# connortannahill/MM-ADMM

Hardware: AMD Instinct MI355X
Metric: ADMM iterations/sec on 1M-node 2D mesh; achieved HBM GB/s in SpMV (higher is better)
Workload: dtype f64

## Files before the change

### include/mmadmm.h

```cpp
#ifndef MMADMM_H
#define MMADMM_H
#include <stdint.h>

#ifdef __cplusplus
extern "C" {
#endif

#define MMADMM_OK 0
#define MMADMM_ERR_INVALID 1
#define MMADMM_ERR_HIP 2
#define MMADMM_ERR_INVERTED 3
#define MMADMM_ERR_IO 4
#define MMADMM_ERR_RCCL 5
#define MMADMM_ERR_NOCONV 6
#define MMADMM_ERR_NONFINITE 7

#define MMADMM_BOUNDARY_FREE 0
#define MMADMM_BOUNDARY_FIXED 1
#define MMADMM_INTERIOR 2

typedef struct mmadmm_engine* mmadmm_handle;
typedef struct mmadmm_meshbuf* mmadmm_mesh;

typedef void (*mmadmm_monitor_fn)(int dim, const double* x, double* M_rowmajor, void* user);

typedef struct mmadmm_params {
  double dt;
  double tau;
  double rho;
  int grad_use;
  int device;
  int rank;
  int nranks;
  int partition;
} mmadmm_params;

typedef struct mmadmm_stats {
  long long steps;
  long long admm_iters;
  long long bfgs_iters;
  int max_bfgs;
  double last_primal;
  double last_dual;
  double t_prox_ms;
  double t_xupdate_ms;
  double t_step_ms;
  long long n_prox;
  long long n_xupdate;
  long long n_steps_timed;
  double prox_bytes;
  double xupdate_bytes;
  long long newton_iters;
  long long jacobians;
  long long cg_iters;
  double t_jac_ms;
  double t_solve_ms;
  double t_be_ms;
  long long regrids;
  long long regrid_rows;
  double regrid_gather_bytes;
  long long regrid_cand;
  long long regrid_fallbacks;
  int monitor_iso;
  double t_exchange_ms;
  long long n_exchange;
  double halo_send_bytes;
  double halo_recv_bytes;
  int interior_nodes;
  int overlap;
} mmadmm_stats;

int mmadmm_regrid(mmadmm_handle h, double t);
int mmadmm_set_regrid(mmadmm_handle h, int every_step);

int mmadmm_regrid_values(mmadmm_handle h, const double* M);
int mmadmm_regrid_values_device(mmadmm_handle h, const double* d_M, void* producer_stream);
int mmadmm_regrid_field(mmadmm_handle h, const double* u, double alpha);
int mmadmm_regrid_field_device(mmadmm_handle h, const double* d_u, double alpha, void* producer_stream);
int mmadmm_field_hessian(mmadmm_handle h, const double* u, double* H);
int mmadmm_field_hessian_device(mmadmm_handle h, const double* d_u, double* d_H, void* stream);
int mmadmm_get_device(mmadmm_handle h, const char* what, double* d_out, void* consumer_stream);
int mmadmm_field_monitor(int dim, int nP, const double* Xp, int nF, const int32_t* F, const double* u,
                         double alpha, double* H, double* M);

int mmadmm_transfer(mmadmm_handle h, const double* Xold, const double* Xnew, int C, const double* uold, double* unew,
                    int32_t* where, int* counts);
int mmadmm_transfer_device(mmadmm_handle h, const double* d_Xold, const double* d_Xnew, int C, const double* d_uold,
                           double* d_unew, int32_t* d_where, int* counts, void* stream);
int mmadmm_transfer_field(int dim, int nP, const double* Xold, int nF, const int32_t* F, const double* Xnew, int C,
                          const double* uold, double* unew, int32_t* where, int* counts);
int mmadmm_face_neighbours(int dim, int nP, int nF, const int32_t* F, int32_t* nbr);

const char* mmadmm_last_error(void);
int mmadmm_version(void);
int mmadmm_build_info(char* out, int len);

int mmadmm_builtin_monitor(int dim, int mon_type, mmadmm_monitor_fn* fn, void** user);
int mmadmm_monitor_grid(int dim, int nP, const double* Xp, mmadmm_monitor_fn fn, void* user, int* rows,
                        double* vals);

int mmadmm_mesh_reorient(int dim, int nP, const double* Xp, int nF, int32_t* F);

int mmadmm_create(int dim, int nP, const double* Xp, const double* Xc, int nF, const int32_t* F,
                  const int32_t* mask, const mmadmm_params* p, mmadmm_monitor_fn fn, void* user,
                  mmadmm_handle* out);
int mmadmm_step(mmadmm_handle h, int n_iters, double tol, double* Ih, int* admm_iters);
int mmadmm_euler_step(mmadmm_handle h, double* Ih);
int mmadmm_backward_euler_step(mmadmm_handle h, double dt, double tol, double* Ih, int* newton_iters);
int mmadmm_get_jacobian(mmadmm_handle h, long long* nnz, int32_t* ia, int32_t* ja, double* a);
int mmadmm_be_begin(mmadmm_handle h, double dt, double* Ih);
int mmadmm_be_residual(mmadmm_handle h, double dt, double* F, double* norm1, double* Ih);
int mmadmm_be_fsubjac(mmadmm_handle h, double* a);
int mmadmm_be_add(mmadmm_handle h, const double* dx);
int mmadmm_energy(mmadmm_handle h, double* E);
int mmadmm_done(mmadmm_handle h);
int mmadmm_get(mmadmm_handle h, const char* what, double* out);
int mmadmm_get_simplices(mmadmm_handle h, int32_t* F);
int mmadmm_sizes(mmadmm_handle h, int* nP, int* nF, int* grid_rows);
int mmadmm_set_timing(mmadmm_handle h, int on);
int mmadmm_stats_get(mmadmm_handle h, mmadmm_stats* s);
int mmadmm_stats_reset(mmadmm_handle h);
int mmadmm_options_get(mmadmm_handle h, char* buf, int cap);
int mmadmm_sync(mmadmm_handle h);
int mmadmm_destroy(mmadmm_handle h);

int mmadmm_mesh_rect(int dim, int nx, int ny, int nz, double xa, double xb, double ya, double yb,
                     double za, double zb, int btype, mmadmm_mesh* out);
int mmadmm_mesh_levelset2d(int nx, int ny, double xa, double xb, double ya, double yb, int btype,
                           int compact_mask, mmadmm_mesh* out);
int mmadmm_mesh_levelset3d(int nx, int ny, int nz, double xa, double xb, double ya, double yb, double za,
                           double zb, int btype, int compact_mask, mmadmm_mesh* out);
int mmadmm_mesh_shoulder(int dim, int nx, int ny, int nz, double xa, double xb, double ya, double yb, double za,
                         double zb, int btype, mmadmm_mesh* out);
int mmadmm_mesh_reference_points(mmadmm_mesh h, double* Xc);
int mmadmm_mesh_hexdisc(int N, double r, double cx, double cy, int btype, mmadmm_mesh* out);
int mmadmm_mesh_read(int dim, const char* tri, const char* pnts, const char* mask, mmadmm_mesh* out);
int mmadmm_mesh_sizes(mmadmm_mesh m, int* dim, int* nP, int* nF, int* mask_len);
int mmadmm_mesh_copy(mmadmm_mesh m, double* Xp, int32_t* F, int32_t* mask);
int mmadmm_mesh_free(mmadmm_mesh m);
int mmadmm_write_points(const char* path, int dim, int nP, const double* Xp);
int mmadmm_write_simplices(const char* path, int dim, int nF, const int32_t* F);

int mmadmm_debug_blockgrad(mmadmm_handle h, int s, const double* z, const double* dxpu, int flags,
                           double* out);

#define MMADMM_PART_RCB 0
#define MMADMM_PART_RANGES 1
#define MMADMM_UNIQUE_ID_BYTES 128
typedef struct mmadmm_comm_s* mmadmm_comm;
typedef struct mmadmm_plan_s* mmadmm_plan;
int mmadmm_layout_check(unsigned* host_word);
int mmadmm_comm_unique_id(void* out, int len);
int mmadmm_comm_create_rccl(int nranks, int rank, const void* uid, int device, mmadmm_comm* out);
int mmadmm_comm_create_rccl_timeout(int nranks, int rank, const void* uid, int device, double timeout_s,
                                    mmadmm_comm* out);
int mmadmm_comm_create_loopback(int nranks, mmadmm_comm* out);
typedef int (*mmadmm_allgather_fn)(void* user, const double* send, double* recv, long long count);
typedef int (*mmadmm_exchange_fn)(void* user, int npeers, const int* peer_rank, const double* send,
                                  const long long* send_off, const long long* send_count, double* recv,
                                  const long long* recv_off, const long long* recv_count);
int mmadmm_comm_create_host(int nranks, int rank, mmadmm_allgather_fn allgather, mmadmm_exchange_fn exchange,
                            void* user, mmadmm_comm* out);
int mmadmm_comm_destroy(mmadmm_comm c);
int mmadmm_comm_nranks(mmadmm_comm c, int* nranks);
int mmadmm_create_partitioned(int dim, int nP, const double* Xp, const double* Xc, int nF, const int32_t* F,
                              const int32_t* mask, const mmadmm_params* p, mmadmm_monitor_fn fn, void* user,
                              mmadmm_comm comm, mmadmm_handle* out);
int mmadmm_local_nodes(mmadmm_handle h, int* n_local, int32_t* global_ids);
int mmadmm_plan_create(int dim, int nP, const double* Xp, int nF, const int32_t* F, int nranks, int rank, int method,
                       mmadmm_plan* out);
int mmadmm_plan_sizes(mmadmm_plan h, int* nLocalNodes, int* nLocalSimplices, int* nSources, int* nSend, int* nRecv,
                      int* nPeers, int* nInterface);
int mmadmm_plan_get(mmadmm_plan h, int32_t* localNodes, int32_t* localSimplices, int32_t* incPtr, int32_t* incSrc,
                    int32_t* sendOff, int32_t* peers);
int mmadmm_plan_destroy(mmadmm_plan h);

int mmadmm_devmath(int op, int n, const double* in, double* out);

#ifdef __cplusplus
}
#endif
#endif
```

### mm-admm_amd/csrc/host/engine.cpp

```cpp
#include <algorithm>
#include <chrono>
#include <cmath>
#include <cstring>
#include <limits>
#include <memory>
#include <mutex>
#include <string>
#include <vector>

#include "../../../include/mmx_sparse.h"
#include "../kernels/admm_kernels.h"
#include "../kernels/field_kernels.h"
#include "../kernels/regrid_kernels.h"
#include "../kernels/transfer_kernels.h"
#include "comm.h"
#include "common.h"
#include "partition.h"
#include "transfer.h"
#include "xup_records.h"

#define MMX_SP(expr)                                                                     \
  do {                                                                                   \
    const int rc_ = (expr);                                                              \
    if (rc_ != MMADMM_OK) throw ::mmx::Error(rc_, std::string(#expr) + ": " + mmadmm_last_error()); \
// ... 366 lines not shown
        timed_.push_back({a0, a1, b1});
      }
      prevEnd = b1;
      if (deferRed) {
        if (firstProx && i < nIters - 1) {
          prevEnd = nullptr;
          launch_reduce_partials(partA_.p + slice * i, nbp, res_ + (size_t)i * 2 * kNumPartials, st_, red_);
          firstDeferred = i + 1;
        } else if (i == nIters - 1) {
          const int i0 = firstProx ? i : firstDeferred;
          launch_reduce_steps(partA_.p + slice * i0, slice, nbp, partB_.p, nbx, nIters - i0,
                              res_ + (size_t)i0 * 2 * kNumPartials, st_, red_);
        }
      } else if (resid) {
        prevEnd = nullptr;
        launch_reduce_partials2(partA_.p, nbp, res_ + (size_t)i * 2 * kNumPartials, partB_.p, nbx,
                                res_ + (size_t)i * 2 * kNumPartials + kNumPartials, st_, red_);
      } else {
        prevEnd = nullptr;
        launch_reduce_partials(partA_.p, nbp, res_ + (size_t)i * 2 * kNumPartials, st_, red_);
      }
      done = i + 1;
      if (early) {
        std::vector<double> rv;
        fetchResults(res_ + (size_t)i * 2 * kNumPartials, 1, rv);
        const double* r = rv.data();
        primal = sqrt(r[kNumPartials + 2]);
        dual = sqrt(r[1]);
        if (r[4] > 0 || (primal < tol && dual < tol)) break;
      }
    }
    MMX_HIP(hipMemcpyAsync(Vp_.p, x_.p, (size_t)nP_ * D * sizeof(double), hipMemcpyDeviceToDevice, st_));
    vpVersion_++;
    if (timing) {
      eStep1 = nextEvent();
      MMX_HIP(hipEventRecord(eStep1, st_));
    }
    fetchResults(res_, done, hostRes_);
    MMX_HIP(hipGetLastError());
    bool bad = false;
    long long bf = 0;
    int mx = 0;
    for (int i = 0; i < done; ++i) {
      const double* r = &hostRes_[(size_t)i * 2 * kNumPartials];
      bad |= r[4] > 0;
      bf += (long long)r[3];
      mx = std::max(mx, (int)r[5]);
    }
#ifdef MMX_HINT_PROBE
    {
      double hits = 0;
      for (int i = 0; i < done; ++i) hits += hostRes_[(size_t)i * 2 * kNumPartials + 2];
      fprintf(stderr, "[hint-probe] step %lld: %.0f hits of %.0f lookups in %d proxes\n", (long long)stepsTaken_, hits,
              3.0 * nF_ * done, done);
    }
#endif
    const double* last = &hostRes_[(size_t)(done - 1) * 2 * kNumPartials];
    primal = sqrt(last[kNumPartials + 2]);
    dual = sqrt(last[1]);
    st_stats_.admm_iters += done;
    st_stats_.bfgs_iters += bf;
    st_stats_.max_bfgs = mx;
    st_stats_.last_primal = primal;
    st_stats_.last_dual = dual;
    st_stats_.steps += 1;
    if (timing) {
      stepEv_.push_back({eStep0, eStep1});
      if (evUsed_ >= kEvResolve) resolveTimed();
    }
    stepsTaken_++;
    if (bad) throwBad("in prox");
    if (Ih) *Ih = hostRes_[0];
    if (itersOut) *itersOut = done;
  }

  double eulerStep() override {
    clearInvFlag();
    int nb = 0;
    launch_grad_simplex<D>(m_, x_.p, gs_.p, false, partA_.p, &nb, st_);
    launch_reduce_partials(partA_.p, nb, res_, st_, red_);
    exchange(1);
    launch_euler_apply<D>(m_, knobs_, gs_.p, x_.p, prm_.dt / prm_.tau, st_);
    std::vector<double> rv;
    fetchResults(res_, 1, rv);
    const double* r = rv.data();
    if (r[4] > 0) throwBad("in the explicit Euler gradient");
    return r[0];
  }

  double backwardEulerStep(double dtBE, double tol, int* newtonOut) override {
    if (nranks_ > 1) throw Error(MMADMM_ERR_INVALID, "backward Euler runs on one rank (no element partition)");
    const auto tStep = Clock::now();
    const int n = nP_ * D;
    ensureJacobian();
    const double dtot = dtBE / prm_.tau;
    const double SAFETY_FAC = 1.0 / 10.0;
    const int MAX_ITERS = 1000;
    clearInvFlag();
    MMX_HIP(hipMemcpyAsync(xn_.p, x_.p, (size_t)n * sizeof(double), hipMemcpyDeviceToDevice, st_));
    int nb = 0, nb2 = 0;
    launch_grad_simplex<D>(m_, x_.p, gs_.p, false, partA_.p, &nb, st_);
    launch_euler_apply<D>(m_, knobs_, gs_.p, x_.p, dtot, st_);
    if (!beStepTaken_) buildJacobian(dtBE);
    int nIter = 0;
    double Ih = 0.0, normPrev = INFINITY;
    std::vector<double> rv;
    void* mst = nullptr;
    MMX_SP(mmx_matrix_stream(jac_, &mst));
    do {
      launch_grad_simplex<D>(m_, x_.p, gs_.p, false, partA_.p, &nb, st_);
      launch_be_residual<D>(m_, knobs_, gs_.p, x_.p, xn_.p, dtot, rhs_.p, partB_.p, &nb2, st_);
      launch_reduce_partials2(partA_.p, nb, res_, partB_.p, nb2, res_ + kNumPartials, st_, red_);
      fetchResults(res_, 1, rv);
      if (rv[4] > 0) throwBad("in backward Euler");
      Ih = rv[0];
      const double norm = rv[kNumPartials];
      if (norm < SAFETY_FAC * tol) break;
      if (!beStepTaken_ || std::fabs(norm - normPrev) / norm < 0.25) {
        buildJacobian(dtBE);
        beStepTaken_ = true;
      }
      waitStream();
      const auto tSolve = Clock::now();
      MMX_SP(mmx_matrix_set_rhs_device(jac_, rhs_.p));
      int cgIter = 0;
      MMX_SP(mmx_matrix_solve_device(jac_, &jprm_, dx_.p, &cgIter, 0));
      st_stats_.t_solve_ms += msSince(tSolve);
      if (cgIter > 0) st_stats_.cg_iters += cgIter;
      if (cgIter <= 0)
        throw Error(MMADMM_ERR_NOCONV, "backward Euler: CG-STAB did not converge (reference: assert(cgIter > 0))");
      launch_add_inplace(n, x_.p, dx_.p, st_);
      nIter++;
      normPrev = norm;
    } while (nIter < MAX_ITERS);
    streamWait();
    st_stats_.steps += 1;
    st_stats_.newton_iters += nIter;
    st_stats_.t_be_ms += msSince(tStep);
    if (newtonOut) *newtonOut = nIter;
    return Ih;
  }

  void newtonOp(int op, double dt, const double* in, double* out, double* sc) override {
    if (nranks_ > 1) throw Error(MMADMM_ERR_INVALID, "backward Euler runs on one rank (no element partition)");
    ensureJacobian();
    const int n = nP_ * D;
    std::vector<double> rv;
    int nb = 0, nb2 = 0;
    if (op == 0 || op == 1) clearInvFlag();
    if (op == 0) {
      MMX_HIP(hipMemcpyAsync(xn_.p, x_.p, (size_t)n * sizeof(double), hipMemcpyDeviceToDevice, st_));
      launch_grad_simplex<D>(m_, x_.p, gs_.p, false, partA_.p, &nb, st_);
      launch_reduce_partials(partA_.p, nb, res_, st_, red_);
      launch_euler_apply<D>(m_, knobs_, gs_.p, x_.p, dt / prm_.tau, st_);
      fetchResults(res_, 1, rv);
      if (rv[4] > 0) throwBad("in backward Euler");
      if (sc) sc[0] = rv[0];
    } else if (op == 1) {
      launch_grad_simplex<D>(m_, x_.p, gs_.p, false, partA_.p, &nb, st_);
      launch_be_residual<D>(m_, knobs_, gs_.p, x_.p, xn_.p, dt / prm_.tau, rhs_.p, partB_.p, &nb2, st_);
      launch_reduce_partials2(partA_.p, nb, res_, partB_.p, nb2, res_ + kNumPartials, st_, red_);
      fetchResults(res_, 1, rv);
      if (rv[4] > 0) throwBad("in backward Euler");
      std::vector<double> r((size_t)n);
      MMX_HIP(hipMemcpyAsync(r.data(), rhs_.p, (size_t)n * sizeof(double), hipMemcpyDeviceToHost, st_));
      streamWait();
      for (int i = 0; i < n; ++i) out[i] = -r[i];
      if (sc) {
        sc[0] = rv[0];
        sc[1] = rv[kNumPartials];
      }
    } else if (op == 2) {
      const double h = 10.0 * sqrt(std::numeric_limits<double>::epsilon());
      launch_fd_jac<D>(m_, Vp_.p, h, dv_.p, st_, fdWork_.p);
      clearInvFlag();
      if (jraw_.n != jja_.n) jraw_.alloc(std::max<size_t>(jja_.n, 1));
      launch_jac_assemble<D>(m_, knobs_, jia_.p, jja_.p, dv_.p, 1.0, jraw_.p, st_, false, maxColNodes_);
      MMX_HIP(hipMemcpyAsync(out, jraw_.p, jja_.n * sizeof(double), hipMemcpyDeviceToHost, st_));
      streamWait();
    } else if (op == 3) {
      MMX_HIP(hipMemcpyAsync(dx_.p, in, (size_t)n * sizeof(double), hipMemcpyHostToDevice, st_));
      launch_add_inplace(n, x_.p, dx_.p, st_);
      streamWait();
    } else {
      throw Error(MMADMM_ERR_INVALID, "newtonOp: unknown op");
    }
  }

  void jacobian(long long* nnz, int32_t* ia, int32_t* ja, double* a) override {
    if (!jac_) throw Error(MMADMM_ERR_INVALID, "no Jacobian yet: run a backward Euler step first");
    if (nnz) *nnz = (long long)jja_.n;
    if (ia) MMX_HIP(hipMemcpyAsync(ia, jia_.p, jia_.n * sizeof(int32_t), hipMemcpyDeviceToHost, st_));
    if (ja) MMX_HIP(hipMemcpyAsync(ja, jja_.p, jja_.n * sizeof(int32_t), hipMemcpyDeviceToHost, st_));
    if (a) MMX_HIP(hipMemcpyAsync(a, jval_.p, jval_.n * sizeof(double), hipMemcpyDeviceToHost, st_));
    streamWait();
  }

  double energy() override {
    int nb = 0;
    launch_energy<D>(m_, Vp_.p, partA_.p, &nb, st_);
    clearInvFlag();
    launch_reduce_partials(partA_.p, nb, res_, st_, red_);
    std::vector<double> rv;
    fetchResults(res_, 1, rv);
    return rv[0];
  }

  void done() override {
    MMX_HIP(hipMemcpyAsync(Vp_.p, x_.p, (size_t)nP_ * D * sizeof(double), hipMemcpyDeviceToDevice, st_));
    vpVersion_++;
    streamWait();
  }

  void get(const std::string& what, double* out) override {
    const DevBuf<double>* b = nullptr;
    if (what == "x") b = &x_;
    else if (what == "xPrev") b = &xPrev_;
    else if (what == "xBar") b = &xBar_;
    else if (what == "z" || what == "u") {
      if (!kZUInterleaved) {
        b = what == "z" ? &z_ : &u_;
      } else {
        std::vector<double> h(z_.n);
        MMX_HIP(hipMemcpyAsync(h.data(), z_.p, z_.n * sizeof(double), hipMemcpyDeviceToHost, st_));
        streamWait();
        const int sh = what == "u" ? D : 0;
        for (int s = 0; s < nF_; ++s)
          for (int i = 0; i < K; ++i) out[(size_t)s * K + i] = h[(size_t)s * 2 * K + (i / D) * 2 * D + i % D + sh];
        return;
      }
    }
    else if (what == "points") b = &Vp_;
    else if (what == "hess") b = &B_;
    else if (what == "gs") b = &gs_;
    else if (what == "grid") {
      if (gridOnDevice_) {
        MMX_HIP(hipMemcpyAsync(out, gvals_.p, gvals_.n * sizeof(double), hipMemcpyDeviceToHost, st_));
        streamWait();
      } else {
        std::memcpy(out, grid_.vals.data(), grid_.vals.size() * sizeof(double));
      }
      return;
    } else if (what == "Ehat") {
      std::memcpy(out, EhatH_, D * D * sizeof(double));
      return;
    } else {
      throw Error(MMADMM_ERR_INVALID, "mmadmm_get: unknown field '" + what + "'");
    }
    if (b == &B_) {
      std::vector<double> h(b->n);
      MMX_HIP(hipMemcpyAsync(h.data(), b->p, b->n * sizeof(double), hipMemcpyDeviceToHost, st_));
      streamWait();
      for (int s = 0; s < nF_; ++s)
        for (int ij = 0; ij < K * K; ++ij) out[(size_t)s * K * K + ij] = h[bIndex(s, ij)];
      return;
    }
    MMX_HIP(hipMemcpyAsync(out, b->p, b->n * sizeof(double), hipMemcpyDeviceToHost, st_));
    streamWait();
  }

  static size_t bIndex(int s, int ij) {
    if (D == 3 && MMX_B3_PAIRS) return ((size_t)(s >> 6) * K * K + (ij & ~1)) * 64 + 2 * (s & 63) + (ij & 1);
    return ((size_t)(s >> 6) * K * K + ij) * 64 + (s & 63);
  }

  void getSimplices(int32_t* F) override {
    for (size_t i = 0; i < plan_.Flocal.size(); ++i) F[i] = plan_.localNodes[plan_.Flocal[i]];
  }

  void localNodes(int* n, int32_t* ids) override {
    if (n) *n = nP_;
    if (ids) std::memcpy(ids, plan_.localNodes.data(), plan_.localNodes.size() * sizeof(int32_t));
  }

  void sizes(int* nP, int* nF, int* gridRows) override {
    if (nP) *nP = nP_;
    if (nF) *nF = nF_;
    if (gridRows) *gridRows = (int)(grid_.vals.size() / (D * D));
  }

  void setTiming(bool on) override {
    resolveTimed();
    timing_ = on;
  }

  void stats(mmadmm_stats* s) override {
    resolveTimed();
    *s = st_stats_;
    const double nF = nF_, nP = nP_;
    const double ts = knobs_.tslot ? 1.0 : 0.0;
    s->prox_bytes = nF * (4.0 * (D + 1) + 1 + 8.0 * (2 * K + K * K) * 2 + 8.0 * K * 2 + ts * 8.0 * K) +
                    nP * 8.0 * D;
    const double ch = D == 2 ? MMX_XU_CH2D : knobs_.xupCh;
    const double fixed = knobs_.xupRec ? nP * (4.0 * kXupRecInts + 8.0 + 4.0 * ch) + 4.0 * (double)xupTail_
                                 : 4.0 * (nP + 1) + 4.0 * (D + 1) * nF + 8.0 * nP;
    s->xupdate_bytes = fixed + (16.0 - 8.0 * ts) * K * nF + 8.0 * D * nP * 2;
    s->monitor_iso = iso_ ? 1 : 0;
    s->halo_send_bytes = 8.0 * D * (double)plan_.sendOff.size();
    s->halo_recv_bytes = nranks_ > 1 ? 8.0 * D * (double)plan_.recvRows : 0.0;
    s->interior_nodes = nInner_;
    s->overlap = knobs_.overlap;
  }

  std::string options() const override { return knobs_.text(); }

  void resetStats() override {
    resolveTimed();
    const mmadmm_stats z{};
    st_stats_ = z;
  }

  void resolveTimed() {
    if (stepEv_.empty() && timed_.empty() && exEv_.empty()) return;
    streamWait();
    float ms = 0;
    for (auto& p : stepEv_) {
      MMX_HIP(hipEventElapsedTime(&ms, p.first, p.second));
      st_stats_.t_step_ms += ms;
      st_stats_.n_steps_timed += 1;
    }
    if (st2_) MMX_HIP(hipStreamSynchronize(st2_));
    for (auto& p : exEv_) {
      MMX_HIP(hipEventElapsedTime(&ms, p.first, p.second));
      st_stats_.t_exchange_ms += ms;
      st_stats_.n_exchange += 1;
    }
    exEv_.clear();
    for (auto& t : timed_) {
      MMX_HIP(hipEventElapsedTime(&ms, t.a0, t.a1));
      st_stats_.t_prox_ms += ms;
      st_stats_.n_prox += 1;
      MMX_HIP(hipEventElapsedTime(&ms, t.a1, t.b1));
      st_stats_.t_xupdate_ms += ms;
      st_stats_.n_xupdate += 1;
    }
    stepEv_.clear();
    timed_.clear();
    evUsed_ = 0;
  }

  void sync() override { streamWait(); }

  void debugBlockGrad(int s, const double* z, const double* dx, int flags, double* out) override {
    if (s < 0 || s >= nF_) throw Error(MMADMM_ERR_INVALID, "debug_blockgrad: simplex out of range");
    DevBuf<double> dz, ddx, dout;
    dz.upload(z, K, st_);
    ddx.upload(dx, K, st_);
    dout.alloc(K + 2);
    launch_debug_blockgrad<D>(m_, s, dz.p, ddx.p, dout.p, flags, st_);
    MMX_HIP(hipMemcpyAsync(out, dout.p, (K + 2) * sizeof(double), hipMemcpyDeviceToHost, st_));
    streamWait();
  }

 private:
  struct Timed {
    hipEvent_t a0, a1, b1;
  };

  void profMark(const char* what, std::chrono::steady_clock::time_point& t) const {
    if (!knobs_.schedProf) return;
    const auto now = std::chrono::steady_clock::now();
    fprintf(stderr, "[sched] engine %s %.3f s\n", what, std::chrono::duration<double>(now - t).count());
    t = now;
  }
  void ensureJacobian() {
    if (jac_) return;
    auto tp = std::chrono::steady_clock::now();
    const int n = nP_ * D;
    mmx_struc sp = nullptr;
    MMX_SP(mmx_struc_create(n, 0, &sp));
    std::vector<int32_t> ia(n + 1), ja;
    long long nnz = 0;
    int rc = mmx_struc_mesh_pattern(sp, D, (int)(Fh_.size() / (D + 1)), Fh_.data());
    if (rc == MMADMM_OK) rc = mmx_struc_pack(sp);
    if (rc == MMADMM_OK) rc = mmx_struc_get(sp, nullptr, &nnz, nullptr, nullptr);
    if (rc == MMADMM_OK) {
      ja.resize(nnz);
      rc = mmx_struc_get(sp, nullptr, &nnz, ia.data(), ja.data());
    }
    profMark("pattern", tp);
    int dev = prm_.device;
    if (dev < 0) MMX_HIP(hipGetDevice(&dev));
    if (rc == MMADMM_OK) rc = mmx_matrix_create_from_struc(dev, sp, &jac_);
    (void)mmx_struc_destroy(sp);
    profMark("matrix create", tp);
    if (rc != MMADMM_OK) throw Error(rc, std::string("backward Euler Jacobian: ") + mmadmm_last_error());
    mmx_param_iter_mesh(&jprm_);
    maxColNodes_ = 0;
    for (int r = 0; r < n; ++r) maxColNodes_ = std::max(maxColNodes_, (ia[r + 1] - ia[r]) / D);
    jia_.upload(ia.data(), ia.size(), st_);
    jja_.upload(ja.data(), ja.size(), st_);
    jval_.alloc(std::max<size_t>(nnz, 1));
    dv_.alloc(std::max<size_t>((size_t)nF_ * (D + 1) * D * K, 1));
    if (knobs_.fdjFast) fdWork_.alloc((size_t)nF_ * (D + 1) + 1);
    xn_.alloc((size_t)n);
    rhs_.alloc((size_t)n);
    dx_.alloc((size_t)n);
    streamWait();
  }

  void buildJacobian(double dtBE) {
    if (jacVp_ == vpVersion_ && jacDt_ == dtBE) return;
    jacVp_ = vpVersion_;
    jacDt_ = dtBE;
    const auto t0 = Clock::now();
    auto tp = t0;
    const double h = 10.0 * sqrt(std::numeric_limits<double>::epsilon());
    launch_fd_jac<D>(m_, Vp_.p, h, dv_.p, st_, fdWork_.p);
    clearInvFlag();
    launch_jac_assemble<D>(m_, knobs_, jia_.p, jja_.p, dv_.p, dtBE / prm_.tau, jval_.p, st_, true, maxColNodes_);
    streamWait();
    profMark("FD Jacobian + assembly", tp);
    MMX_SP(mmx_matrix_set_values_device(jac_, jval_.p));
    if (!jacFactored_) {
      MMX_SP(mmx_matrix_sfac(jac_, &jprm_));
      jacFactored_ = true;
      profMark("sfac", tp);
    }
    streamWait();
    st_stats_.jacobians += 1;
    st_stats_.t_jac_ms += msSince(t0);
  }
  using Clock = std::chrono::steady_clock;
  static double msSince(Clock::time_point t) {
    return std::chrono::duration<double, std::milli>(Clock::now() - t).count();
  }

  static double hostDet(const double (&a)[3][3]) {
    if (D == 2) return a[0][0] * a[1][1] - a[1][0] * a[0][1];
    const double h0 = a[0][0] * (a[1][1] * a[2][2] - a[1][2] * a[2][1]);
    const double h1 = a[0][1] * (a[1][0] * a[2][2] - a[1][2] * a[2][0]);
    const double h2 = a[0][2] * (a[1][0] * a[2][1] - a[1][1] * a[2][0]);
    return h0 - h1 + h2;
  }

  void exchange(int mode, const PackZX& pz = {}, hipStream_t st = nullptr) {
    if (nranks_ == 1) return;
    if (!st) st = st_;
    hipEvent_t e0 = nullptr, e1 = nullptr;
    if (timing_ && mode == 0) {
      e0 = nextEvent();
      MMX_HIP(hipEventRecord(e0, st));
    }
    launch_pack_export<D>(mode, (int)plan_.sendOff.size(), expOff_.p, z_.p, uPtr(), gs_.p, w_, export_.p, st, pz);
    comm_->exchange(rank_, export_.p, remote_.p, plan_.peers, D, st);
    if (e0) {
      e1 = nextEvent();
      MMX_HIP(hipEventRecord(e1, st));
      exEv_.push_back({e0, e1});
    }
  }

  void xupdateHalo(const StepScalars& sc, int* nbx, bool resid, bool useTs, const PackZX& pz) {
    if (!knobs_.overlap) {
      exchange(0, pz);
      launch_xupdate<D>(m_, knobs_, sc, xBar_.p, z_.p, uPtr(), x_.p, partB_.p, nbx, resid, st_, useTs);
      return;
    }
    MMX_HIP(hipEventRecord(evProx_, st_));
    DeviceMesh<D> mi = m_;
    mi.xupHi = nInner_;
    int nb1 = 0, nb2 = 0;
    launch_xupdate<D>(mi, knobs_, sc, xBar_.p, z_.p, uPtr(), x_.p, partB_.p, &nb1, resid, st_, useTs);
    MMX_HIP(hipStreamWaitEvent(st2_, evProx_, 0));
    exchange(0, pz, st2_);
    MMX_HIP(hipEventRecord(evEx_, st2_));
    MMX_HIP(hipStreamWaitEvent(st_, evEx_, 0));
    DeviceMesh<D> mb = m_;
    mb.xupLo = nInner_;
    launch_xupdate<D>(mb, knobs_, sc, xBar_.p, z_.p, uPtr(), x_.p, partB_.p + (size_t)nb1 * kNumPartials, &nb2, resid,
                      st_, useTs);
    *nbx = nb1 + nb2;
  }

  void waitStream() {
    if (!knobs_.spin) {
      streamWait();
      return;
    }
    if (!evSync_) MMX_HIP(hipEventCreateWithFlags(&evSync_, hipEventDisableTiming));
    MMX_HIP(hipEventRecord(evSync_, st_));
    hipError_t r;
    while ((r = hipEventQuery(evSync_)) == hipErrorNotReady) __builtin_ia32_pause();
    MMX_HIP(r);
  }

  void streamWait() {
    if (nranks_ > 1 && comm_)
      comm_->wait(st_);
    else
      MMX_HIP(hipStreamSynchronize(st_));
  }

  void fetchResults(const double* dev, int rows, std::vector<double>& out) {
    const size_t cnt = (size_t)rows * 2 * kNumPartials;
    out.resize(cnt);
    if (resH_) {
      waitStream();
      std::memcpy(out.data(), resH_ + (dev - res_), cnt * sizeof(double));
      return;
    }
    if (nranks_ == 1) {
      MMX_HIP(hipMemcpyAsync(out.data(), dev, cnt * sizeof(double), hipMemcpyDeviceToHost, st_));
      streamWait();
      return;
    }
    if (resAll_.n < cnt * nranks_) resAll_.alloc(cnt * nranks_);
    comm_->allgather(rank_, dev, resAll_.p, cnt, st_);
    std::vector<double> all(cnt * nranks_);
    MMX_HIP(hipMemcpyAsync(all.data(), resAll_.p, all.size() * sizeof(double), hipMemcpyDeviceToHost, st_));
    streamWait();
    for (size_t i = 0; i < cnt; ++i) {
      const bool isMax = (i % kNumPartials) == 5;
      double v = all[i];
      for (int q = 1; q < nranks_; ++q) v = isMax ? std::max(v, all[(size_t)q * cnt + i]) : v + all[(size_t)q * cnt + i];
      out[i] = v;
    }
  }

  void setRegrid(bool on) override { regridEachStep_ = on; }

  void regrid(double t) override {
    if (nranks_ > 1) {
      const bool all = knobs_.regridGatherAll;
      if (!all && regridNear(t)) return;
      st_stats_.regrid_fallbacks += all ? 0 : 1;
    }
    regridAll(t);
  }

  void afterProducer(void* stream) {
    if (!stream) return;
    if (!evIn_) MMX_HIP(hipEventCreateWithFlags(&evIn_, hipEventDisableTiming));
    MMX_HIP(hipEventRecord(evIn_, (hipStream_t)stream));
    MMX_HIP(hipStreamWaitEvent(st_, evIn_, 0));
  }
  void beforeConsumer(void* stream) {
    if (!stream) {
      streamWait();
      return;
    }
    if (!evOut_) MMX_HIP(hipEventCreateWithFlags(&evOut_, hipEventDisableTiming));
    MMX_HIP(hipEventRecord(evOut_, st_));
    MMX_HIP(hipStreamWaitEvent((hipStream_t)stream, evOut_, 0));
  }
  void singleRankOnly(const char* what) const {
    if (nranks_ > 1) throw Error(MMADMM_ERR_INVALID, std::string(what) + ": single rank only (no element partition)");
  }
  void fieldScratch() {
    if (fldE_.p) return;
    fldE_.alloc(std::max<size_t>(field_ebuf_doubles<D>(nF_), 1));
    fldG_.alloc((size_t)nP_ * D);
  }

  void regridFrom(int src, const double* p, bool onDevice, double alpha, void* stream) override {
    singleRankOnly(src == kMonField ? "mmadmm_regrid_field" : "mmadmm_regrid_values");
    const size_t n = (size_t)nP_ * (src == kMonField ? 1 : D * D);
    if (!onDevice) {
      if (fldIn_.n < n) fldIn_.alloc(n);
      MMX_HIP(hipMemcpyAsync(fldIn_.p, p, n * sizeof(double), hipMemcpyHostToDevice, st_));
      streamWait();
      p = fldIn_.p;
    } else {
      afterProducer(stream);
    }
    srcPtr_ = p;
    srcAlpha_ = alpha;
    regridAll(0.0, (MonSource)src);
    srcPtr_ = nullptr;
    if (onDevice && !knobs_.iso) streamWait();
  }

  void fieldHessian(const double* u, double* H, bool onDevice, void* stream) override {
    singleRankOnly("mmadmm_field_hessian");
    fieldScratch();
    if (!onDevice) {
      if (fldIn_.n < (size_t)nP_) fldIn_.alloc(nP_);
      if (fldOut_.n < (size_t)nP_ * D * D) fldOut_.alloc((size_t)nP_ * D * D);
      MMX_HIP(hipMemcpyAsync(fldIn_.p, u, (size_t)nP_ * sizeof(double), hipMemcpyHostToDevice, st_));
      launch_field_hessian<D>(Vp_.p, fldIn_.p, F_.p, nF_, incPtr_.p, incOff_.p, nodeOrder_.p, nP_, fldE_.p, fldG_.p, 1.0,
                              fldOut_.p, nullptr, st_);
      MMX_HIP(hipGetLastError());
      MMX_HIP(hipMemcpyAsync(H, fldOut_.p, (size_t)nP_ * D * D * sizeof(double), hipMemcpyDeviceToHost, st_));
      streamWait();
      return;
    }
    afterProducer(stream);
    launch_field_hessian<D>(Vp_.p, u, F_.p, nF_, incPtr_.p, incOff_.p, nodeOrder_.p, nP_, fldE_.p, fldG_.p, 1.0, H,
                            nullptr, st_);
    MMX_HIP(hipGetLastError());
    beforeConsumer(stream);
  }

  void transferScratch() {
    if (trNbr_.p) return;
    trNbrH_.assign(std::max<size_t>((size_t)nF_ * (D + 1), 1), -1);
    build_face_neighbours(D, nF_, plan_.Flocal.data(), trNbrH_.data());
    trNbr_.upload(trNbrH_.data(), trNbrH_.size(), st_);
    trWhere_.alloc(std::max(nP_, 1));
    trCnt_.alloc(kTransferCountInts);
  }

  void transfer(const double* Xold, const double* Xnew, int C, const double* uold, double* unew, int32_t* where,
                int* counts, bool onDevice, void* stream) override {
    const char* who = onDevice ? "mmadmm_transfer_device" : "mmadmm_transfer";
    singleRankOnly(who);
    transferScratch();
    const size_t nx = (size_t)nP_ * D, nu = (size_t)nP_ * C;
    int cnt[kTransferCountInts];
    if (!onDevice) {
      if (trStage_.n < 2 * nx + 2 * nu) trStage_.alloc(2 * nx + 2 * nu);
      double *dXo = trStage_.p, *dXn = dXo + nx, *dUo = dXn + nx, *dUn = dUo + nu;
      MMX_HIP(hipMemcpyAsync(dXo, Xold, nx * sizeof(double), hipMemcpyHostToDevice, st_));
      if (Xnew) MMX_HIP(hipMemcpyAsync(dXn, Xnew, nx * sizeof(double), hipMemcpyHostToDevice, st_));
      MMX_HIP(hipMemcpyAsync(dUo, uold, nu * sizeof(double), hipMemcpyHostToDevice, st_));
      launch_transfer<D>(dXo, Xnew ? dXn : Vp_.p, F_.p, incPtr_.p, incOff_.p, nodeOrder_.p, trNbr_.p, nP_, C, dUo, dUn,
                         trWhere_.p, trCnt_.p, st_);
      MMX_HIP(hipGetLastError());
      MMX_HIP(hipMemcpyAsync(unew, dUn, nu * sizeof(double), hipMemcpyDeviceToHost, st_));
      if (where) MMX_HIP(hipMemcpyAsync(where, trWhere_.p, (size_t)nP_ * sizeof(int32_t), hipMemcpyDeviceToHost, st_));
      if (counts) MMX_HIP(hipMemcpyAsync(cnt, trCnt_.p, sizeof cnt, hipMemcpyDeviceToHost, st_));
      streamWait();
    } else {
      if (D == 2 && ((((uintptr_t)Xold) | ((uintptr_t)(Xnew ? Xnew : Vp_.p))) & 15))
        throw Error(MMADMM_ERR_INVALID, std::string(who) + ": 2D position arrays must be 16-byte aligned");
      afterProducer(stream);
      launch_transfer<D>(Xold, Xnew ? Xnew : Vp_.p, F_.p, incPtr_.p, incOff_.p, nodeOrder_.p, trNbr_.p, nP_, C, uold, unew,
                         where ? where : trWhere_.p, trCnt_.p, st_);
      MMX_HIP(hipGetLastError());
      if (counts) MMX_HIP(hipMemcpyAsync(cnt, trCnt_.p, sizeof cnt, hipMemcpyDeviceToHost, st_));
      beforeConsumer(stream);
      if (counts && stream) streamWait();
    }
    if (counts) transfer_sum_counts(cnt, counts);
  }

  void getDevice(const std::string& what, double* dOut, void* stream) override {
    singleRankOnly("mmadmm_get_device");
    const DevBuf<double>* b = what == "x" ? &x_ : what == "points" ? &Vp_ : nullptr;
    if (!b) throw Error(MMADMM_ERR_INVALID, "mmadmm_get_device: unknown field '" + what + "' (x, points)");
    MMX_HIP(hipMemcpyAsync(dOut, b->p, (size_t)nP_ * D * sizeof(double), hipMemcpyDeviceToDevice, st_));
    beforeConsumer(stream);
  }

  bool regridNear(double t) {
    constexpr int DD = D * D;
    const int nG = plan_.nP;
    const int nbl = std::max(1, std::min(256, (nP_ + 255) / 256));
    const int nbe = std::max(1, std::min(256, (nF_ + 255) / 256));
    const size_t smallN = (size_t)std::max(2 * D, nranks_);
    if (!rgnPart_.p) {
      rgnPart_.alloc((size_t)256 * 2 * D + 256 * D);
      rgnSmallS_.alloc(smallN);
      rgnSmallR_.alloc(smallN * nranks_);
      rgnSbox_.alloc((size_t)nranks_ * 2 * D);
      rgnCnt_.alloc(nranks_ + 1);
      rgnSend_.alloc((size_t)nranks_ * maxOwned_ * (D + 1));
      rgnGid_.upload(plan_.localNodes.data(), plan_.localNodes.size(), st_);
      ownGidH_.assign(ownAllGidH_.begin() + (size_t)rank_ * maxOwned_,
                      ownAllGidH_.begin() + (size_t)rank_ * maxOwned_ + std::max(nOwned_, 1));
      rgnOwnGid_.upload(ownGidH_.data(), ownGidH_.size(), st_);
      rgTmp_.alloc(gvals_.n);
      rgTmp2_.alloc(gvals_.n);
      MMX_HIP(hipHostMalloc((void**)&rgnHost_, sizeof(double) * ((size_t)256 * 3 * D + 2 * smallN * nranks_ + 64),
                            hipHostMallocDefault));
    }
    double* H0 = rgnHost_;
    launch_bbox<D>(Vp_.p, nP_, rgnPart_.p, nbl, st_);
    launch_extent<D>(Vp_.p, F_.p, nF_, rgnPart_.p + (size_t)256 * 2 * D, nbe, st_);
    MMX_HIP(hipMemcpyAsync(H0, rgnPart_.p, sizeof(double) * nbl * 2 * D, hipMemcpyDeviceToHost, st_));
    MMX_HIP(hipMemcpyAsync(H0 + (size_t)256 * 2 * D, rgnPart_.p + (size_t)256 * 2 * D, sizeof(double) * nbe * D,
                           hipMemcpyDeviceToHost, st_));
    streamWait();
    double llo[3] = {INFINITY, INFINITY, INFINITY}, lhi[3] = {-INFINITY, -INFINITY, -INFINITY};
    for (int b = 0; b < nbl; ++b)
      for (int d = 0; d < D; ++d) {
        llo[d] = std::min(llo[d], H0[(size_t)b * 2 * D + d]);
        lhi[d] = std::max(lhi[d], H0[(size_t)b * 2 * D + D + d]);
      }
    for (int d = 0; d < D; ++d) extMax_[d] = 0.0;
    for (int b = 0; b < nbe; ++b)
      for (int d = 0; d < D; ++d) extMax_[d] = std::max(extMax_[d], H0[(size_t)256 * 2 * D + (size_t)b * D + d]);
    double* hs = H0 + (size_t)256 * 3 * D;
    double* hr = hs + smallN;
    auto smallGather = [&](const double* in, int n) {
      MMX_HIP(hipMemcpyAsync(rgnSmallS_.p, in, sizeof(double) * n, hipMemcpyHostToDevice, st_));
      comm_->allgather(rank_, rgnSmallS_.p, rgnSmallR_.p, (size_t)n, st_);
      MMX_HIP(hipMemcpyAsync(hr, rgnSmallR_.p, sizeof(double) * n * nranks_, hipMemcpyDeviceToHost, st_));
      streamWait();
    };
    for (int d = 0; d < D; ++d) {
      hs[d] = llo[d];
      hs[D + d] = lhi[d];
    }
    smallGather(hs, 2 * D);
    double lo[3] = {INFINITY, INFINITY, INFINITY}, hi[3] = {-INFINITY, -INFINITY, -INFINITY};
    for (int q = 0; q < nranks_; ++q)
      for (int d = 0; d < D; ++d) {
        lo[d] = std::min(lo[d], hr[(size_t)q * 2 * D + d]);
        hi[d] = std::max(hi[d], hr[(size_t)q * 2 * D + D + d]);
      }
    setGridGeometry(nG, lo, hi);
    const CellGrid cg = cellGrid(lo, hi);
    int marg[3] = {0, 0, 0};
    const GridBox R = rowBox(llo, lhi, marg);
    const int passes = smoothPasses();
    const GridBox H = widenBox(R, passes);
    double slo[3] = {0, 0, 0}, shi[3] = {0, 0, 0};
    double diam = 0.0;
    for (int d = 0; d < D; ++d) diam += extMax_[d] * extMax_[d];
    diam = std::sqrt(diam);
    const double marginScale = knobs_.regridMargin;
    for (int d = 0; d < D; ++d) {
      const std::vector<double>& g = d == 0 ? grid_.gx : d == 1 ? grid_.gy : grid_.gz;
      const int sd = (D == 3 && d < 2) ? 1 - d : d;
      const double mu = marginScale * (diam + 2.0 * (g[1] - g[0]));
      slo[d] = g[H.lo[sd]] - mu;
      shi[d] = g[H.hi[sd]] + mu;
    }
    for (int d = 0; d < D; ++d) {
      hs[d] = slo[d];
      hs[D + d] = shi[d];
    }
    smallGather(hs, 2 * D);
    MMX_HIP(hipMemcpyAsync(rgnSbox_.p, hr, sizeof(double) * nranks_ * 2 * D, hipMemcpyHostToDevice, st_));
    MMX_HIP(hipMemsetAsync(rgnCnt_.p, 0, sizeof(int) * (nranks_ + 1), st_));
    launch_select_owned<D>(Vp_.p, ownLocal_.p, rgnOwnGid_.p, nOwned_, nranks_, rank_, rgnSbox_.p, rgnCnt_.p,
                           rgnSend_.p, maxOwned_, st_);
    std::vector<int> cnt(nranks_ + 1);
    MMX_HIP(hipMemcpyAsync(cnt.data(), rgnCnt_.p, sizeof(int) * nranks_, hipMemcpyDeviceToHost, st_));
    streamWait();
    for (int q = 0; q < nranks_; ++q) hs[q] = (double)cnt[q];
    smallGather(hs, nranks_);
    std::vector<HaloPeer> peers;
    int nRecv = 0;
    for (int q = 0; q < nranks_; ++q) {
      if (q == rank_) continue;
      const int sc = cnt[q], rc = (int)hr[(size_t)q * nranks_ + rank_];
      if (sc == 0 && rc == 0) continue;
      HaloPeer p;
      p.rank = q;
      p.sendOff = q * maxOwned_;
      p.sendCount = sc;
      p.recvOff = nRecv;
      p.recvCount = rc;
      nRecv += rc;
      peers.push_back(p);
    }
    const int nCand = nP_ + nRecv;
    if ((int)rgnRecv_.n < std::max(nRecv, 1) * (D + 1)) rgnRecv_.alloc((size_t)std::max(nRecv, 1) * (D + 1) * 2);
    if ((int)rgnCandX_.n < nCand * D) {
      rgnCandX_.alloc((size_t)nCand * D * 2);
      rgnCandGid_.alloc((size_t)nCand * 2);
      rgnCellOf_.alloc((size_t)nCand * 2);
      rgnNodes_.alloc((size_t)nCand * 2);
      rgnMon_.alloc((size_t)nCand * DD * 2);
    }
    comm_->exchange(rank_, rgnSend_.p, rgnRecv_.p, peers, D + 1, st_);
    launch_build_cand<D>(Vp_.p, rgnGid_.p, nP_, rgnRecv_.p, nRecv, rgnCandX_.p, rgnCandGid_.p, st_);
    evalMonitorAt(rgnCandX_.p, nCand, t, rgnMon_.p);
    ensureCells(cg);
    launch_bin<D>(rgnCandX_.p, nCand, cg, rgnCellOf_.p, rgCounts_.p, rgStarts_.p, rgFill_.p, rgnNodes_.p, rgScan_.p,
                  rgScanBytes_, st_);
    double clo[3], chi[3];
    for (int d = 0; d < 3; ++d) {
      clo[d] = (d < D && slo[d] <= lo[d]) ? -INFINITY : slo[d];
      chi[d] = (d < D && shi[d] >= hi[d]) ? INFINITY : shi[d];
    }
    NnCand nc{rgnCandGid_.p, {clo[0], clo[1], clo[2]}, {chi[0], chi[1], chi[2]}, rgnCnt_.p + nranks_};
    launch_nn_fill<D>(rgnCandX_.p, cg, rgStarts_.p, rgnNodes_.p, gx_.p, gy_.p, D == 3 ? gz_.p : gy_.p, grid_.nx,
                      grid_.ny, grid_.nz, rgnMon_.p, rgTmp_.p, H, st_, nc);
    int fail = 0;
    MMX_HIP(hipMemcpyAsync(&fail, rgnCnt_.p + nranks_, sizeof(int), hipMemcpyDeviceToHost, st_));
    streamWait();
    hs[0] = (double)fail;
    smallGather(hs, 1);
    for (int q = 0; q < nranks_; ++q)
      if (hr[q] != 0.0) return false;
    smoothCommit(R, passes, true);
    st_stats_.regrid_rows = (long long)(H.hi[0] - H.lo[0] + 1) * (H.hi[1] - H.lo[1] + 1) * (H.hi[2] - H.lo[2] + 1);
    st_stats_.regrid_gather_bytes = (double)sizeof(double) * ((size_t)nranks_ * (4 * D + nranks_ + 1) +
                                                              (size_t)nRecv * (D + 1));
    st_stats_.regrid_cand = nCand;
    MMX_HIP(hipGetLastError());
    gridOnDevice_ = true;
    updateIso();
    m_ = makeView();
    st_stats_.regrids += 1;
    return true;
  }

  void updateIso() {
    iso_ = false;
    if (!knobs_.iso) return;
    const long long np = (long long)(gvals_.n / (D * D));
    if (np <= 0) return;
    if ((long long)giso_.n != np) giso_.alloc(np);
    if (!isoFlag_.p) isoFlag_.alloc(1);
    MMX_HIP(hipMemsetAsync(isoFlag_.p, 0, sizeof(int), st_));
    launch_iso_compact<D>(gvals_.p, np, giso_.p, isoFlag_.p, st_);
    int notIso = 1;
    MMX_HIP(hipMemcpyAsync(&notIso, isoFlag_.p, sizeof(int), hipMemcpyDeviceToHost, st_));
    streamWait();
    iso_ = (notIso == 0);
  }
  void uploadGridCoords() {
    gx_.upload(grid_.gx.data(), grid_.gx.size(), st_);
    gy_.upload(grid_.gy.data(), grid_.gy.size(), st_);
    if (D == 3) {
      gz_.upload(grid_.gz.data(), grid_.gz.size(), st_);
      const std::vector<double>* ax[3] = {&grid_.gx, &grid_.gy, &grid_.gz};
      for (int a = 0; a < 3; ++a) {
        const std::vector<double>& g = *ax[a];
        const size_t nc = g.size() > 1 ? g.size() - 1 : 1;
        std::vector<double>& t = gcellH_[a];
        t.assign(4 * nc, 0.0);
        for (size_t i = 0; i + 1 < g.size(); ++i) {
          const double h = g[i + 1] - g[i];
          t[4 * i] = g[i];
          t[4 * i + 1] = h;
          t[4 * i + 2] = 1.0 / h;
        }
        gcell_[a].upload(t.data(), t.size(), st_);
      }
    }
  }
  void setGridGeometry(int nG, const double* lo, const double* hi) {
    grid_geometry(D, nG, lo, hi, grid_);
    uploadGridCoords();
  }
  CellGrid cellGrid(const double* lo, const double* hi) const {
    CellGrid cg{};
    const int gn[3] = {grid_.nx, grid_.ny, grid_.nz};
    cg.hmin = INFINITY;
    for (int d = 0; d < 3; ++d) {
      const double ext = d < D ? hi[d] - lo[d] : 0.0;
      cg.lo[d] = d < D ? lo[d] : 0.0;
      cg.n[d] = (d < D && ext > 0) ? std::max(1, gn[d] / 2) : 1;
      cg.inv[d] = (d < D && ext > 0) ? cg.n[d] / ext : 0.0;
      if (d < D && ext > 0) cg.hmin = std::min(cg.hmin, ext / cg.n[d]);
    }
    if (!(cg.hmin < INFINITY)) cg.hmin = 0.0;
    return cg;
  }
  void ensureCells(const CellGrid& cg) {
    const int ncell = cg.n[0] * cg.n[1] * cg.n[2];
    if ((int)rgStarts_.n < ncell + 1) {
      rgCounts_.alloc(ncell + 1);
      rgStarts_.alloc(ncell + 1);
      rgFill_.alloc(ncell);
      rgScanBytes_ = bin_scan_bytes(ncell);
      rgScan_.alloc(std::max<size_t>(rgScanBytes_, 1));
    }
  }
  static int smoothPasses() { return (D == 2) ? 5 : 2; }
  GridBox rowBox(const double* llo, const double* lhi, int* marg) const {
    const int gn3[3] = {grid_.nx, grid_.ny, D == 3 ? grid_.nz : 0};
    GridBox R{{0, 0, 0}, {gn3[0], gn3[1], gn3[2]}};
    for (int d = 0; d < D; ++d) {
      const std::vector<double>& g = d == 0 ? grid_.gx : d == 1 ? grid_.gy : grid_.gz;
      const double h = g[1] - g[0];
      const int M = (int)std::ceil(2.0 * extMax_[d] / h) + 2;
      marg[d] = M;
      R.lo[d] = std::max(0, std::min(gn3[d], (int)std::floor((llo[d] - g[0]) / h) - M));
      R.hi[d] = std::max(0, std::min(gn3[d], (int)std::floor((lhi[d] - g[0]) / h) + 1 + M));
    }
    return R;
  }
  GridBox widenBox(const GridBox& b, int w) const {
    const int gn3[3] = {grid_.nx, grid_.ny, D == 3 ? grid_.nz : 0};
    GridBox o = b;
    for (int d = 0; d < D; ++d) {
      o.lo[d] = std::max(0, b.lo[d] - w);
      o.hi[d] = std::min(gn3[d], b.hi[d] + w);
    }
    return o;
  }
  void evalMonitorAt(const double* X, int n, double t, double* mon) {
    constexpr int DD = D * D;
    if (builtin_monitor_kind(monFn_, monUser_) == 7) {
      double c[3];
      moving_bump_centre(t, c);
      launch_monitor_tv<D>(X, n, c, mon, st_);
    } else {
      std::vector<double> Xh((size_t)n * D), mv((size_t)n * DD);
      MMX_HIP(hipMemcpyAsync(Xh.data(), X, Xh.size() * sizeof(double), hipMemcpyDeviceToHost, st_));
      streamWait();
      for (int v = 0; v < n; ++v) {
        double M[9];
        for (int i = 0; i < DD; ++i) M[i] = 0.0;
        monFn_(D, &Xh[(size_t)v * D], M, monUser_);
        std::memcpy(&mv[(size_t)v * DD], M, DD * sizeof(double));
      }
      MMX_HIP(hipMemcpyAsync(mon, mv.data(), mv.size() * sizeof(double), hipMemcpyHostToDevice, st_));
      streamWait();
    }
  }
  void smoothCommit(const GridBox& R, int passes, bool part) {
    double* cur = rgTmp_.p;
    double* oth = part ? rgTmp2_.p : gvals_.p;
    for (int it = 0; it < passes; ++it) {
      launch_smooth<D>(cur, oth, grid_.nx, grid_.ny, grid_.nz, widenBox(R, part ? passes - 1 - it : 0), st_);
      std::swap(cur, oth);
    }
    if (part) {
      launch_box_commit<D>(cur, gvals_.p, D == 3 ? gpad_.p : nullptr, grid_.nx, grid_.ny, grid_.nz, R, st_);
    } else {
      if (cur != gvals_.p)
        MMX_HIP(hipMemcpyAsync(gvals_.p, cur, gvals_.n * sizeof(double), hipMemcpyDeviceToDevice, st_));
      if (D == 3) launch_pad_rows(gvals_.p, (long long)(gvals_.n / 9), gpad_.p, st_);
    }
  }

  void regridAll(double t, MonSource src = kMonCallback) {
    constexpr int DD = D * D;
    const int nG = (nranks_ > 1) ? plan_.nP : nP_;
    const int nb = std::max(1, std::min(256, (nG + 255) / 256));
    if (!rgPart_.p) {
      rgPart_.alloc((size_t)512 * 2 * D + 256 * D);
      rgMon_.alloc((size_t)nG * DD);
      rgCellOf_.alloc(nG);
      rgNodes_.alloc(nG);
      rgTmp_.alloc(gvals_.n);
      if (nranks_ > 1) rgTmp2_.alloc(gvals_.n);
      if (nranks_ > 1) {
        rgXg_.alloc((size_t)nG * D);
        rgSend_.alloc((size_t)maxOwned_ * D);
        rgRecv_.alloc((size_t)nranks_ * maxOwned_ * D);
      }
      MMX_HIP(hipHostMalloc((void**)&rgHost_, sizeof(double) * (512 * 2 * D + 256 * D), hipHostMallocDefault));
    }
    const double* X = Vp_.p;
    const bool part = nranks_ > 1;
    const int nbl = part ? std::max(1, std::min(256, (nP_ + 255) / 256)) : 0;
    const int nbe = part ? std::max(1, std::min(256, (nF_ + 255) / 256)) : 0;
    double* extPart = rgPart_.p + (size_t)512 * 2 * D;
    if (part) {
      launch_rows_gather(D, ownLocal_.p, nOwned_, Vp_.p, rgSend_.p, st_);
      comm_->allgather(rank_, rgSend_.p, rgRecv_.p, (size_t)maxOwned_ * D, st_);
      launch_rows_scatter(D, ownAllGid_.p, nranks_ * maxOwned_, rgRecv_.p, rgXg_.p, st_);
      X = rgXg_.p;
      launch_bbox<D>(Vp_.p, nP_, rgPart_.p + (size_t)256 * 2 * D, nbl, st_);
      launch_extent<D>(Vp_.p, F_.p, nF_, extPart, nbe, st_);
    }
    launch_bbox<D>(X, nG, rgPart_.p, nb, st_);
    MMX_HIP(hipMemcpyAsync(rgHost_, rgPart_.p, sizeof(double) * nb * 2 * D, hipMemcpyDeviceToHost, st_));
    if (part) {
      MMX_HIP(hipMemcpyAsync(rgHost_ + (size_t)256 * 2 * D, rgPart_.p + (size_t)256 * 2 * D, sizeof(double) * nbl * 2 * D,
                             hipMemcpyDeviceToHost, st_));
      MMX_HIP(hipMemcpyAsync(rgHost_ + (size_t)512 * 2 * D, extPart, sizeof(double) * nbe * D, hipMemcpyDeviceToHost,
                             st_));
    }
    streamWait();
    double lo[3] = {INFINITY, INFINITY, INFINITY}, hi[3] = {-INFINITY, -INFINITY, -INFINITY};
    double llo[3] = {INFINITY, INFINITY, INFINITY}, lhi[3] = {-INFINITY, -INFINITY, -INFINITY};
    for (int b = 0; b < nb; ++b)
      for (int d = 0; d < D; ++d) {
        lo[d] = std::min(lo[d], rgHost_[(size_t)b * 2 * D + d]);
        hi[d] = std::max(hi[d], rgHost_[(size_t)b * 2 * D + D + d]);
      }
    for (int b = 0; b < nbl; ++b)
      for (int d = 0; d < D; ++d) {
        llo[d] = std::min(llo[d], rgHost_[(size_t)(256 + b) * 2 * D + d]);
        lhi[d] = std::max(lhi[d], rgHost_[(size_t)(256 + b) * 2 * D + D + d]);
      }
    if (part) {
      for (int d = 0; d < D; ++d) extMax_[d] = 0.0;
      for (int b = 0; b < nbe; ++b)
        for (int d = 0; d < D; ++d) extMax_[d] = std::max(extMax_[d], rgHost_[(size_t)512 * 2 * D + (size_t)b * D + d]);
    }
    grid_geometry(D, nG, lo, hi, grid_);
    uploadGridCoords();
    CellGrid cg{};
    const int gn[3] = {grid_.nx, grid_.ny, grid_.nz};
    cg.hmin = INFINITY;
    for (int d = 0; d < 3; ++d) {
      const double ext = d < D ? hi[d] - lo[d] : 0.0;
      cg.lo[d] = d < D ? lo[d] : 0.0;
      cg.n[d] = (d < D && ext > 0) ? std::max(1, gn[d] / 2) : 1;
      cg.inv[d] = (d < D && ext > 0) ? cg.n[d] / ext : 0.0;
      if (d < D && ext > 0) cg.hmin = std::min(cg.hmin, ext / cg.n[d]);
    }
    if (!(cg.hmin < INFINITY)) cg.hmin = 0.0;
    const int ncell = cg.n[0] * cg.n[1] * cg.n[2];
    if ((int)rgStarts_.n < ncell + 1) {
      rgCounts_.alloc(ncell + 1);
      rgStarts_.alloc(ncell + 1);
      rgFill_.alloc(ncell);
      rgScanBytes_ = bin_scan_bytes(ncell);
      rgScan_.alloc(std::max<size_t>(rgScanBytes_, 1));
    }
    launch_bin<D>(X, nG, cg, rgCellOf_.p, rgCounts_.p, rgStarts_.p, rgFill_.p, rgNodes_.p, rgScan_.p, rgScanBytes_,
                  st_);
    if (src == kMonCallback && builtin_monitor_kind(monFn_, monUser_) == 7) src = kMonBuiltin7;
    if (src == kMonValues) {
      MMX_HIP(hipMemcpyAsync(rgMon_.p, srcPtr_, (size_t)nG * DD * sizeof(double), hipMemcpyDeviceToDevice, st_));
    } else if (src == kMonField) {
      fieldScratch();
      launch_field_hessian<D>(X, srcPtr_, F_.p, nF_, incPtr_.p, incOff_.p, nodeOrder_.p, nP_, fldE_.p, fldG_.p,
                              srcAlpha_, nullptr, rgMon_.p, st_);
    } else if (src == kMonBuiltin7) {
      double c[3];
      moving_bump_centre(t, c);
      launch_monitor_tv<D>(X, nG, c, rgMon_.p, st_);
    } else {
      std::vector<double> Xh((size_t)nG * D), mv((size_t)nG * DD);
      MMX_HIP(hipMemcpyAsync(Xh.data(), X, Xh.size() * sizeof(double), hipMemcpyDeviceToHost, st_));
      streamWait();
      for (int v = 0; v < nG; ++v) {
        double M[9];
        for (int i = 0; i < DD; ++i) M[i] = 0.0;
        monFn_(D, &Xh[(size_t)v * D], M, monUser_);
        std::memcpy(&mv[(size_t)v * DD], M, DD * sizeof(double));
      }
      MMX_HIP(hipMemcpyAsync(rgMon_.p, mv.data(), mv.size() * sizeof(double), hipMemcpyHostToDevice, st_));
      streamWait();
    }
    const int passes = (D == 2) ? 5 : 2;
    const int gn3[3] = {grid_.nx, grid_.ny, D == 3 ? grid_.nz : 0};
    GridBox R{{0, 0, 0}, {gn3[0], gn3[1], gn3[2]}};
    if (part) {
      for (int d = 0; d < D; ++d) {
        const std::vector<double>& g = d == 0 ? grid_.gx : d == 1 ? grid_.gy : grid_.gz;
        const double h = g[1] - g[0];
        const int M = (int)std::ceil(2.0 * extMax_[d] / h) + 2;
        R.lo[d] = std::max(0, std::min(gn3[d], (int)std::floor((llo[d] - g[0]) / h) - M));
        R.hi[d] = std::max(0, std::min(gn3[d], (int)std::floor((lhi[d] - g[0]) / h) + 1 + M));
      }
    }
    auto widen = [&](const GridBox& b, int w) {
      GridBox o = b;
      for (int d = 0; d < D; ++d) {
        o.lo[d] = std::max(0, b.lo[d] - w);
        o.hi[d] = std::min(gn3[d], b.hi[d] + w);
      }
      return o;
    };
    const GridBox H = widen(R, part ? passes : 0);
    launch_nn_fill<D>(X, cg, rgStarts_.p, rgNodes_.p, gx_.p, gy_.p, D == 3 ? gz_.p : gy_.p, grid_.nx, grid_.ny,
                      grid_.nz, rgMon_.p, rgTmp_.p, H, st_);
    double* cur = rgTmp_.p;
    double* oth = part ? rgTmp2_.p : gvals_.p;
    for (int it = 0; it < passes; ++it) {
      launch_smooth<D>(cur, oth, grid_.nx, grid_.ny, grid_.nz, widen(R, part ? passes - 1 - it : 0), st_);
      std::swap(cur, oth);
    }
    if (part) {
      launch_box_commit<D>(cur, gvals_.p, D == 3 ? gpad_.p : nullptr, grid_.nx, grid_.ny, grid_.nz, R, st_);
    } else {
      if (cur != gvals_.p)
        MMX_HIP(hipMemcpyAsync(gvals_.p, cur, gvals_.n * sizeof(double), hipMemcpyDeviceToDevice, st_));
      if (D == 3) launch_pad_rows(gvals_.p, (long long)(gvals_.n / 9), gpad_.p, st_);
    }
    st_stats_.regrid_rows = (long long)(H.hi[0] - H.lo[0] + 1) * (H.hi[1] - H.lo[1] + 1) * (H.hi[2] - H.lo[2] + 1);
    st_stats_.regrid_gather_bytes = part ? (double)nranks_ * maxOwned_ * D * sizeof(double) : 0.0;
    st_stats_.regrid_cand = part ? nG : 0;
    MMX_HIP(hipGetLastError());
    gridOnDevice_ = true;
    updateIso();
    m_ = makeView();
    st_stats_.regrids += 1;
  }

  DeviceMesh<D> makeView() const {
    DeviceMesh<D> m{};
    m.nP = nP_;
    m.nF = nF_;
    m.F = F_.p;
    m.sbits = sbits_.p;
    m.nodeInterior = interior_.p;
    m.inc_ptr = incPtr_.p;
    m.inc_off = incOff_.p;
    m.remote = nranks_ > 1 ? remote_.p : nullptr;
    m.tslot = knobs_.tslot ? tslot_.p : nullptr;
    m.gcache = gcache_.p;
    m.tieList = tieList_.p;
    m.tieCount = tieCount_.p + tiePar_;
    m.tieStale = tieCount_.p + (tiePar_ ^ 1);
    m.invFlag = tieCount_.p + 2;
    m.nodeOrder = nodeOrder_.p;
    m.xupLo = 0;
    m.xupHi = nP_;
    m.prox2dWave = knobs_.prox2dWave;
    m.xupSweep = knobs_.xupSweep;
    m.xupCh = knobs_.xupCh;
    m.xupEarly = knobs_.xupEarly;
    m.forceTie = knobs_.forceTie;
    m.monHint = knobs_.monHint;
    if (knobs_.xupRec) {
      m.xrec = xrec_.p;
      m.xinv = xinv_.p;
      m.xslot = xslot_.p;
      m.xslotStride = xslotStride_;
      m.xslotCh = xslotCh_;
    }
    m.invdiag = invdiag_.p;
    m.Vc = compMesh_ ? Vc_.p : nullptr;
    m.gx = gx_.p;
    m.gy = gy_.p;
    m.gz = (D == 3) ? gz_.p : gy_.p;
    m.gvals = gvals_.p;
    m.gpad = (D == 3) ? gpad_.p : nullptr;
    for (int a = 0; a < 3; ++a) m.gcell[a] = (D == 3) ? gcell_[a].p : nullptr;
    m.giso = iso_ ? giso_.p : nullptr;
    m.gnx = grid_.nx;
    m.gny = grid_.ny;
    m.gnz = grid_.nz;
    m.ghx = grid_.gx[1] - grid_.gx[0];
    m.ghy = grid_.gy[1] - grid_.gy[0];
    m.ghz = (D == 3) ? grid_.gz[1] - grid_.gz[0] : 1.0;
    m.grhx = 1.0 / m.ghx;
    m.grhy = 1.0 / m.ghy;
    m.grhz = 1.0 / m.ghz;
    const int ns[3] = {grid_.nx, grid_.ny, grid_.nz};
    double* A[3] = {&m.gax, &m.gay, &m.gaz};
    double* SP[3] = {&m.gspx, &m.gspy, &m.gspz};
    double* NS[3] = {&m.gnsx, &m.gnsy, &m.gnsz};
    double* RNS[3] = {&m.grnsx, &m.grnsy, &m.grnsz};
    for (int d = 0; d < 3; ++d) {
      const bool on = d < D;
      *A[d] = on ? grid_.lo[d] : 0.0;
      *SP[d] = on ? grid_.hi[d] - grid_.lo[d] : 0.0;
      *NS[d] = on ? (double)ns[d] : 1.0;
      *RNS[d] = 1.0 / *NS[d];
    }
    for (int i = 0; i < D * D; ++i) m.Ehat[i] = EhatH_[i];
    m.powd = powd_;
    m.w = w_;
    m.compMesh = compMesh_ ? 1 : 0;
    return m;
  }

  void ensureResults(int nIters) {
    if (nIters <= resultsCap_) return;
    resultsCap_ = std::max(nIters, 64);
    const size_t n = (size_t)resultsCap_ * 2 * kNumPartials;
    if (nranks_ == 1 && knobs_.spin) {
      if (resH_) MMX_HIP(hipHostFree(resH_));
      resH_ = nullptr;
      MMX_HIP(hipHostMalloc((void**)&resH_, n * sizeof(double), hipHostMallocMapped));
      MMX_HIP(hipHostGetDevicePointer((void**)&res_, resH_, 0));
    } else {
      results_.alloc(n);
      res_ = results_.p;
    }
  }

  void clearInvFlag() { MMX_HIP(hipMemsetAsync(tieCount_.p + 2, 0, sizeof(unsigned), st_)); }

  [[noreturn]] void throwBad(const char* where) {
    unsigned flag = 0;
    MMX_HIP(hipMemcpyAsync(&flag, tieCount_.p + 2, sizeof(unsigned), hipMemcpyDeviceToHost, st_));
    streamWait();
    if (flag) {
      MMX_HIP(hipMemsetAsync(tieCount_.p + 2, 0, sizeof(unsigned), st_));
      streamWait();
      throw Error(MMADMM_ERR_INVERTED, std::string("inverted element ") + where + " (reference: assert(Edet > 0))");
    }
    if (nranks_ > 1 && regridEachStep_)
      throw Error(MMADMM_ERR_NONFINITE, std::string("non-finite energy ") + where +
                                            ": a monitor evaluation left this rank's regrid box (no element inverted)");
    throw Error(MMADMM_ERR_NONFINITE, std::string("non-finite energy ") + where +
                                          " without an inverted element (a monitor value that is not finite)");
  }

  hipEvent_t nextEvent() {
    if (evUsed_ == evPool_.size()) {
      hipEvent_t e;
      MMX_HIP(hipEventCreateWithFlags(&e, hipEventDisableSystemFence));
      evPool_.push_back(e);
    }
    return evPool_[evUsed_++];
  }

  static std::vector<int32_t> orientedSimplices(int nP, const double* Xp, int nF, const int32_t* F) {
    std::vector<int32_t> Fh(F, F + (size_t)nF * (D + 1));
    for (int32_t v : Fh)
      if (v < 0 || v >= nP) throw Error(MMADMM_ERR_INVALID, "simplex vertex id out of range");
    reorient_simplices(D, Xp, nF, Fh.data());
    return Fh;
  }

  std::vector<int32_t> Fh_;
  PartitionPlan plan_;
  const EngineKnobs knobs_;
  int nP_ = 0, nF_ = 0;
  mmadmm_params prm_{};
  bool compMesh_ = false;
  double w_ = 0, powd_ = 0;
  double EhatH_[9] = {0};
  std::vector<int32_t> maskH_;
  HostGrid grid_;
  mmadmm_monitor_fn monFn_ = nullptr;
  void* monUser_ = nullptr;
  bool regridEachStep_ = false, gridOnDevice_ = false;
  DevBuf<double> rgPart_, rgMon_, rgTmp_, rgTmp2_, rgXg_, rgSend_, rgRecv_;
  DevBuf<double> fldE_, fldG_, fldIn_, fldOut_;
  std::vector<int32_t> trNbrH_;
  DevBuf<int32_t> trNbr_, trWhere_, trCnt_;
  DevBuf<double> trStage_;
  const double* srcPtr_ = nullptr;
  double srcAlpha_ = 1.0;
  hipEvent_t evIn_ = nullptr, evOut_ = nullptr;
  double extMax_[3] = {0.0, 0.0, 0.0};
  DevBuf<int> ownLocal_, ownAllGid_;
  std::vector<int> ownAllGidH_, ownGidH_;
  DevBuf<double> rgnPart_, rgnSmallS_, rgnSmallR_, rgnSbox_, rgnSend_, rgnRecv_, rgnCandX_, rgnMon_;
  DevBuf<int> rgnCnt_, rgnGid_, rgnOwnGid_, rgnCandGid_, rgnCellOf_, rgnNodes_;
  double* rgnHost_ = nullptr;
  int nOwned_ = 0, maxOwned_ = 1;
  DevBuf<int> rgCellOf_, rgNodes_, rgCounts_, rgStarts_, rgFill_;
  DevBuf<unsigned char> rgScan_;
  size_t rgScanBytes_ = 0;
  double* rgHost_ = nullptr;
  hipStream_t st_ = nullptr;
  hipStream_t st2_ = nullptr;
  hipEvent_t evProx_ = nullptr, evEx_ = nullptr;
  int nInner_ = 0;
  std::vector<std::pair<hipEvent_t, hipEvent_t>> exEv_;
  DevBuf<int32_t> F_, incPtr_, incOff_;
  DevBuf<double> tslot_;
  DevBuf<uint8_t> sbits_, interior_;
  DevBuf<double> gcell_[3];
  DevBuf<double> giso_;
  DevBuf<int> isoFlag_;
  bool iso_ = false;
  std::vector<double> gcellH_[3];
  DevBuf<double> invdiag_, Vc_, gx_, gy_, gz_, gvals_, Vp_, x_, xPrev_, xBar_, z_, u_, gs_, B_, B2_, gcache_, gpad_;
  DevBuf<double> partA_, partB_, results_, export_, remote_, resAll_, redScratch_;
  RedWork red_;
  DevBuf<int32_t> expOff_, tieList_, nodeOrder_;
  DevBuf<int32_t> xrec_, xslot_;
  DevBuf<double> xinv_;
  int xslotStride_ = 0, xslotCh_ = 0;
  long long xupTail_ = 0;
  DevBuf<unsigned> tieCount_;
  int tiePar_ = 0;
  Comm* comm_ = nullptr;
  int rank_ = 0, nranks_ = 1;
  int resultsCap_ = 0;
  std::vector<double> hostRes_;
  DeviceMesh<D> m_{};
  bool hessComputed_ = false, stepTaken_ = false, gcacheValid_ = false;
  mmx_matrix jac_ = nullptr;
  mmx_param_iter jprm_{};
  bool beStepTaken_ = false, jacFactored_ = false;
  long long vpVersion_ = 0, jacVp_ = -1;
  double jacDt_ = 0.0;
  DevBuf<int32_t> jia_, jja_;
  DevBuf<double> jval_, jraw_, dv_, xn_, rhs_, dx_;
  DevBuf<unsigned> fdWork_;
  int maxColNodes_ = 65;
  int stepsTaken_ = 0;
  size_t maxBlocks_ = 1;
  static constexpr int kDeferMax = 64;
  bool timing_ = false;
  std::vector<hipEvent_t> evPool_;
  size_t evUsed_ = 0;
  static constexpr bool kZUInterleaved = (D == 2) && MMX_ZU_INTER;
  double* uPtr() const { return kZUInterleaved ? z_.p + D : u_.p; }
  void clearU() {
    if (kZUInterleaved)
      MMX_HIP(hipMemsetAsync(z_.p, 0, z_.n * sizeof(double), st_));
    else
      MMX_HIP(hipMemsetAsync(u_.p, 0, u_.n * sizeof(double), st_));
  }
  double* res_ = nullptr;
  double* resH_ = nullptr;
  hipEvent_t evSync_ = nullptr;
  std::vector<Timed> timed_;
  std::vector<std::pair<hipEvent_t, hipEvent_t>> stepEv_;
  static constexpr size_t kEvResolve = 4096;
  mmadmm_stats st_stats_{};
};

}

using mmx::EngineBase;
using mmx::Error;
using mmx::guarded;

struct mmadmm_engine {
  std::unique_ptr<EngineBase> e;
};

static EngineBase& eng(mmadmm_handle h) {
  if (!h || !h->e) throw Error(MMADMM_ERR_INVALID, "null engine handle");
  return *h->e;
}

extern "C" {

const char* mmadmm_last_error(void) { return mmx::g_last_error.c_str(); }
int mmadmm_version(void) { return 100; }

int mmadmm_mesh_reorient(int dim, int nP, const double* Xp, int nF, int32_t* F) {
  return guarded([&] {
    if ((dim != 2 && dim != 3) || nP < 1 || nF < 0 || !Xp || (nF > 0 && !F))
      throw Error(MMADMM_ERR_INVALID, "mmadmm_mesh_reorient: bad arguments");
    for (long long i = 0; i < (long long)nF * (dim + 1); ++i)
      if (F[i] < 0 || F[i] >= nP) throw Error(MMADMM_ERR_INVALID, "simplex vertex id out of range");
    mmx::reorient_simplices(dim, Xp, nF, F);
  });
}

int mmadmm_create(int dim, int nP, const double* Xp, const double* Xc, int nF, const int32_t* F, const int32_t* mask,
                  const mmadmm_params* p, mmadmm_monitor_fn fn, void* user, mmadmm_handle* out) {
  return guarded([&] {
    if (!out) throw Error(MMADMM_ERR_INVALID, "mmadmm_create: out is NULL");
    *out = nullptr;
    if ((dim != 2 && dim != 3) || nP < dim + 1 || nF < 1 || !Xp || !F || !mask || !p || !fn)
      throw Error(MMADMM_ERR_INVALID, "mmadmm_create: bad arguments");
    if (!(p->dt > 0) || !(p->tau > 0) || !(p->rho > 0))
      throw Error(MMADMM_ERR_INVALID, "mmadmm_create: dt, tau, rho must be positive");
    if (p->nranks > 1) throw Error(MMADMM_ERR_INVALID, "mmadmm_create: use mmadmm_create_partitioned for nranks > 1");
    mmx::check_kernel_layout(mmx::kLayoutWord);
    int ndev = 0;
    if (hipGetDeviceCount(&ndev) != hipSuccess || ndev == 0)
      throw Error(MMADMM_ERR_HIP, "mmadmm_create: no HIP device (the engine has no CPU fallback)");
    auto* h = new mmadmm_engine();
    try {
      if (dim == 2)
        h->e.reset(new mmx::Engine<2>(nP, Xp, Xc, nF, F, mask, *p, fn, user, nullptr));
      else
        h->e.reset(new mmx::Engine<3>(nP, Xp, Xc, nF, F, mask, *p, fn, user, nullptr));
    } catch (...) {
      delete h;
      throw;
    }
    *out = h;
  });
}

int mmadmm_create_partitioned(int dim, int nP, const double* Xp, const double* Xc, int nF, const int32_t* F,
                              const int32_t* mask, const mmadmm_params* p, mmadmm_monitor_fn fn, void* user,
                              mmadmm_comm comm, mmadmm_handle* out) {
  return guarded([&] {
    if (!out) throw Error(MMADMM_ERR_INVALID, "mmadmm_create_partitioned: out is NULL");
    *out = nullptr;
    if ((dim != 2 && dim != 3) || nP < dim + 1 || nF < 1 || !Xp || !F || !mask || !p || !fn)
      throw Error(MMADMM_ERR_INVALID, "mmadmm_create_partitioned: bad arguments");
    if (!(p->dt > 0) || !(p->tau > 0) || !(p->rho > 0))
      throw Error(MMADMM_ERR_INVALID, "mmadmm_create_partitioned: dt, tau, rho must be positive");
    if (p->nranks < 1 || p->rank < 0 || p->rank >= p->nranks)
      throw Error(MMADMM_ERR_INVALID, "mmadmm_create_partitioned: bad rank / nranks");
    mmx::Comm* c = mmx::comm_of(comm);
    if (p->nranks > 1 && (!c || c->nranks != p->nranks))
      throw Error(MMADMM_ERR_INVALID, "mmadmm_create_partitioned: communicator missing or of another size");
    mmx::check_kernel_layout(mmx::kLayoutWord);
    int ndev = 0;
    if (hipGetDeviceCount(&ndev) != hipSuccess || ndev == 0)
      throw Error(MMADMM_ERR_HIP, "mmadmm_create_partitioned: no HIP device (the engine has no CPU fallback)");
    auto* h = new mmadmm_engine();
    try {
      if (dim == 2)
        h->e.reset(new mmx::Engine<2>(nP, Xp, Xc, nF, F, mask, *p, fn, user, c));
      else
        h->e.reset(new mmx::Engine<3>(nP, Xp, Xc, nF, F, mask, *p, fn, user, c));
    } catch (...) {
      delete h;
      throw;
    }
    *out = h;
  });
}

int mmadmm_local_nodes(mmadmm_handle h, int* n_local, int32_t* global_ids) {
  return guarded([&] { eng(h).localNodes(n_local, global_ids); });
}

int mmadmm_step(mmadmm_handle h, int n_iters, double tol, double* Ih, int* admm_iters) {
  return guarded([&] { eng(h).step(n_iters, tol, Ih, admm_iters); });
}
int mmadmm_euler_step(mmadmm_handle h, double* Ih) {
  return guarded([&] {
    const double r = eng(h).eulerStep();
    if (Ih) *Ih = r;
  });
}
int mmadmm_backward_euler_step(mmadmm_handle h, double dt, double tol, double* Ih, int* newton_iters) {
  return guarded([&] {
    if (!(dt > 0)) throw mmx::Error(MMADMM_ERR_INVALID, "backward Euler: dt must be > 0");
    const double r = eng(h).backwardEulerStep(dt, tol, newton_iters);
    if (Ih) *Ih = r;
  });
}
int mmadmm_be_begin(mmadmm_handle h, double dt, double* Ih) {
  return guarded([&] {
    if (!(dt > 0)) throw mmx::Error(MMADMM_ERR_INVALID, "backward Euler: dt must be > 0");
    double sc[2] = {0.0, 0.0};
    eng(h).newtonOp(0, dt, nullptr, nullptr, sc);
    if (Ih) *Ih = sc[0];
  });
}
int mmadmm_be_residual(mmadmm_handle h, double dt, double* F, double* norm1, double* Ih) {
  return guarded([&] {
    if (!F) throw mmx::Error(MMADMM_ERR_INVALID, "mmadmm_be_residual: F is NULL");
    double sc[2] = {0.0, 0.0};
    eng(h).newtonOp(1, dt, nullptr, F, sc);
    if (Ih) *Ih = sc[0];
    if (norm1) *norm1 = sc[1];
  });
}
int mmadmm_be_fsubjac(mmadmm_handle h, double* a) {
  return guarded([&] {
    if (!a) throw mmx::Error(MMADMM_ERR_INVALID, "mmadmm_be_fsubjac: a is NULL");
    eng(h).newtonOp(2, 0.0, nullptr, a, nullptr);
  });
}
int mmadmm_be_add(mmadmm_handle h, const double* dx) {
  return guarded([&] {
    if (!dx) throw mmx::Error(MMADMM_ERR_INVALID, "mmadmm_be_add: dx is NULL");
    eng(h).newtonOp(3, 0.0, dx, nullptr, nullptr);
  });
}
int mmadmm_get_jacobian(mmadmm_handle h, long long* nnz, int32_t* ia, int32_t* ja, double* a) {
  return guarded([&] { eng(h).jacobian(nnz, ia, ja, a); });
}
int mmadmm_energy(mmadmm_handle h, double* E) {
  return guarded([&] {
    const double r = eng(h).energy();
    if (E) *E = r;
  });
}
int mmadmm_done(mmadmm_handle h) {
  return guarded([&] { eng(h).done(); });
}
int mmadmm_get(mmadmm_handle h, const char* what, double* out) {
  return guarded([&] {
    if (!what || !out) throw Error(MMADMM_ERR_INVALID, "mmadmm_get: NULL argument");
    eng(h).get(what, out);
  });
}
int mmadmm_get_simplices(mmadmm_handle h, int32_t* F) {
  return guarded([&] { eng(h).getSimplices(F); });
}
int mmadmm_sizes(mmadmm_handle h, int* nP, int* nF, int* grid_rows) {
  return guarded([&] { eng(h).sizes(nP, nF, grid_rows); });
}
int mmadmm_set_timing(mmadmm_handle h, int on) {
  return guarded([&] { eng(h).setTiming(on != 0); });
}
int mmadmm_stats_get(mmadmm_handle h, mmadmm_stats* s) {
  return guarded([&] {
    if (!s) throw Error(MMADMM_ERR_INVALID, "NULL stats");
    eng(h).stats(s);
  });
}
int mmadmm_options_get(mmadmm_handle h, char* buf, int cap) {
  int need = 0;
  const int rc = guarded([&] { need = mmx::knobs_detail::copy_out(eng(h).options(), buf, cap); });
  return rc == MMADMM_OK ? need : -rc;
}
int mmadmm_stats_reset(mmadmm_handle h) {
  return guarded([&] { eng(h).resetStats(); });
}
int mmadmm_regrid(mmadmm_handle h, double t) {
  return guarded([&] { eng(h).regrid(t); });
}
int mmadmm_set_regrid(mmadmm_handle h, int every_step) {
  return guarded([&] { eng(h).setRegrid(every_step != 0); });
}
int mmadmm_regrid_values(mmadmm_handle h, const double* M) {
  return guarded([&] {
    if (!M) throw Error(MMADMM_ERR_INVALID, "mmadmm_regrid_values: M is NULL");
    eng(h).regridFrom(mmx::kMonValues, M, false, 1.0, nullptr);
  });
}
int mmadmm_regrid_values_device(mmadmm_handle h, const double* d_M, void* producer_stream) {
  return guarded([&] {
    if (!d_M) throw Error(MMADMM_ERR_INVALID, "mmadmm_regrid_values_device: d_M is NULL");
    eng(h).regridFrom(mmx::kMonValues, d_M, true, 1.0, producer_stream);
  });
}
static void check_alpha(const char* who, double alpha) {
  if (!(std::isfinite(alpha) && alpha > 0))
    throw Error(MMADMM_ERR_INVALID, std::string(who) + ": alpha must be finite and > 0");
}
int mmadmm_regrid_field(mmadmm_handle h, const double* u, double alpha) {
  return guarded([&] {
    if (!u) throw Error(MMADMM_ERR_INVALID, "mmadmm_regrid_field: u is NULL");
    check_alpha("mmadmm_regrid_field", alpha);
    eng(h).regridFrom(mmx::kMonField, u, false, alpha, nullptr);
  });
}
int mmadmm_regrid_field_device(mmadmm_handle h, const double* d_u, double alpha, void* producer_stream) {
  return guarded([&] {
    if (!d_u) throw Error(MMADMM_ERR_INVALID, "mmadmm_regrid_field_device: d_u is NULL");
    check_alpha("mmadmm_regrid_field_device", alpha);
    eng(h).regridFrom(mmx::kMonField, d_u, true, alpha, producer_stream);
  });
}
int mmadmm_field_hessian(mmadmm_handle h, const double* u, double* H) {
  return guarded([&] {
    if (!u || !H) throw Error(MMADMM_ERR_INVALID, "mmadmm_field_hessian: NULL array");
    eng(h).fieldHessian(u, H, false, nullptr);
  });
}
int mmadmm_field_hessian_device(mmadmm_handle h, const double* d_u, double* d_H, void* stream) {
  return guarded([&] {
    if (!d_u || !d_H) throw Error(MMADMM_ERR_INVALID, "mmadmm_field_hessian_device: NULL array");
    eng(h).fieldHessian(d_u, d_H, true, stream);
  });
}
static void check_transfer(const char* who, const double* Xold, int C, const double* uold, const double* unew) {
  if (C < 1) throw Error(MMADMM_ERR_INVALID, std::string(who) + ": C must be >= 1");
  if (!Xold || !uold || !unew) throw Error(MMADMM_ERR_INVALID, std::string(who) + ": NULL array");
  if (unew == uold) throw Error(MMADMM_ERR_INVALID, std::string(who) + ": unew must not be uold");
}
int mmadmm_transfer(mmadmm_handle h, const double* Xold, const double* Xnew, int C, const double* uold, double* unew,
                    int32_t* where, int* counts) {
  return guarded([&] {
    check_transfer("mmadmm_transfer", Xold, C, uold, unew);
    eng(h).transfer(Xold, Xnew, C, uold, unew, where, counts, false, nullptr);
// ... 41 lines not shown
```

### mm-admm_amd/csrc/host/knobs.h

```cpp
#pragma once
#include <climits>
#include <cstdio>
#include <cstdlib>
#include <cstring>
#include <stdexcept>
#include <string>

namespace mmx {

constexpr int kTslot2dMax = 2 * 2048 * 64;
constexpr int kXupEarlyDefault = 1;
constexpr int kRedSplitMin = 4096;
constexpr int kProxBlock = 64;
constexpr int kSweepGrid = 128;
constexpr int kFacWaveChunk = 0;
constexpr int kChainImportLat = 8;
constexpr int kFacImpRows = 384;
constexpr int kFacRMax = 4;

inline int env_int(const char* name, int dflt, int lo = INT_MIN, int hi = INT_MAX) {
  const char* e = std::getenv(name);
  if (!e) return dflt;
  const int v = std::atoi(e);
  return v < lo ? lo : v > hi ? hi : v;
}
inline int env_flag(const char* name, bool dflt) { return env_int(name, dflt ? 1 : 0) != 0 ? 1 : 0; }
inline int env_word(const char* name, const char* words) {
  const char* e = std::getenv(name);
  if (!e) return 0;
  const size_t n = std::strlen(e);
  int i = 0;
  for (const char* w = words; *w; ++i) {
    const char* bar = std::strchr(w, '|');
    const size_t len = bar ? (size_t)(bar - w) : std::strlen(w);
    if (len == n && std::strncmp(w, e, n) == 0) return i;
    w += len + (bar ? 1 : 0);
  }
  return 0;
}
inline int env_set(const char* name) { return std::getenv(name) != nullptr ? 1 : 0; }
inline double env_double(const char* name, double dflt) {
  const char* e = std::getenv(name);
  return e ? std::atof(e) : dflt;
}

namespace knobs_detail {
inline int snap_xup_ch(int c) { return c >= 24 ? 24 : c >= 16 ? 16 : 8; }
inline int one_of3(int v, int a, int b, int c, int dflt) { return (v == a || v == b || v == c) ? v : dflt; }
inline int in_range_or(int v, int lo, int hi, int dflt) { return (v < lo || v > hi) ? dflt : v; }
inline void put(std::string& s, const char* name, const char* words, int v) {
  s += name;
  s += '=';
  if (!words) {
    s += std::to_string(v);
  } else {
    const char* w = words;
    for (int i = 0; i < v; ++i) w = std::strchr(w, '|') + 1;
    const char* bar = std::strchr(w, '|');
    s.append(w, bar ? (size_t)(bar - w) : std::strlen(w));
  }
  s += '\n';
}
inline void put(std::string& s, const char* name, const char*, double v) {
  char b[64];
  std::snprintf(b, sizeof b, "%.17g", v);
  s += name;
  s += '=';
  s += b;
  s += '\n';
}
inline int copy_out(const std::string& s, char* buf, int cap) {
  if (buf && cap > 0) {
    const size_t n = s.size() < (size_t)cap - 1 ? s.size() : (size_t)cap - 1;
    std::memcpy(buf, s.data(), n);
    buf[n] = 0;
  }
  return (int)s.size() + 1;
}
}

#define MMX_ENGINE_KNOBS(X) \
   \
   \
  X(int, tslot, "MMX_TSLOT", nullptr, env_flag("MMX_TSLOT", D == 3 || nF <= kTslot2dMax)) \
   \
  X(int, spin, "MMX_SPIN", nullptr, env_flag("MMX_SPIN", true)) \
   \
  X(int, zx, "MMX_ZX", nullptr, env_flag("MMX_ZX", true)) \
   \
  X(int, overlap, "MMX_OVERLAP", nullptr, nranks > 1 && env_flag("MMX_OVERLAP", true)) \
   \
  X(int, fusePred, "MMX_FUSE_PRED", nullptr, env_flag("MMX_FUSE_PRED", true)) \
   \
  X(int, gcSkip, "MMX_GC_SKIP", nullptr, env_flag("MMX_GC_SKIP", true)) \
   \
  X(int, xupOrder, "MMX_XUP_ORDER", nullptr, env_int("MMX_XUP_ORDER", D == 3) == 1) \
   \
  X(int, xupRec, "MMX_XUP_REC", nullptr, env_flag("MMX_XUP_REC", true)) \
   \
  X(int, xupCh, "MMX_XUP_CH", nullptr, knobs_detail::snap_xup_ch(env_int("MMX_XUP_CH", 8))) \
   \
   \
   \
  X(int, xupSweep, "MMX_XUP_SWEEP", nullptr, env_int("MMX_XUP_SWEEP", D == 3 ? 1 : (k.xupRec ? 2 : 0), 0)) \
   \
  X(int, xupEarly, "MMX_XUP_EARLY", nullptr, env_flag("MMX_XUP_EARLY", kXupEarlyDefault != 0)) \
   \
  X(int, xupSweepResid, "MMX_XUP_SWEEP_RESID", nullptr, env_flag("MMX_XUP_SWEEP_RESID", true)) \
   \
   \
  X(int, xcdMap, "MMX_XCD_MAP", nullptr, env_int("MMX_XCD_MAP", 1)) \
   \
  X(int, prox2dWave, "MMX_PROX2D", "lds|wave", D == 2 && env_word("MMX_PROX2D", "lds|wave")) \
   \
  X(int, prox3dQuad, "MMX_PROX3D", "wave|quad", env_word("MMX_PROX3D", "wave|quad")) \
   \
  X(int, proxBlock, "MMX_PROX_BLOCK", nullptr, knobs_detail::one_of3(env_int("MMX_PROX_BLOCK", 0), 64, 128, 256, kProxBlock)) \
   \
  X(int, gradCache, "MMX_GRAD_CACHE", nullptr, env_int("MMX_GRAD_CACHE", 1)) \
   \
  X(int, forceTie, "MMX_FORCE_TIE", nullptr, env_int("MMX_FORCE_TIE", 0)) \
   \
  X(int, monHint, "MMX_MON_HINT", nullptr, knobs_detail::in_range_or(env_int("MMX_MON_HINT", 1), 0, 3, 1)) \
   \
  X(int, iso, "MMX_ISO", nullptr, env_flag("MMX_ISO", true)) \
   \
  X(int, redSplitMin, "MMX_RED_SPLIT_MIN", nullptr, env_int("MMX_RED_SPLIT_MIN", kRedSplitMin)) \
   \
  X(int, regridGatherAll, "MMX_REGRID_GATHER", "near|all", env_word("MMX_REGRID_GATHER", "near|all")) \
   \
  X(double, regridMargin, "MMX_REGRID_MARGIN", nullptr, env_double("MMX_REGRID_MARGIN", 1.0)) \
   \
  X(int, fdjFast, "MMX_FDJ_FAST", nullptr, env_flag("MMX_FDJ_FAST", true)) \
   \
  X(int, jacAssembleEntry, "MMX_JAC_ASSEMBLE", "auto|entry", env_word("MMX_JAC_ASSEMBLE", "auto|entry")) \
   \
  X(int, schedProf, "MMX_SCHED_PROF", nullptr, env_set("MMX_SCHED_PROF"))

#define MMX_CHAIN_KNOBS(X) \
   \
  X(int, importLat, "MMX_CHAIN_LAT", nullptr, env_int("MMX_CHAIN_LAT", kChainImportLat, 0)) \
   \
  X(int, e48, "MMX_CHAIN_E48", nullptr, env_flag("MMX_CHAIN_E48", true)) \
   \
  X(int, pair, "MMX_CHAIN_PAIR", nullptr, env_flag("MMX_CHAIN_PAIR", true)) \
   \
  X(int, align, "MMX_CHAIN_ALIGN", nullptr, env_int("MMX_CHAIN_ALIGN", -1)) \
   \
  X(int, facR, "MMX_FAC_R", nullptr, env_int("MMX_FAC_R", kFacRMax)) \
   \
  X(int, facRI, "MMX_FAC_RI", nullptr, env_int("MMX_FAC_RI", kFacImpRows, 1, kFacImpRows)) \
   \
  X(int, schedProf, "MMX_SCHED_PROF", nullptr, env_set("MMX_SCHED_PROF"))

#define MMX_MATRIX_KNOBS(X) \
   \
  X(int, spmv, "MMX_SPMV", nullptr, env_int("MMX_SPMV", 2) == 1 ? 1 : 2) \
   \
  X(int, spin, "MMX_SPIN", nullptr, env_flag("MMX_SPIN", true)) \
   \
  X(int, sweepLevel, "MMX_SWEEP", "chain|level", env_word("MMX_SWEEP", "chain|level")) \
   \
   \
  X(int, factor, "MMX_FACTOR", "auto|level|global|wave", env_word("MMX_FACTOR", "auto|level|global|wave")) \
   \
   \
  X(int, factorGran, "MMX_FACTOR_GRAN", nullptr, env_int("MMX_FACTOR_GRAN", 0) == 1) \
   \
  X(int, chainProf, "MMX_CHAIN_PROF", nullptr, env_int("MMX_CHAIN_PROF", 0)) \
   \
  X(int, chainTrim, "MMX_CHAIN_TRIM", nullptr, env_flag("MMX_CHAIN_TRIM", true)) \
   \
  X(int, bwdGran, "MMX_BWD_GRAN", nullptr, env_flag("MMX_BWD_GRAN", true)) \
   \
  X(int, cgsUnfuse, "MMX_CGS_UNFUSE", nullptr, env_flag("MMX_CGS_UNFUSE", true)) \
   \
  X(int, sweepGrid, "MMX_SWEEP_GRID", nullptr, env_int("MMX_SWEEP_GRID", 0) > 0 ? env_int("MMX_SWEEP_GRID", 0) : kSweepGrid) \
   \
  X(int, facWg, "MMX_FAC_WG", nullptr, env_int("MMX_FAC_WG", 4) == 8 ? 8 : 4) \
   \
  X(int, facChunk, "MMX_FAC_CHUNK", nullptr, env_int("MMX_FAC_CHUNK", kFacWaveChunk, 0))

#define MMX_KNOB_FIELD(type, member, name, words, parse) type member;
#define MMX_KNOB_PARSE(type, member, name, words, parse) k.member = (parse);
#define MMX_KNOB_PUT(type, member, name, words, parse) knobs_detail::put(s, name, words, member);

struct EngineKnobs {
  MMX_ENGINE_KNOBS(MMX_KNOB_FIELD)

  static EngineKnobs from_env(int D, int nF, int nranks) {
    EngineKnobs k{};
    MMX_ENGINE_KNOBS(MMX_KNOB_PARSE)
    return k;
  }
  std::string text() const {
    std::string s;
    MMX_ENGINE_KNOBS(MMX_KNOB_PUT)
    return s;
  }
  int xup_sweep_max(size_t maxBlocks) const { return (int)(maxBlocks / 256 / (overlap ? 2 : 1)); }
  void check_xup_sweep(size_t maxBlocks) const {
    if (xupSweep > xup_sweep_max(maxBlocks))
      throw std::invalid_argument("MMX_XUP_SWEEP=" + std::to_string(xupSweep) + " is above " +
                                  std::to_string(xup_sweep_max(maxBlocks)) +
                                  ", what this mesh's partial-sum buffer holds");
  }
};

struct ChainKnobs {
  MMX_CHAIN_KNOBS(MMX_KNOB_FIELD)

  static ChainKnobs from_env() {
    ChainKnobs k{};
    MMX_CHAIN_KNOBS(MMX_KNOB_PARSE)
    return k;
  }
  std::string text() const {
    std::string s;
    MMX_CHAIN_KNOBS(MMX_KNOB_PUT)
    return s;
  }
};

struct MatrixKnobs {
  MMX_MATRIX_KNOBS(MMX_KNOB_FIELD)
  ChainKnobs sched;

  static MatrixKnobs from_env() {
    MatrixKnobs k{};
    MMX_MATRIX_KNOBS(MMX_KNOB_PARSE)
    k.sched = ChainKnobs::from_env();
    return k;
  }
  std::string text() const {
    std::string s;
    MMX_MATRIX_KNOBS(MMX_KNOB_PUT)
    return s + sched.text();
  }
};

}
```

### mm-admm_amd/csrc/kernels/regrid_kernels.h

```cpp
#pragma once
#include <hip/hip_runtime.h>
#include <stddef.h>

namespace mmx {

struct CellGrid {
  double lo[3];
  double inv[3];
  int n[3];
  double hmin;
};

struct GridBox {
  int lo[3];
  int hi[3];
};

template <int D>
void launch_bbox(const double* X, int n, double* partials, int nblocks, hipStream_t st);
template <int D>
void launch_extent(const double* X, const int* F, int nF, double* partials, int nblocks, hipStream_t st);
template <int D>
void launch_bin(const double* X, int n, const CellGrid& cg, int* cellOfV, int* counts, int* starts, int* fill,
                int* cellNodes, void* scanTmp, size_t scanTmpBytes, hipStream_t st);
size_t bin_scan_bytes(int ncell);
template <int D>
void launch_monitor_tv(const double* X, int n, const double* c, double* monVals, hipStream_t st);
struct NnCand {
  const int* gid;
  double slo[3], shi[3];
  int* fail;
};
template <int D>
void launch_nn_fill(const double* X, const CellGrid& cg, const int* starts, const int* cellNodes, const double* gx,
                    const double* gy, const double* gz, int nx, int ny, int nz, const double* monVals, double* vals,
                    const GridBox& box, hipStream_t st, const NnCand& cand = NnCand{nullptr, {0, 0, 0}, {0, 0, 0}, nullptr});
template <int D>
void launch_select_owned(const double* X, const int* ownLocal, const int* ownGid, int nOwned, int nranks, int rank,
                         const double* sboxes, int* counts, double* send, int cap, hipStream_t st);
template <int D>
void launch_build_cand(const double* X, const int* gidLocal, int nLocal, const double* recv, int nRecv, double* cx,
                       int* cgid, hipStream_t st);
template <int D>
void launch_smooth(const double* in, double* out, int nx, int ny, int nz, const GridBox& box, hipStream_t st);
template <int D>
void launch_box_commit(const double* src, double* vals, double* pad, int nx, int ny, int nz, const GridBox& box,
                       hipStream_t st);

void launch_rows_gather(int D, const int* idx, int n, const double* in, double* out, hipStream_t st);
void launch_rows_scatter(int D, const int* idx, int n, const double* in, double* out, hipStream_t st);

}
```

### mm-admm_amd/csrc/kernels/regrid_kernels.hip

```cpp
#include <hip/hip_runtime.h>

#include <hipcub/hipcub.hpp>

#include "regrid_kernels.h"

namespace mmx {
namespace {

constexpr int kRB = 256;

template <int D>
__global__ void __launch_bounds__(kRB) k_bbox(const double* __restrict__ X, int n, double* __restrict__ part) {
  __shared__ double sm[2 * D][kRB];
  double lo[D], hi[D];
#pragma unroll
  for (int d = 0; d < D; ++d) {
    lo[d] = INFINITY;
    hi[d] = -INFINITY;
  }
  for (int v = blockIdx.x * kRB + threadIdx.x; v < n; v += gridDim.x * kRB)
#pragma unroll
    for (int d = 0; d < D; ++d) {
      const double x = X[(size_t)v * D + d];
      lo[d] = x < lo[d] ? x : lo[d];
      hi[d] = x > hi[d] ? x : hi[d];
    }
#pragma unroll
  for (int d = 0; d < D; ++d) {
    sm[d][threadIdx.x] = lo[d];
    sm[D + d][threadIdx.x] = hi[d];
  }
  __syncthreads();
  for (int w = kRB / 2; w > 0; w >>= 1) {
    if ((int)threadIdx.x < w)
#pragma unroll
      for (int d = 0; d < D; ++d) {
        const double a = sm[d][threadIdx.x + w], b = sm[D + d][threadIdx.x + w];
        sm[d][threadIdx.x] = a < sm[d][threadIdx.x] ? a : sm[d][threadIdx.x];
        sm[D + d][threadIdx.x] = b > sm[D + d][threadIdx.x] ? b : sm[D + d][threadIdx.x];
      }
    __syncthreads();
  }
  if (threadIdx.x < 2 * D) part[(size_t)blockIdx.x * 2 * D + threadIdx.x] = sm[threadIdx.x][0];
}

template <int D>
__global__ void __launch_bounds__(kRB) k_extent(const double* __restrict__ X, const int* __restrict__ F, int nF,
                                                double* __restrict__ part) {
  __shared__ double sm[D][kRB];
  double ext[D];
#pragma unroll
  for (int d = 0; d < D; ++d) ext[d] = 0.0;
  for (int s = blockIdx.x * kRB + threadIdx.x; s < nF; s += gridDim.x * kRB) {
    int v[D + 1];
#pragma unroll
    for (int n = 0; n <= D; ++n) v[n] = F[(size_t)s * (D + 1) + n];
#pragma unroll
    for (int d = 0; d < D; ++d) {
      double a = X[(size_t)v[0] * D + d], b = a;
#pragma unroll
      for (int n = 1; n <= D; ++n) {
        const double c = X[(size_t)v[n] * D + d];
        a = c < a ? c : a;
        b = c > b ? c : b;
      }
      const double e = b - a;
      ext[d] = e > ext[d] ? e : ext[d];
    }
  }
#pragma unroll
  for (int d = 0; d < D; ++d) sm[d][threadIdx.x] = ext[d];
  __syncthreads();
  for (int w = kRB / 2; w > 0; w >>= 1) {
    if ((int)threadIdx.x < w)
#pragma unroll
      for (int d = 0; d < D; ++d) {
        const double a = sm[d][threadIdx.x + w];
        sm[d][threadIdx.x] = a > sm[d][threadIdx.x] ? a : sm[d][threadIdx.x];
      }
    __syncthreads();
  }
  if (threadIdx.x < D) part[(size_t)blockIdx.x * D + threadIdx.x] = sm[threadIdx.x][0];
}

template <int D>
__device__ __forceinline__ int cellOf(const double* x, const CellGrid& cg, int (&c)[3]) {
  int id = 0;
#pragma unroll
  for (int d = D - 1; d >= 0; --d) {
    int k = (int)((x[d] - cg.lo[d]) * cg.inv[d]);
    k = k < 0 ? 0 : (k >= cg.n[d] ? cg.n[d] - 1 : k);
    c[d] = k;
    id = id * cg.n[d] + k;
  }
  return id;
}

template <int D>
__global__ void __launch_bounds__(kRB) k_bin_count(const double* __restrict__ X, int n, CellGrid cg,
                                                   int* __restrict__ cellOfV, int* __restrict__ counts) {
  const int v = blockIdx.x * kRB + threadIdx.x;
  if (v >= n) return;
  double x[D];
#pragma unroll
  for (int d = 0; d < D; ++d) x[d] = X[(size_t)v * D + d];
  int c[3];
  const int id = cellOf<D>(x, cg, c);
  cellOfV[v] = id;
  atomicAdd(&counts[id], 1);
}

__global__ void __launch_bounds__(kRB) k_bin_fill(int n, const int* __restrict__ cellOfV,
                                                  const int* __restrict__ starts, int* __restrict__ fill,
                                                  int* __restrict__ cellNodes) {
  const int v = blockIdx.x * kRB + threadIdx.x;
  if (v >= n) return;
  const int c = cellOfV[v];
  cellNodes[starts[c] + atomicAdd(&fill[c], 1)] = v;
}

template <int D>
__global__ void __launch_bounds__(kRB) k_monitor_tv(const double* __restrict__ X, int n, double c0, double c1,
                                                    double c2, double* __restrict__ monVals) {
  const int v = blockIdx.x * kRB + threadIdx.x;
  if (v >= n) return;
  const double c[3] = {c0, c1, c2};
  double sq = 0.0;
#pragma unroll
  for (int d = 0; d < D; ++d) {
    const double t = X[(size_t)v * D + d] - c[d];
    sq = (d == 0) ? t * t : sq + t * t;
  }
  const double s = 1 + 5.0 / (1 + 50.0 * sq);
#pragma unroll
  for (int i = 0; i < D * D; ++i) monVals[(size_t)v * D * D + i] = (i / D == i % D) ? s : 0.0;
}

__device__ __forceinline__ size_t box_row(const GridBox& b, long long p, int nx, int ny, int& sx, int& sy, int& sk) {
  const long long bx = b.hi[0] - b.lo[0] + 1, by = b.hi[1] - b.lo[1] + 1;
  sx = b.lo[0] + (int)(p % bx);
  sy = b.lo[1] + (int)((p / bx) % by);
  sk = b.lo[2] + (int)(p / (bx * by));
  return ((size_t)sk * (ny + 1) + sy) * (nx + 1) + sx;
}
__device__ __forceinline__ long long box_rows(const GridBox& b) {
  return (long long)(b.hi[0] - b.lo[0] + 1) * (b.hi[1] - b.lo[1] + 1) * (b.hi[2] - b.lo[2] + 1);
}

template <int D>
__global__ void __launch_bounds__(kRB) k_nn_fill(const double* __restrict__ X, CellGrid cg,
                                                 const int* __restrict__ starts, const int* __restrict__ cellNodes,
                                                 const double* __restrict__ gx, const double* __restrict__ gy,
                                                 const double* __restrict__ gz, int nx, int ny, int nz,
                                                 const double* __restrict__ monVals, double* __restrict__ vals,
                                                 GridBox box, NnCand cand) {
  constexpr int DD = D * D;
  const long long p = (long long)blockIdx.x * kRB + threadIdx.x;
  if (p >= box_rows(box)) return;
  int sx, sy, k;
  const size_t row = box_row(box, p, nx, ny, sx, sy, k);
  const int i = (D == 2) ? sx : sy, j = (D == 2) ? sy : sx;
  double q[3] = {gx[i], gy[j], D == 3 ? gz[k] : 0.0};
  int c[3] = {0, 0, 0};
  cellOf<D>(q, cg, c);
  double best = INFINITY;
  int bi = -1, bg = -1;
  int rmax = 0;
#pragma unroll
  for (int d = 0; d < D; ++d) rmax = max(rmax, max(c[d], cg.n[d] - 1 - c[d]));
  for (int r = 0; r <= rmax; ++r) {
    const int z0 = (D == 3) ? max(c[2] - r, 0) : 0, z1 = (D == 3) ? min(c[2] + r, cg.n[2] - 1) : 0;
    const int y0 = max(c[1] - r, 0), y1 = min(c[1] + r, cg.n[1] - 1);
    const int x0 = max(c[0] - r, 0), x1 = min(c[0] + r, cg.n[0] - 1);
    for (int cz = z0; cz <= z1; ++cz)
      for (int cy = y0; cy <= y1; ++cy)
        for (int cx = x0; cx <= x1; ++cx) {
          const int dz = (D == 3) ? abs(cz - c[2]) : 0;
          if (max(max(abs(cx - c[0]), abs(cy - c[1])), dz) != r) continue;
          const int cell = (cz * cg.n[1] + cy) * cg.n[0] + cx;
          for (int t = starts[cell]; t < starts[cell + 1]; ++t) {
            const int v = cellNodes[t];
            const int gv = cand.gid ? cand.gid[v] : v;
            double dd = 0.0;
#pragma unroll
            for (int d = 0; d < D; ++d) {
              const double df = q[d] - X[(size_t)v * D + d];
              dd += df * df;
            }
            if (dd < best || (dd == best && gv < bg)) {
              best = dd;
              bi = v;
              bg = gv;
            }
          }
        }
    const double lb = ((double)r - 1e-6) * cg.hmin;
    if (bi >= 0 && r > 0 && best < lb * lb) break;
  }
  if (cand.gid) {
    double gap = INFINITY;
#pragma unroll
    for (int d = 0; d < D; ++d) gap = fmin(gap, fmin(q[d] - cand.slo[d], cand.shi[d] - q[d]));
    if (!(bi >= 0 && gap > 0.0 && best < gap * gap * (1.0 - 1e-9))) {
      atomicOr(cand.fail, 1);
      if (bi < 0) return;
    }
  }
#pragma unroll
  for (int e = 0; e < DD; ++e) vals[row * DD + e] = monVals[(size_t)bi * DD + e];
}

template <int D>
__global__ void __launch_bounds__(kRB) k_select_owned(const double* __restrict__ X, const int* __restrict__ ownLocal,
                                                      const int* __restrict__ ownGid, int nOwned, int nranks, int rank,
                                                      const double* __restrict__ sboxes, int* __restrict__ counts,
                                                      double* __restrict__ send, int cap) {
  const int i = blockIdx.x * kRB + threadIdx.x;
  if (i >= nOwned) return;
  const int v = ownLocal[i];
  double x[D];
#pragma unroll
  for (int d = 0; d < D; ++d) x[d] = X[(size_t)v * D + d];
  for (int q = 0; q < nranks; ++q) {
    if (q == rank) continue;
    const double* s = sboxes + (size_t)q * 2 * D;
    bool in = true;
#pragma unroll
    for (int d = 0; d < D; ++d) in = in && x[d] >= s[d] && x[d] <= s[D + d];
    if (in) {
      const int k = atomicAdd(&counts[q], 1);
      double* r = send + ((size_t)q * cap + k) * (D + 1);
#pragma unroll
      for (int d = 0; d < D; ++d) r[d] = x[d];
      r[D] = (double)ownGid[i];
    }
  }
}

template <int D>
__global__ void __launch_bounds__(kRB) k_build_cand(const double* __restrict__ X, const int* __restrict__ gidLocal,
                                                    int nLocal, const double* __restrict__ recv, int nRecv,
                                                    double* __restrict__ cx, int* __restrict__ cgid) {
  const int i = blockIdx.x * kRB + threadIdx.x;
  if (i >= nLocal + nRecv) return;
  if (i < nLocal) {
#pragma unroll
    for (int d = 0; d < D; ++d) cx[(size_t)i * D + d] = X[(size_t)i * D + d];
    cgid[i] = gidLocal[i];
  } else {
    const double* r = recv + (size_t)(i - nLocal) * (D + 1);
#pragma unroll
    for (int d = 0; d < D; ++d) cx[(size_t)i * D + d] = r[d];
    cgid[i] = (int)r[D];
  }
}

template <int D>
__global__ void __launch_bounds__(kRB) k_smooth(const double* __restrict__ in, double* __restrict__ out, int nx,
                                                int ny, int nz, GridBox box) {
  constexpr int DD = D * D;
  const long long p = (long long)blockIdx.x * kRB + threadIdx.x;
  const long long P = (long long)(nx + 1) * (ny + 1);
  if (p >= box_rows(box)) return;
  int i, j, k;
  const long long c = (long long)box_row(box, p, nx, ny, i, j, k);
  const bool interior = i >= 1 && i < nx && j >= 1 && j < ny && (D == 2 || (k >= 1 && k < nz));
  for (int q = 0; q < DD; ++q) {
    double v;
    if (!interior) {
      v = in[c * DD + q];
    } else if constexpr (D == 2) {
      v = 0.6 * in[c * DD + q];
      v += 0.1 * in[(c + 1) * DD + q];
      v += 0.1 * in[(c - 1) * DD + q];
      v += 0.1 * in[(c + nx + 1) * DD + q];
      v += 0.1 * in[(c - nx - 1) * DD + q];
    } else {
      const double h = 0.4 / 6.0;
      v = 0.6 * in[c * DD + q] + h * in[(c + 1) * DD + q] + h * in[(c - 1) * DD + q] + h * in[(c + nx + 1) * DD + q] +
          h * in[(c - nx - 1) * DD + q] + h * in[(c + P) * DD + q] + h * in[(c - P) * DD + q];
    }
    out[c * DD + q] = v;
  }
}

template <int D>
__global__ void __launch_bounds__(kRB) k_box_commit(const double* __restrict__ src, double* __restrict__ vals,
                                                    double* __restrict__ pad, int nx, int ny, int nz, GridBox box) {
  constexpr int DD = D * D;
  const long long c = (long long)blockIdx.x * kRB + threadIdx.x;
  const long long P = (long long)(nx + 1) * (ny + 1);
  if (c >= P * (D == 3 ? nz + 1 : 1)) return;
  const int i = (int)(c % (nx + 1)), j = (int)((c / (nx + 1)) % (ny + 1)), k = (D == 3) ? (int)(c / P) : 0;
  const bool in = i >= box.lo[0] && i <= box.hi[0] && j >= box.lo[1] && j <= box.hi[1] && k >= box.lo[2] &&
                  k <= box.hi[2];
  const double nan = __builtin_nan("");
  for (int q = 0; q < DD; ++q) vals[c * DD + q] = in ? src[c * DD + q] : nan;
  if (D == 3 && pad) {
    for (int q = 0; q < DD; ++q) pad[c * 10 + q] = in ? src[c * DD + q] : nan;
    pad[c * 10 + 9] = 0.0;
  }
}

__global__ void __launch_bounds__(kRB) k_rows_gather(int D, const int* __restrict__ idx, int n,
                                                     const double* __restrict__ in, double* __restrict__ out) {
  const int i = blockIdx.x * kRB + threadIdx.x;
  if (i >= n) return;
  for (int c = 0; c < D; ++c) out[(size_t)i * D + c] = in[(size_t)idx[i] * D + c];
}
__global__ void __launch_bounds__(kRB) k_rows_scatter(int D, const int* __restrict__ idx, int n,
                                                      const double* __restrict__ in, double* __restrict__ out) {
  const int i = blockIdx.x * kRB + threadIdx.x;
  if (i >= n || idx[i] < 0) return;
  for (int c = 0; c < D; ++c) out[(size_t)idx[i] * D + c] = in[(size_t)i * D + c];
}

inline unsigned blocks(long long n) { return (unsigned)((n + kRB - 1) / kRB); }

}

template <int D>
void launch_bbox(const double* X, int n, double* partials, int nblocks, hipStream_t st) {
  hipLaunchKernelGGL(k_bbox<D>, dim3(nblocks), dim3(kRB), 0, st, X, n, partials);
}

template <int D>
void launch_extent(const double* X, const int* F, int nF, double* partials, int nblocks, hipStream_t st) {
  hipLaunchKernelGGL(k_extent<D>, dim3(nblocks), dim3(kRB), 0, st, X, F, nF, partials);
}

template <int D>
void launch_bin(const double* X, int n, const CellGrid& cg, int* cellOfV, int* counts, int* starts, int* fill,
                int* cellNodes, void* scanTmp, size_t scanTmpBytes, hipStream_t st) {
  const int ncell = cg.n[0] * cg.n[1] * cg.n[2];
  (void)hipMemsetAsync(counts, 0, sizeof(int) * (ncell + 1), st);
  (void)hipMemsetAsync(fill, 0, sizeof(int) * ncell, st);
  hipLaunchKernelGGL(k_bin_count<D>, dim3(blocks(n)), dim3(kRB), 0, st, X, n, cg, cellOfV, counts);
  size_t bytes = scanTmpBytes;
  (void)hipcub::DeviceScan::ExclusiveSum(scanTmp, bytes, counts, starts, ncell + 1, st);
  hipLaunchKernelGGL(k_bin_fill, dim3(blocks(n)), dim3(kRB), 0, st, n, cellOfV, starts, fill, cellNodes);
}

size_t bin_scan_bytes(int ncell) {
  size_t bytes = 0;
  (void)hipcub::DeviceScan::ExclusiveSum(nullptr, bytes, (int*)nullptr, (int*)nullptr, ncell + 1, (hipStream_t)0);
  return bytes;
}

template <int D>
void launch_monitor_tv(const double* X, int n, const double* c, double* monVals, hipStream_t st) {
  hipLaunchKernelGGL(k_monitor_tv<D>, dim3(blocks(n)), dim3(kRB), 0, st, X, n, c[0], c[1], c[2], monVals);
}

static long long host_box_rows(const GridBox& b) {
  return (long long)(b.hi[0] - b.lo[0] + 1) * (b.hi[1] - b.lo[1] + 1) * (b.hi[2] - b.lo[2] + 1);
}

template <int D>
void launch_nn_fill(const double* X, const CellGrid& cg, const int* starts, const int* cellNodes, const double* gx,
                    const double* gy, const double* gz, int nx, int ny, int nz, const double* monVals, double* vals,
                    const GridBox& box, hipStream_t st, const NnCand& cand) {
  const long long n = host_box_rows(box);
  if (n > 0)
    hipLaunchKernelGGL(k_nn_fill<D>, dim3(blocks(n)), dim3(kRB), 0, st, X, cg, starts, cellNodes, gx, gy, gz, nx, ny,
                       nz, monVals, vals, box, cand);
}

template <int D>
void launch_select_owned(const double* X, const int* ownLocal, const int* ownGid, int nOwned, int nranks, int rank,
                         const double* sboxes, int* counts, double* send, int cap, hipStream_t st) {
  if (nOwned > 0)
    hipLaunchKernelGGL(k_select_owned<D>, dim3(blocks(nOwned)), dim3(kRB), 0, st, X, ownLocal, ownGid, nOwned, nranks,
                       rank, sboxes, counts, send, cap);
}

template <int D>
void launch_build_cand(const double* X, const int* gidLocal, int nLocal, const double* recv, int nRecv, double* cx,
                       int* cgid, hipStream_t st) {
  if (nLocal + nRecv > 0)
    hipLaunchKernelGGL(k_build_cand<D>, dim3(blocks(nLocal + nRecv)), dim3(kRB), 0, st, X, gidLocal, nLocal, recv,
                       nRecv, cx, cgid);
}

template <int D>
void launch_smooth(const double* in, double* out, int nx, int ny, int nz, const GridBox& box, hipStream_t st) {
  const long long n = host_box_rows(box);
  if (n > 0) hipLaunchKernelGGL(k_smooth<D>, dim3(blocks(n)), dim3(kRB), 0, st, in, out, nx, ny, nz, box);
}

template <int D>
void launch_box_commit(const double* src, double* vals, double* pad, int nx, int ny, int nz, const GridBox& box,
                       hipStream_t st) {
  const long long rows = (long long)(nx + 1) * (ny + 1) * (D == 3 ? nz + 1 : 1);
  hipLaunchKernelGGL(k_box_commit<D>, dim3(blocks(rows)), dim3(kRB), 0, st, src, vals, pad, nx, ny, nz, box);
}

void launch_rows_gather(int D, const int* idx, int n, const double* in, double* out, hipStream_t st) {
  if (n > 0) hipLaunchKernelGGL(k_rows_gather, dim3(blocks(n)), dim3(kRB), 0, st, D, idx, n, in, out);
}
void launch_rows_scatter(int D, const int* idx, int n, const double* in, double* out, hipStream_t st) {
  if (n > 0) hipLaunchKernelGGL(k_rows_scatter, dim3(blocks(n)), dim3(kRB), 0, st, D, idx, n, in, out);
}

#define MMX_REGRID_INST(D)                                                                                       \
  template void launch_bbox<D>(const double*, int, double*, int, hipStream_t);                                 \
  template void launch_extent<D>(const double*, const int*, int, double*, int, hipStream_t);                    \
  template void launch_bin<D>(const double*, int, const CellGrid&, int*, int*, int*, int*, int*, void*, size_t, \
                              hipStream_t);                                                                    \
  template void launch_monitor_tv<D>(const double*, int, const double*, double*, hipStream_t);                  \
  template void launch_nn_fill<D>(const double*, const CellGrid&, const int*, const int*, const double*,        \
                                  const double*, const double*, int, int, int, const double*, double*,          \
                                  const GridBox&, hipStream_t, const NnCand&);                                 \
  template void launch_select_owned<D>(const double*, const int*, const int*, int, int, int, const double*, int*, \
                                       double*, int, hipStream_t);                                               \
  template void launch_build_cand<D>(const double*, const int*, int, const double*, int, double*, int*,          \
                                     hipStream_t);                                                               \
  template void launch_smooth<D>(const double*, double*, int, int, int, const GridBox&, hipStream_t);           \
  template void launch_box_commit<D>(const double*, double*, double*, int, int, int, const GridBox&, hipStream_t);
MMX_REGRID_INST(2)
MMX_REGRID_INST(3)
#undef MMX_REGRID_INST

}
```

### mm-admm_amd/python/mmadmm_amd.py

```python
import ctypes
import os
import time

import numpy as np

_HERE = os.path.dirname(os.path.abspath(__file__))
LIB_PATH = os.environ.get("MMADMM_LIB", os.path.join(os.path.dirname(_HERE), "lib", "libmmadmm.so"))

MMADMM_OK = 0
BOUNDARY_FREE, BOUNDARY_FIXED, INTERIOR = 0, 1, 2

c_double_p = ctypes.POINTER(ctypes.c_double)
c_int_p = ctypes.POINTER(ctypes.c_int32)
MONITOR_FN = ctypes.CFUNCTYPE(None, ctypes.c_int, c_double_p, c_double_p, ctypes.c_void_p)
c_ll_p = ctypes.POINTER(ctypes.c_longlong)
ALLGATHER_FN = ctypes.CFUNCTYPE(ctypes.c_int, ctypes.c_void_p, c_double_p, c_double_p, ctypes.c_longlong)
EXCHANGE_FN = ctypes.CFUNCTYPE(ctypes.c_int, ctypes.c_void_p, ctypes.c_int, c_int_p, c_double_p, c_ll_p, c_ll_p,
                               c_double_p, c_ll_p, c_ll_p)


class mmadmm_params(ctypes.Structure):
    _fields_ = [("dt", ctypes.c_double), ("tau", ctypes.c_double), ("rho", ctypes.c_double),
                ("grad_use", ctypes.c_int), ("device", ctypes.c_int), ("rank", ctypes.c_int),
                ("nranks", ctypes.c_int), ("partition", ctypes.c_int)]


PARTITION = {"rcb": 0, "ranges": 1}


class mmadmm_stats(ctypes.Structure):
    _fields_ = [("steps", ctypes.c_longlong), ("admm_iters", ctypes.c_longlong),
                ("bfgs_iters", ctypes.c_longlong), ("max_bfgs", ctypes.c_int),
                ("last_primal", ctypes.c_double), ("last_dual", ctypes.c_double),
                ("t_prox_ms", ctypes.c_double), ("t_xupdate_ms", ctypes.c_double),
                ("t_step_ms", ctypes.c_double), ("n_prox", ctypes.c_longlong),
                ("n_xupdate", ctypes.c_longlong), ("n_steps_timed", ctypes.c_longlong),
                ("prox_bytes", ctypes.c_double), ("xupdate_bytes", ctypes.c_double),
                ("newton_iters", ctypes.c_longlong), ("jacobians", ctypes.c_longlong),
                ("cg_iters", ctypes.c_longlong), ("t_jac_ms", ctypes.c_double), ("t_solve_ms", ctypes.c_double),
                ("t_be_ms", ctypes.c_double), ("regrids", ctypes.c_longlong), ("regrid_rows", ctypes.c_longlong),
                ("regrid_gather_bytes", ctypes.c_double), ("regrid_cand", ctypes.c_longlong),
                ("regrid_fallbacks", ctypes.c_longlong), ("monitor_iso", ctypes.c_int),
                ("t_exchange_ms", ctypes.c_double), ("n_exchange", ctypes.c_longlong),
                ("halo_send_bytes", ctypes.c_double), ("halo_recv_bytes", ctypes.c_double),
                ("interior_nodes", ctypes.c_int), ("overlap", ctypes.c_int)]

    def as_dict(self):
        return {k: getattr(self, k) for k, _ in self._fields_}


class MMADMMError(RuntimeError):
    def __init__(self, code, msg):
        super().__init__(f"mmadmm error {code}: {msg}")
        self.code = code


class InvertedElementError(MMADMMError):
    """The reference aborts on assert(Edet > 0) (src/AdaptationFunctional.cpp:174)."""


class NonFiniteEnergyError(MMADMMError):
    """MMADMM_ERR_NONFINITE: a NaN energy with no inverted element -- a monitor value that is not
    finite (on an element partition with a time-varying monitor: an evaluation outside the rank's
    rebuilt grid box)."""


_lib = None


def lib():
    global _lib
    if _lib is not None:
        return _lib
    if not os.path.exists(LIB_PATH):
        raise ImportError(f"libmmadmm.so not built ({LIB_PATH}); run `make -C mm-admm_amd`")
    L = ctypes.CDLL(LIB_PATH)
    L.mmadmm_last_error.restype = ctypes.c_char_p
    L.mmadmm_builtin_monitor.argtypes = [ctypes.c_int, ctypes.c_int, ctypes.POINTER(MONITOR_FN),
                                         ctypes.POINTER(ctypes.c_void_p)]
    L.mmadmm_create.argtypes = [ctypes.c_int, ctypes.c_int, c_double_p, c_double_p, ctypes.c_int, c_int_p,
                                c_int_p, ctypes.POINTER(mmadmm_params), MONITOR_FN, ctypes.c_void_p,
                                ctypes.POINTER(ctypes.c_void_p)]
    L.mmadmm_step.argtypes = [ctypes.c_void_p, ctypes.c_int, ctypes.c_double, c_double_p,
                              ctypes.POINTER(ctypes.c_int)]
    L.mmadmm_euler_step.argtypes = [ctypes.c_void_p, c_double_p]
    L.mmadmm_energy.argtypes = [ctypes.c_void_p, c_double_p]
    L.mmadmm_backward_euler_step.argtypes = [ctypes.c_void_p, ctypes.c_double, ctypes.c_double, c_double_p,
                                             ctypes.POINTER(ctypes.c_int)]
    L.mmadmm_get_jacobian.argtypes = [ctypes.c_void_p, ctypes.POINTER(ctypes.c_longlong), c_int_p, c_int_p,
                                      c_double_p]
    L.mmadmm_done.argtypes = [ctypes.c_void_p]
    L.mmadmm_get.argtypes = [ctypes.c_void_p, ctypes.c_char_p, c_double_p]
    L.mmadmm_get_simplices.argtypes = [ctypes.c_void_p, c_int_p]
    L.mmadmm_sizes.argtypes = [ctypes.c_void_p] + [ctypes.POINTER(ctypes.c_int)] * 3
    L.mmadmm_set_timing.argtypes = [ctypes.c_void_p, ctypes.c_int]
    L.mmadmm_stats_get.argtypes = [ctypes.c_void_p, ctypes.POINTER(mmadmm_stats)]
    L.mmadmm_stats_reset.argtypes = [ctypes.c_void_p]
    L.mmadmm_options_get.argtypes = [ctypes.c_void_p, ctypes.c_char_p, ctypes.c_int]
    L.mmadmm_sync.argtypes = [ctypes.c_void_p]
    L.mmadmm_regrid.argtypes = [ctypes.c_void_p, ctypes.c_double]
    L.mmadmm_set_regrid.argtypes = [ctypes.c_void_p, ctypes.c_int]
    L.mmadmm_regrid_values.argtypes = [ctypes.c_void_p, c_double_p]
    L.mmadmm_regrid_values_device.argtypes = [ctypes.c_void_p, ctypes.c_void_p, ctypes.c_void_p]
    L.mmadmm_regrid_field.argtypes = [ctypes.c_void_p, c_double_p, ctypes.c_double]
    L.mmadmm_regrid_field_device.argtypes = [ctypes.c_void_p, ctypes.c_void_p, ctypes.c_double, ctypes.c_void_p]
    L.mmadmm_field_hessian.argtypes = [ctypes.c_void_p, c_double_p, c_double_p]
    L.mmadmm_field_hessian_device.argtypes = [ctypes.c_void_p, ctypes.c_void_p, ctypes.c_void_p, ctypes.c_void_p]
    L.mmadmm_get_device.argtypes = [ctypes.c_void_p, ctypes.c_char_p, ctypes.c_void_p, ctypes.c_void_p]
    L.mmadmm_field_monitor.argtypes = [ctypes.c_int, ctypes.c_int, c_double_p, ctypes.c_int, c_int_p, c_double_p,
                                       ctypes.c_double, c_double_p, c_double_p]
    L.mmadmm_transfer.argtypes = [ctypes.c_void_p, c_double_p, c_double_p, ctypes.c_int, c_double_p, c_double_p,
                                  c_int_p, c_int_p]
    L.mmadmm_transfer_device.argtypes = [ctypes.c_void_p, ctypes.c_void_p, ctypes.c_void_p, ctypes.c_int,
                                         ctypes.c_void_p, ctypes.c_void_p, ctypes.c_void_p, c_int_p, ctypes.c_void_p]
    L.mmadmm_transfer_field.argtypes = [ctypes.c_int, ctypes.c_int, c_double_p, ctypes.c_int, c_int_p, c_double_p,
                                        ctypes.c_int, c_double_p, c_double_p, c_int_p, c_int_p]
    L.mmadmm_face_neighbours.argtypes = [ctypes.c_int, ctypes.c_int, ctypes.c_int, c_int_p, c_int_p]
    L.mmadmm_destroy.argtypes = [ctypes.c_void_p]
    L.mmadmm_mesh_rect.argtypes = [ctypes.c_int] * 4 + [ctypes.c_double] * 6 + [ctypes.c_int,
                                                                                 ctypes.POINTER(ctypes.c_void_p)]
    L.mmadmm_mesh_levelset2d.argtypes = [ctypes.c_int] * 2 + [ctypes.c_double] * 4 + [
        ctypes.c_int, ctypes.c_int, ctypes.POINTER(ctypes.c_void_p)]
    L.mmadmm_mesh_levelset3d.argtypes = [ctypes.c_int] * 3 + [ctypes.c_double] * 6 + [
        ctypes.c_int, ctypes.c_int, ctypes.POINTER(ctypes.c_void_p)]
    L.mmadmm_mesh_hexdisc.argtypes = [ctypes.c_int] + [ctypes.c_double] * 3 + [ctypes.c_int,
                                                                               ctypes.POINTER(ctypes.c_void_p)]
    L.mmadmm_mesh_shoulder.argtypes = [ctypes.c_int] * 4 + [ctypes.c_double] * 6 + [ctypes.c_int,
                                                                                     ctypes.POINTER(ctypes.c_void_p)]
    L.mmadmm_mesh_reference_points.argtypes = [ctypes.c_void_p, c_double_p]
    L.mmadmm_mesh_read.argtypes = [ctypes.c_int, ctypes.c_char_p, ctypes.c_char_p, ctypes.c_char_p,
                                   ctypes.POINTER(ctypes.c_void_p)]
    L.mmadmm_mesh_sizes.argtypes = [ctypes.c_void_p] + [ctypes.POINTER(ctypes.c_int)] * 4
    L.mmadmm_mesh_copy.argtypes = [ctypes.c_void_p, c_double_p, c_int_p, c_int_p]
    L.mmadmm_mesh_free.argtypes = [ctypes.c_void_p]
    L.mmadmm_write_points.argtypes = [ctypes.c_char_p, ctypes.c_int, ctypes.c_int, c_double_p]
    L.mmadmm_write_simplices.argtypes = [ctypes.c_char_p, ctypes.c_int, ctypes.c_int, c_int_p]
    L.mmadmm_debug_blockgrad.argtypes = [ctypes.c_void_p, ctypes.c_int, c_double_p, c_double_p, ctypes.c_int,
                                         c_double_p]
    L.mmadmm_devmath.argtypes = [ctypes.c_int, ctypes.c_int, c_double_p, c_double_p]
    vp = ctypes.c_void_p
    L.mmadmm_comm_unique_id.argtypes = [vp, ctypes.c_int]
    L.mmadmm_comm_create_rccl.argtypes = [ctypes.c_int, ctypes.c_int, vp, ctypes.c_int, ctypes.POINTER(vp)]
    L.mmadmm_comm_create_rccl_timeout.argtypes = [ctypes.c_int, ctypes.c_int, vp, ctypes.c_int, ctypes.c_double,
                                                  ctypes.POINTER(vp)]
    L.mmadmm_comm_create_loopback.argtypes = [ctypes.c_int, ctypes.POINTER(vp)]
    L.mmadmm_comm_destroy.argtypes = [vp]
    L.mmadmm_comm_nranks.argtypes = [vp, ctypes.POINTER(ctypes.c_int)]
    L.mmadmm_build_info.argtypes = [ctypes.c_char_p, ctypes.c_int]
    L.mmadmm_comm_create_host.argtypes = [ctypes.c_int, ctypes.c_int, ALLGATHER_FN, EXCHANGE_FN, vp, ctypes.POINTER(vp)]
    L.mmadmm_be_begin.argtypes = [vp, ctypes.c_double, c_double_p]
    L.mmadmm_be_residual.argtypes = [vp, ctypes.c_double, c_double_p, c_double_p, c_double_p]
    L.mmadmm_be_fsubjac.argtypes = [vp, c_double_p]
    L.mmadmm_be_add.argtypes = [vp, c_double_p]
    L.mmadmm_create_partitioned.argtypes = [ctypes.c_int, ctypes.c_int, c_double_p, c_double_p, ctypes.c_int, c_int_p,
                                            c_int_p, ctypes.POINTER(mmadmm_params), MONITOR_FN, vp, vp,
                                            ctypes.POINTER(vp)]
    L.mmadmm_local_nodes.argtypes = [vp, ctypes.POINTER(ctypes.c_int), c_int_p]
    L.mmadmm_plan_create.argtypes = [ctypes.c_int, ctypes.c_int, c_double_p, ctypes.c_int, c_int_p, ctypes.c_int,
                                     ctypes.c_int, ctypes.c_int, ctypes.POINTER(vp)]
    L.mmadmm_plan_sizes.argtypes = [vp] + [ctypes.POINTER(ctypes.c_int)] * 7
    L.mmadmm_plan_get.argtypes = [vp] + [c_int_p] * 6
    L.mmadmm_plan_destroy.argtypes = [vp]
    _lib = L
    return L


def build_info():
    buf = ctypes.create_string_buffer(256)
    _check(lib().mmadmm_build_info(buf, 256))
    return dict(kv.split("=", 1) for kv in buf.value.decode().split())


def _close_at_exit(obj):
    try:
        obj.close()
    except (TypeError, AttributeError, NameError):
        pass


def _check(rc):
    if rc != MMADMM_OK:
        msg = lib().mmadmm_last_error().decode(errors="replace")
        if rc == 3:
            raise InvertedElementError(rc, msg)
        if rc == 7:
            raise NonFiniteEnergyError(rc, msg)
        raise MMADMMError(rc, msg)


def _options(fn, h):
    need = fn(h, None, 0)
    _check(-need if need < 0 else MMADMM_OK)
    buf = ctypes.create_string_buffer(need)
    fn(h, buf, need)
    return dict(line.split("=", 1) for line in buf.value.decode().splitlines())


def _dp(a):
    return a.ctypes.data_as(c_double_p)


def _ip(a):
    return a.ctypes.data_as(c_int_p)


def field_monitor(Xp, F, u, alpha=None, hessian=True, monitor=True):
    Xp = np.ascontiguousarray(Xp, dtype=np.float64)
    F = np.ascontiguousarray(F, dtype=np.int32)
    u = np.ascontiguousarray(u, dtype=np.float64).reshape(-1)
    nP, D = Xp.shape
    if u.shape[0] != nP or F.ndim != 2 or F.shape[1] != D + 1:
        raise ValueError("field_monitor: Xp nP x D, F nF x (D + 1), u nP values")
    H = np.zeros((nP, D, D)) if hessian else None
    M = np.zeros((nP, D, D)) if (monitor and alpha is not None) else None
    _check(lib().mmadmm_field_monitor(D, nP, _dp(Xp), F.shape[0], _ip(F), _dp(u),
                                      float(alpha) if alpha is not None else 1.0,
                                      _dp(H) if H is not None else None, _dp(M) if M is not None else None))
    return H, M


TRANSFER_COUNTS = ("copied", "patch", "walked", "outside")


def _field_2d(u, nP, who):
    u = np.ascontiguousarray(u, dtype=np.float64)
    if u.ndim not in (1, 2) or u.shape[0] != nP or u.size == 0:
        raise ValueError(f"{who}: u must be nP or nP x C values (C >= 1), nP = {nP}")
    return u.reshape(nP, -1)


def transfer_field(Xold, F, Xnew, u, where=True):
    Xold = np.ascontiguousarray(Xold, dtype=np.float64)
    Xnew = np.ascontiguousarray(Xnew, dtype=np.float64)
    F = np.ascontiguousarray(F, dtype=np.int32)
    if Xold.ndim != 2 or Xnew.shape != Xold.shape or F.ndim != 2 or F.shape[1] != Xold.shape[1] + 1:
        raise ValueError("transfer_field: Xold, Xnew nP x D, F nF x (D + 1)")
    nP, D = Xold.shape
    shape = np.shape(u)
    u2 = _field_2d(u, nP, "transfer_field")
    out = np.zeros_like(u2)
    w = np.zeros(nP, dtype=np.int32) if where else None
    cnt = np.zeros(4, dtype=np.int32)
    _check(lib().mmadmm_transfer_field(D, nP, _dp(Xold), F.shape[0], _ip(F), _dp(Xnew), u2.shape[1], _dp(u2), _dp(out),
                                       _ip(w) if where else None, _ip(cnt)))
    info = {k: int(c) for k, c in zip(TRANSFER_COUNTS, cnt)}
    if where:
        info["where"] = w
    return out.reshape(shape), info


def face_neighbours(F, nP=None):
    F = np.ascontiguousarray(F, dtype=np.int32)
    nbr = np.zeros_like(F)
    _check(lib().mmadmm_face_neighbours(F.shape[1] - 1, int(F.max()) + 1 if nP is None else nP, F.shape[0], _ip(F),
                                        _ip(nbr)))
    return nbr


def _is_tensor(a):
    t = type(a)
    return t.__module__.split(".")[0] == "torch" and hasattr(a, "data_ptr")


class MeshData:

    def __init__(self, dim, Xp, F, mask):
        self.dim = dim
        self.Xp = np.ascontiguousarray(Xp, dtype=np.float64)
        self.F = np.ascontiguousarray(F, dtype=np.int32)
        self.mask = np.ascontiguousarray(mask, dtype=np.int32)

    @property
    def nP(self):
        return self.Xp.shape[0]

    @property
    def nF(self):
        return self.F.shape[0]

    @staticmethod
    def _take(h):
        L = lib()
        d, nP, nF, ml = (ctypes.c_int() for _ in range(4))
        _check(L.mmadmm_mesh_sizes(h, ctypes.byref(d), ctypes.byref(nP), ctypes.byref(nF), ctypes.byref(ml)))
        Xp = np.zeros((nP.value, d.value))
        F = np.zeros((nF.value, d.value + 1), dtype=np.int32)
        mask = np.zeros(ml.value, dtype=np.int32)
        _check(L.mmadmm_mesh_copy(h, _dp(Xp), _ip(F), _ip(mask)))
        Xc = np.zeros_like(Xp)
        _check(L.mmadmm_mesh_reference_points(h, _dp(Xc)))
        L.mmadmm_mesh_free(h)
        m = MeshData(d.value, Xp, F, mask)
        m.Xc = Xc
        return m

    @staticmethod
    def shoulder(dim, n, xa=0, xb=1, ya=0, yb=1, za=0, zb=1, btype=BOUNDARY_FIXED):
        h = ctypes.c_void_p()
        _check(lib().mmadmm_mesh_shoulder(dim, n, n, n if dim == 3 else 0, xa, xb, ya, yb, za, zb, btype,
                                          ctypes.byref(h)))
        return MeshData._take(h)

    @staticmethod
    def rect(dim, n, xa=0, xb=1, ya=0, yb=1, za=0, zb=1, btype=BOUNDARY_FIXED):
        h = ctypes.c_void_p()
        _check(lib().mmadmm_mesh_rect(dim, n, n, n if dim == 3 else 0, xa, xb, ya, yb, za, zb, btype,
                                      ctypes.byref(h)))
        return MeshData._take(h)

    @staticmethod
    def levelset2d(n, xa=0.0, xb=1.0, ya=0.0, yb=1.0, btype=BOUNDARY_FIXED, compact_mask=True):
        h = ctypes.c_void_p()
        _check(lib().mmadmm_mesh_levelset2d(n, n, xa, xb, ya, yb, btype, int(compact_mask), ctypes.byref(h)))
        return MeshData._take(h)

    @staticmethod
    def levelset3d(n, xa=0.0, xb=1.0, ya=0.0, yb=1.0, za=0.0, zb=1.0, btype=BOUNDARY_FIXED, compact_mask=True):
        h = ctypes.c_void_p()
        _check(lib().mmadmm_mesh_levelset3d(n, n, n, xa, xb, ya, yb, za, zb, btype, int(compact_mask),
                                            ctypes.byref(h)))
        return MeshData._take(h)

    @staticmethod
    def hexdisc(N, r=0.5, cx=0.5, cy=0.5, btype=BOUNDARY_FIXED):
        h = ctypes.c_void_p()
        _check(lib().mmadmm_mesh_hexdisc(N, r, cx, cy, btype, ctypes.byref(h)))
        return MeshData._take(h)

    @staticmethod
    def read(dim, tri, pnts, mask):
        h = ctypes.c_void_p()
        _check(lib().mmadmm_mesh_read(dim, tri.encode(), pnts.encode(), mask.encode(), ctypes.byref(h)))
        return MeshData._take(h)


def write_points(path, Xp):
    Xp = np.ascontiguousarray(Xp, dtype=np.float64)
    _check(lib().mmadmm_write_points(path.encode(), Xp.shape[1], Xp.shape[0], _dp(Xp)))


def write_simplices(path, F):
    F = np.ascontiguousarray(F, dtype=np.int32)
    _check(lib().mmadmm_write_simplices(path.encode(), F.shape[1] - 1, F.shape[0], _ip(F)))


class MonitorFunction:

    dim = 2

    def __call__(self, x, M):
        raise NotImplementedError

    def _cfunc(self):
        def tramp(dim, xp, Mp, _user):
            x = np.ctypeslib.as_array(xp, shape=(dim,))
            M = np.ctypeslib.as_array(Mp, shape=(dim, dim))
            self(x, M)

        self._keep = MONITOR_FN(tramp)
        return self._keep, None


class BuiltinMonitor(MonitorFunction):

    def __init__(self, dim, mon_type):
        self.dim = dim
        self.mon_type = mon_type

    def _cfunc(self):
        fn = MONITOR_FN()
        user = ctypes.c_void_p()
        _check(lib().mmadmm_builtin_monitor(self.dim, self.mon_type, ctypes.byref(fn), ctypes.byref(user)))
        return fn, user


class Mesh:

    def __init__(self, Xp, F, boundaryMask, Mon, numThreads=1, rho=50.0, w=None, tau=0.5,
                 integrationMode=0, gradUse=False, Xc=None, device=-1):
        self.Xp = np.ascontiguousarray(Xp, dtype=np.float64)
        self.dim = self.Xp.shape[1]
        self.F = np.ascontiguousarray(F, dtype=np.int32)
        self.mask = np.ascontiguousarray(np.asarray(boundaryMask)[: self.Xp.shape[0]], dtype=np.int32)
        self.Mon = Mon
        self.numThreads = numThreads
        self.rho = float(rho)
        self.w = 0.5 * np.sqrt(self.rho)
        self.tau = float(tau)
        self.integrationMode = integrationMode
        self.gradUse = bool(gradUse)
        self.Xc = None if Xc is None else np.ascontiguousarray(Xc, dtype=np.float64)
        self.device = device


UNIQUE_ID_BYTES = 128


class Comm:

    def __init__(self, h):
        self.h = h

    @staticmethod
    def unique_id():
        buf = ctypes.create_string_buffer(UNIQUE_ID_BYTES)
        _check(lib().mmadmm_comm_unique_id(buf, UNIQUE_ID_BYTES))
        return buf.raw

    @staticmethod
    def rccl(nranks, rank, uid, device, timeout_s=None):
        h = ctypes.c_void_p()
        buf = ctypes.create_string_buffer(bytes(uid), UNIQUE_ID_BYTES)
        if timeout_s is None:
            _check(lib().mmadmm_comm_create_rccl(int(nranks), int(rank), buf, int(device), ctypes.byref(h)))
        else:
            _check(lib().mmadmm_comm_create_rccl_timeout(int(nranks), int(rank), buf, int(device),
                                                         ctypes.c_double(float(timeout_s)), ctypes.byref(h)))
        return Comm(h)

    @staticmethod
    def loopback(nranks):
        h = ctypes.c_void_p()
        _check(lib().mmadmm_comm_create_loopback(int(nranks), ctypes.byref(h)))
        return Comm(h)

    @staticmethod
    def host(nranks, rank, transport):

        def ag(_user, send, recv, count):
            try:
                n = int(count)
                s = np.ctypeslib.as_array(send, shape=(max(n, 1),))[:n]
                r = np.ctypeslib.as_array(recv, shape=(max(n * nranks, 1),))[: n * nranks]
                transport.allgather(s, r)
                return 0
            except BaseException:
                import traceback
                traceback.print_exc()
                _abort(transport)
                return 1

        def ex(_user, npeers, peer, send, so, sc, recv, ro, rc):
# ... 101 lines not shown
        _check(L.mmadmm_plan_get(h, *[_ip(out[k]) for k in ("localNodes", "localSimplices", "incPtr", "incSrc",
                                                             "sendOff", "peers")]))
        out.update(recvRows=nrecv, interfaceNodes=nif)
        return out
    finally:
        L.mmadmm_plan_destroy(h)


class Engine:

    def __init__(self, mesh, dt, rank=0, nranks=1, comm=None, partition="rcb"):
        L = lib()
        p = mmadmm_params(dt=float(dt), tau=mesh.tau, rho=mesh.rho, grad_use=int(mesh.gradUse),
                          device=mesh.device, rank=int(rank), nranks=int(nranks), partition=PARTITION[partition])
        fn, user = mesh.Mon._cfunc()
        self._fn = fn
        h = ctypes.c_void_p()
        Xc = _dp(mesh.Xc) if mesh.Xc is not None else None
        if nranks == 1 and comm is None:
            _check(L.mmadmm_create(mesh.dim, mesh.Xp.shape[0], _dp(mesh.Xp), Xc, mesh.F.shape[0], _ip(mesh.F),
                                   _ip(mesh.mask), ctypes.byref(p), fn, user, ctypes.byref(h)))
        else:
            _check(L.mmadmm_create_partitioned(mesh.dim, mesh.Xp.shape[0], _dp(mesh.Xp), Xc, mesh.F.shape[0],
                                               _ip(mesh.F), _ip(mesh.mask), ctypes.byref(p), fn, user,
                                               comm.h if comm is not None else None, ctypes.byref(h)))
        self.h = h
        self.comm = comm
        self.dim = mesh.dim
        nP, nF, gr = ctypes.c_int(), ctypes.c_int(), ctypes.c_int()
        _check(L.mmadmm_sizes(h, ctypes.byref(nP), ctypes.byref(nF), ctypes.byref(gr)))
        self.nP, self.nF, self.gridRows = nP.value, nF.value, gr.value
        self.K = self.dim * (self.dim + 1)
        self.device = mesh.device
        self._side = None

    def local_nodes(self):
        ids = np.zeros(self.nP, dtype=np.int32)
        _check(lib().mmadmm_local_nodes(self.h, None, _ip(ids)))
        return ids

    def close(self):
        if getattr(self, "h", None):
            lib().mmadmm_destroy(self.h)
            self.h = None

    def __del__(self):
        try:
            _close_at_exit(self)
        except TypeError:
            pass

    def step(self, nIters, tol=1e-3):
        Ih = ctypes.c_double()
        it = ctypes.c_int()
        _check(lib().mmadmm_step(self.h, nIters, tol, ctypes.byref(Ih), ctypes.byref(it)))
        return Ih.value, it.value

    def euler_step(self):
        Ih = ctypes.c_double()
        _check(lib().mmadmm_euler_step(self.h, ctypes.byref(Ih)))
        return Ih.value

    def backwards_euler_step(self, dt, tol=1e-3):
        Ih = ctypes.c_double()
        it = ctypes.c_int()
        _check(lib().mmadmm_backward_euler_step(self.h, dt, tol, ctypes.byref(Ih), ctypes.byref(it)))
        return Ih.value, it.value

    def jacobian(self):
        nnz = ctypes.c_longlong()
        _check(lib().mmadmm_get_jacobian(self.h, ctypes.byref(nnz), None, None, None))
        ia = np.zeros(self.nP * self.dim + 1, dtype=np.int32)
        ja = np.zeros(nnz.value, dtype=np.int32)
        a = np.zeros(nnz.value)
        _check(lib().mmadmm_get_jacobian(self.h, None, _ip(ia), _ip(ja), _dp(a)))
        return ia, ja, a

    def energy(self):
        E = ctypes.c_double()
        _check(lib().mmadmm_energy(self.h, ctypes.byref(E)))
        return E.value

    def done(self):
        _check(lib().mmadmm_done(self.h))

    def get(self, what):
        n = {"x": self.nP * self.dim, "xPrev": self.nP * self.dim, "xBar": self.nP * self.dim,
             "points": self.nP * self.dim, "z": self.nF * self.K, "u": self.nF * self.K,
             "hess": self.nF * self.K * self.K, "gs": self.nF * self.K, "grid": self.gridRows * self.dim * self.dim,
             "Ehat": self.dim * self.dim}[what]
        out = np.zeros(n)
        _check(lib().mmadmm_get(self.h, what.encode(), _dp(out)))
        return out

    def simplices(self):
        F = np.zeros((self.nF, self.dim + 1), dtype=np.int32)
        _check(lib().mmadmm_get_simplices(self.h, _ip(F)))
        return F

    def set_timing(self, on):
        _check(lib().mmadmm_set_timing(self.h, int(on)))

    def stats(self):
        s = mmadmm_stats()
        _check(lib().mmadmm_stats_get(self.h, ctypes.byref(s)))
        return s.as_dict()

    def reset_stats(self):
        _check(lib().mmadmm_stats_reset(self.h))

    def options(self):
        return _options(lib().mmadmm_options_get, self.h)

    def sync(self):
        _check(lib().mmadmm_sync(self.h))

    def regrid(self, t):
        _check(lib().mmadmm_regrid(self.h, t))

    def set_regrid(self, every_step=True):
        _check(lib().mmadmm_set_regrid(self.h, 1 if every_step else 0))

    def _device_arg(self, a, n, who):
        import torch

        if a.dtype != torch.float64 or not a.is_cuda or not a.is_contiguous() or a.numel() != n:
            raise ValueError(f"{who}: a torch tensor must be float64, contiguous, on the GPU, with {n} values "
                             f"(got {a.dtype}, {a.device}, {a.numel()} values)")
        if self.device is not None and self.device >= 0 and a.device.index != self.device:
            raise ValueError(f"{who}: tensor on {a.device}, the engine on device {self.device}")
        cur = torch.cuda.current_stream(a.device)
        if cur.cuda_stream != 0:
            return a.data_ptr(), cur.cuda_stream, None
        if self._side is None:
            self._side = torch.cuda.Stream(a.device)
        self._side.wait_stream(cur)
        a.record_stream(self._side)
        return a.data_ptr(), self._side.cuda_stream, (cur, self._side)

    @staticmethod
    def _rejoin(j):
        if j is not None:
            j[0].wait_stream(j[1])

    def regrid_values(self, M):
        n = self.nP * self.dim * self.dim
        if _is_tensor(M):
            p, st, j = self._device_arg(M, n, "regrid_values")
            _check(lib().mmadmm_regrid_values_device(self.h, p, st))
            self._rejoin(j)
            return
        M = np.ascontiguousarray(M, dtype=np.float64)
        if M.size != n:
            raise ValueError(f"regrid_values: M must hold {n} values")
        _check(lib().mmadmm_regrid_values(self.h, _dp(M)))

    def field_hessian(self, u):
        if _is_tensor(u):
            import torch

            p, st, j = self._device_arg(u, self.nP, "field_hessian")
            H = torch.empty((self.nP, self.dim, self.dim), dtype=torch.float64, device=u.device)
            if j is not None:
                H.record_stream(j[1])
            _check(lib().mmadmm_field_hessian_device(self.h, p, H.data_ptr(), st))
            self._rejoin(j)
            return H
        u = np.ascontiguousarray(u, dtype=np.float64).reshape(-1)
        if u.size != self.nP:
            raise ValueError(f"field_hessian: u must hold {self.nP} values")
        H = np.zeros((self.nP, self.dim, self.dim))
        _check(lib().mmadmm_field_hessian(self.h, _dp(u), _dp(H)))
        return H

    def regrid_field(self, u, alpha=None):
        if alpha is None:
            H = self.field_hessian(u)
            if _is_tensor(H):
                alpha = float((H * H).sum(dim=(1, 2)).sqrt().mean())
            else:
                alpha = float(np.sqrt((H * H).sum(axis=(1, 2))).mean())
            if alpha == 0.0:
                alpha = 1.0
        alpha = float(alpha)
        if _is_tensor(u):
            p, st, j = self._device_arg(u, self.nP, "regrid_field")
            _check(lib().mmadmm_regrid_field_device(self.h, p, alpha, st))
            self._rejoin(j)
            return alpha
        u = np.ascontiguousarray(u, dtype=np.float64).reshape(-1)
        if u.size != self.nP:
            raise ValueError(f"regrid_field: u must hold {self.nP} values")
        _check(lib().mmadmm_regrid_field(self.h, _dp(u), alpha))
        return alpha

    def transfer(self, u, X_old, X_new=None, where=False):
        nx = self.nP * self.dim
        cnt = np.zeros(4, dtype=np.int32)
        if _is_tensor(u):
            import torch

            if u.dim() not in (1, 2) or u.shape[0] != self.nP or u.numel() == 0:
                raise ValueError(f"transfer: u must be nP or nP x C values (C >= 1), nP = {self.nP}")
            C = u.numel() // self.nP
            if not _is_tensor(X_old) or not (X_new is None or _is_tensor(X_new)):
                raise ValueError("transfer: u, X_old and X_new must all be tensors or all be arrays")
            pu, st, j = self._device_arg(u, self.nP * C, "transfer")
            po, st, j = self._device_arg(X_old, nx, "transfer")
            pn = None
            if X_new is not None:
                pn, st, j = self._device_arg(X_new, nx, "transfer")
            out = torch.empty_like(u)
            w = torch.empty(self.nP, dtype=torch.int32, device=u.device) if where else None
            if j is not None:
                out.record_stream(j[1])
                if where:
                    w.record_stream(j[1])
            _check(lib().mmadmm_transfer_device(self.h, po, pn, C, pu, out.data_ptr(), w.data_ptr() if where else None,
                                                _ip(cnt), st))
            self._rejoin(j)
        else:
            if _is_tensor(X_old) or _is_tensor(X_new):
                raise ValueError("transfer: u, X_old and X_new must all be tensors or all be arrays")
            shape = np.shape(u)
            u2 = _field_2d(u, self.nP, "transfer")
            X_old = np.ascontiguousarray(X_old, dtype=np.float64)
            if X_new is not None:
                X_new = np.ascontiguousarray(X_new, dtype=np.float64)
            if X_old.size != nx or (X_new is not None and X_new.size != nx):
                raise ValueError(f"transfer: positions must hold {nx} values")
            out2 = np.zeros_like(u2)
            w = np.zeros(self.nP, dtype=np.int32) if where else None
            _check(lib().mmadmm_transfer(self.h, _dp(X_old), _dp(X_new) if X_new is not None else None, u2.shape[1],
                                         _dp(u2), _dp(out2), _ip(w) if where else None, _ip(cnt)))
            out = out2.reshape(shape)
        info = {k: int(c) for k, c in zip(TRANSFER_COUNTS, cnt)}
        if where:
            info["where"] = w
        return out, info

    def get_tensor(self, what):
        import torch

        if what not in ("points", "x"):
            raise ValueError("get_tensor: 'points' or 'x'")
        dev = torch.device("cuda", self.device if self.device is not None and self.device >= 0
                           else torch.cuda.current_device())
        out = torch.empty((self.nP, self.dim), dtype=torch.float64, device=dev)
        p, st, j = self._device_arg(out, self.nP * self.dim, "get_tensor")
        _check(lib().mmadmm_get_device(self.h, what.encode(), p, st))
        self._rejoin(j)
        return out

    def block_grad(self, sid, z, dxpu=None, computeGrad=True, regularize=False):
        z = np.ascontiguousarray(z, dtype=np.float64)
        dx = np.ascontiguousarray(dxpu if dxpu is not None else z, dtype=np.float64)
        out = np.zeros(self.K + 2)
        _check(lib().mmadmm_debug_blockgrad(self.h, sid, _dp(z), _dp(dx),
                                            int(computeGrad) | (2 * int(regularize)), _dp(out)))
        return out[0], out[2:], out[1]


class MeshIntegrator:

    def __init__(self, dt, a):
        self.a = a
        self.dt = float(dt)
        self.engine = Engine(a, dt)
        self.proxTime = 0.0
        self.predTime = 0.0
        self.stepsTaken = 0

    def step(self, nIters, tol):
        t0 = time.perf_counter()
        Ih, _ = self.engine.step(nIters, tol)
        self.proxTime += time.perf_counter() - t0
        self.stepsTaken += 1
        return Ih

    def eulerStep(self, tol=1e-3):
        return self.engine.euler_step()

    def backwardsEulerStep(self, dt, tol):
        return self.engine.backwards_euler_step(dt, tol)[0]

    def getEnergy(self):
        return self.engine.energy()

    def done(self):
        self.engine.done()

    def outputX(self, fname):
        write_points(fname, self.engine.get("x").reshape(-1, self.a.dim))

    def outputZ(self, fname):
        write_points(fname, self.engine.get("z").reshape(-1, self.a.dim))


def devmath(op, x):
    x = np.ascontiguousarray(x, dtype=np.float64)
    out = np.zeros_like(x)
    _check(lib().mmadmm_devmath(op, x.size, _dp(x), _dp(out)))
    return out
```

Before: 2656.

## Rework regrid nearest-neighbour fill and smoothing kernels with fused pad and run-based grids

Replaces the regrid nearest-neighbour fill with a new kernel that uses a super-cell scratch buffer. Smoothing and box-commit now launch over contiguous x-runs, and the final smoothing pass writes the 3D pad rows directly. In the non-partitioned case, the fill now lands in the values array when the pass count is even, which removes the device-to-device copy and the separate pad kernel. The old kernels stay available behind an environment knob, and debug entry points were added to compare the two paths.

```diff
diff --git a/include/mmadmm.h b/include/mmadmm.h
--- a/include/mmadmm.h
+++ b/include/mmadmm.h
@@ -144,6 +144,12 @@
 int mmadmm_debug_blockgrad(mmadmm_handle h, int s, const double* z, const double* dxpu, int flags,
                            double* out);
 
+int mmadmm_debug_smooth(int dim, int nx, int ny, int nz, const double* in, const int* box, int passes, int part,
+                        double* vals, double* pad);
+int mmadmm_debug_nn_fill(int dim, int nV, const double* X, const int32_t* gid, const double* sbox,
+                         const int32_t* ncell, int nx, int ny, int nz, const double* gx, const double* gy,
+                         const double* gz, const double* mon, const int* box, double* vals, int* fail);
+
 #define MMADMM_PART_RCB 0
 #define MMADMM_PART_RANGES 1
 #define MMADMM_UNIQUE_ID_BYTES 128
diff --git a/mm-admm_amd/csrc/host/engine.cpp b/mm-admm_amd/csrc/host/engine.cpp
--- a/mm-admm_amd/csrc/host/engine.cpp
+++ b/mm-admm_amd/csrc/host/engine.cpp
@@ -692,7 +692,7 @@
     s->overlap = knobs_.overlap;
   }
 
-  std::string options() const override { return knobs_.text(); }
+  std::string options() const override { return knobs_.text() + knobs_.regrid.text(); }
 
   void resetStats() override {
     resolveTimed();
@@ -1159,7 +1159,7 @@
     }
     NnCand nc{rgnCandGid_.p, {clo[0], clo[1], clo[2]}, {chi[0], chi[1], chi[2]}, rgnCnt_.p + nranks_};
     launch_nn_fill<D>(rgnCandX_.p, cg, rgStarts_.p, rgnNodes_.p, gx_.p, gy_.p, D == 3 ? gz_.p : gy_.p, grid_.nx,
-                      grid_.ny, grid_.nz, rgnMon_.p, rgTmp_.p, H, st_, nc);
+                      grid_.ny, grid_.nz, rgnMon_.p, rgTmp_.p, H, nnScratch(), st_, nc);
     int fail = 0;
     MMX_HIP(hipMemcpyAsync(&fail, rgnCnt_.p + nranks_, sizeof(int), hipMemcpyDeviceToHost, st_));
     streamWait();
@@ -1242,7 +1242,9 @@
       rgScanBytes_ = bin_scan_bytes(ncell);
       rgScan_.alloc(std::max<size_t>(rgScanBytes_, 1));
     }
-  }
+    if (rgSup_.n < nn_super_cells(cg)) rgSup_.alloc(nn_super_cells(cg));
+  }
+  int* nnScratch() const { return knobs_.regrid.parentKernels ? nullptr : rgSup_.p; }
   static int smoothPasses() { return (D == 2) ? 5 : 2; }
   GridBox rowBox(const double* llo, const double* lhi, int* marg) const {
     const int gn3[3] = {grid_.nx, grid_.ny, D == 3 ? grid_.nz : 0};
@@ -1287,19 +1289,11 @@
     }
   }
   void smoothCommit(const GridBox& R, int passes, bool part) {
-    double* cur = rgTmp_.p;
-    double* oth = part ? rgTmp2_.p : gvals_.p;
-    for (int it = 0; it < passes; ++it) {
-      launch_smooth<D>(cur, oth, grid_.nx, grid_.ny, grid_.nz, widenBox(R, part ? passes - 1 - it : 0), st_);
-      std::swap(cur, oth);
-    }
-    if (part) {
-      launch_box_commit<D>(cur, gvals_.p, D == 3 ? gpad_.p : nullptr, grid_.nx, grid_.ny, grid_.nz, R, st_);
-    } else {
-      if (cur != gvals_.p)
-        MMX_HIP(hipMemcpyAsync(gvals_.p, cur, gvals_.n * sizeof(double), hipMemcpyDeviceToDevice, st_));
-      if (D == 3) launch_pad_rows(gvals_.p, (long long)(gvals_.n / 9), gpad_.p, st_);
-    }
+    launch_smooth_commit<D>(rgTmp_.p, rgTmp2_.p, gvals_.p, D == 3 ? gpad_.p : nullptr, grid_.nx, grid_.ny, grid_.nz, R,
+                            passes, part, knobs_.regrid.parentKernels != 0, st_);
+  }
+  double* fillDst(int passes, bool part) const {
+    return smooth_fill_in_vals(passes, part, knobs_.regrid.parentKernels != 0) ? gvals_.p : rgTmp_.p;
   }
 
   void regridAll(double t, MonSource src = kMonCallback) {
@@ -1372,14 +1366,7 @@
       if (d < D && ext > 0) cg.hmin = std::min(cg.hmin, ext / cg.n[d]);
     }
     if (!(cg.hmin < INFINITY)) cg.hmin = 0.0;
-    const int ncell = cg.n[0] * cg.n[1] * cg.n[2];
-    if ((int)rgStarts_.n < ncell + 1) {
-      rgCounts_.alloc(ncell + 1);
-      rgStarts_.alloc(ncell + 1);
-      rgFill_.alloc(ncell);
-      rgScanBytes_ = bin_scan_bytes(ncell);
-      rgScan_.alloc(std::max<size_t>(rgScanBytes_, 1));
-    }
+    ensureCells(cg);
     launch_bin<D>(X, nG, cg, rgCellOf_.p, rgCounts_.p, rgStarts_.p, rgFill_.p, rgNodes_.p, rgScan_.p, rgScanBytes_,
                   st_);
     if (src == kMonCallback && builtin_monitor_kind(monFn_, monUser_) == 7) src = kMonBuiltin7;
@@ -1428,20 +1415,8 @@
     };
     const GridBox H = widen(R, part ? passes : 0);
     launch_nn_fill<D>(X, cg, rgStarts_.p, rgNodes_.p, gx_.p, gy_.p, D == 3 ? gz_.p : gy_.p, grid_.nx, grid_.ny,
-                      grid_.nz, rgMon_.p, rgTmp_.p, H, st_);
-    double* cur = rgTmp_.p;
-    double* oth = part ? rgTmp2_.p : gvals_.p;
-    for (int it = 0; it < passes; ++it) {
-      launch_smooth<D>(cur, oth, grid_.nx, grid_.ny, grid_.nz, widen(R, part ? passes - 1 - it : 0), st_);
-      std::swap(cur, oth);
-    }
-    if (part) {
-      launch_box_commit<D>(cur, gvals_.p, D == 3 ? gpad_.p : nullptr, grid_.nx, grid_.ny, grid_.nz, R, st_);
-    } else {
-      if (cur != gvals_.p)
-        MMX_HIP(hipMemcpyAsync(gvals_.p, cur, gvals_.n * sizeof(double), hipMemcpyDeviceToDevice, st_));
-      if (D == 3) launch_pad_rows(gvals_.p, (long long)(gvals_.n / 9), gpad_.p, st_);
-    }
+                      grid_.nz, rgMon_.p, fillDst(passes, part), H, nnScratch(), st_);
+    smoothCommit(R, passes, part);
     st_stats_.regrid_rows = (long long)(H.hi[0] - H.lo[0] + 1) * (H.hi[1] - H.lo[1] + 1) * (H.hi[2] - H.lo[2] + 1);
     st_stats_.regrid_gather_bytes = part ? (double)nranks_ * maxOwned_ * D * sizeof(double) : 0.0;
     st_stats_.regrid_cand = part ? nG : 0;
@@ -1599,7 +1574,7 @@
   DevBuf<int> rgnCnt_, rgnGid_, rgnOwnGid_, rgnCandGid_, rgnCellOf_, rgnNodes_;
   double* rgnHost_ = nullptr;
   int nOwned_ = 0, maxOwned_ = 1;
-  DevBuf<int> rgCellOf_, rgNodes_, rgCounts_, rgStarts_, rgFill_;
+  DevBuf<int> rgCellOf_, rgNodes_, rgCounts_, rgStarts_, rgFill_, rgSup_;
   DevBuf<unsigned char> rgScan_;
   size_t rgScanBytes_ = 0;
   double* rgHost_ = nullptr;
diff --git a/mm-admm_amd/csrc/host/knobs.h b/mm-admm_amd/csrc/host/knobs.h
--- a/mm-admm_amd/csrc/host/knobs.h
+++ b/mm-admm_amd/csrc/host/knobs.h
@@ -137,6 +137,11 @@
    \
   X(int, schedProf, "MMX_SCHED_PROF", nullptr, env_set("MMX_SCHED_PROF"))
 
+#define MMX_REGRID_KNOBS(X) \
+   \
+   \
+  X(int, parentKernels, "MMX_REGRID_KERNELS", "new|parent", env_word("MMX_REGRID_KERNELS", "new|parent"))
+
 #define MMX_CHAIN_KNOBS(X) \
    \
   X(int, importLat, "MMX_CHAIN_LAT", nullptr, env_int("MMX_CHAIN_LAT", kChainImportLat, 0)) \
@@ -185,12 +190,29 @@
 #define MMX_KNOB_PARSE(type, member, name, words, parse) k.member = (parse);
 #define MMX_KNOB_PUT(type, member, name, words, parse) knobs_detail::put(s, name, words, member);
 
+struct RegridKnobs {
+  MMX_REGRID_KNOBS(MMX_KNOB_FIELD)
+
+  static RegridKnobs from_env() {
+    RegridKnobs k{};
+    MMX_REGRID_KNOBS(MMX_KNOB_PARSE)
+    return k;
+  }
+  std::string text() const {
+    std::string s;
+    MMX_REGRID_KNOBS(MMX_KNOB_PUT)
+    return s;
+  }
+};
+
 struct EngineKnobs {
   MMX_ENGINE_KNOBS(MMX_KNOB_FIELD)
+  RegridKnobs regrid;
 
   static EngineKnobs from_env(int D, int nF, int nranks) {
     EngineKnobs k{};
     MMX_ENGINE_KNOBS(MMX_KNOB_PARSE)
+    k.regrid = RegridKnobs::from_env();
     return k;
   }
   std::string text() const {
diff --git a/mm-admm_amd/csrc/host/regrid_debug.cpp b/mm-admm_amd/csrc/host/regrid_debug.cpp
--- /dev/null
+++ b/mm-admm_amd/csrc/host/regrid_debug.cpp
@@ -0,0 +1,142 @@
+#include <algorithm>
+#include <cmath>
+#include <cstring>
+#include <limits>
+#include <vector>
+
+#include "../kernels/regrid_kernels.h"
+#include "common.h"
+#include "knobs.h"
+
+namespace mmx {
+namespace {
+
+GridBox checked_box(const char* who, int dim, int nx, int ny, int nz, const int* box) {
+  const int gn[3] = {nx, ny, dim == 3 ? nz : 0};
+  GridBox b{{0, 0, 0}, {0, 0, 0}};
+  for (int d = 0; d < 3; ++d) {
+    b.lo[d] = box[d];
+    b.hi[d] = box[3 + d];
+    if (b.lo[d] < 0 || b.hi[d] > gn[d] || b.lo[d] > b.hi[d])
+      throw Error(MMADMM_ERR_INVALID, std::string(who) + ": box outside the grid");
+  }
+  return b;
+}
+
+template <int D>
+void debug_smooth(int nx, int ny, int nz, const double* in, const int* box, int passes, int part, double* vals,
+                  double* pad) {
+  const GridBox R = checked_box("mmadmm_debug_smooth", D, nx, ny, nz, box);
+  const size_t rows = (size_t)(nx + 1) * (ny + 1) * (D == 3 ? nz + 1 : 1), n = rows * D * D;
+  const bool parent = RegridKnobs::from_env().parentKernels != 0;
+  DevBuf<double> tmp, tmp2, dv, dp;
+  tmp.alloc(n);
+  tmp2.alloc(n);
+  dv.alloc(n);
+  if (D == 3 && pad) dp.alloc(rows * 10);
+  MMX_HIP(hipMemset(tmp.p, 0xFF, n * sizeof(double)));
+  MMX_HIP(hipMemset(tmp2.p, 0xFF, n * sizeof(double)));
+  MMX_HIP(hipMemset(dv.p, 0xFF, n * sizeof(double)));
+  if (dp.p) MMX_HIP(hipMemset(dp.p, 0xFF, rows * 10 * sizeof(double)));
+  double* fill = smooth_fill_in_vals(passes, part != 0, parent) ? dv.p : tmp.p;
+  MMX_HIP(hipMemcpy(fill, in, n * sizeof(double), hipMemcpyHostToDevice));
+  launch_smooth_commit<D>(tmp.p, tmp2.p, dv.p, dp.p, nx, ny, nz, R, passes, part != 0, parent, nullptr);
+  MMX_HIP(hipGetLastError());
+  MMX_HIP(hipDeviceSynchronize());
+  MMX_HIP(hipMemcpy(vals, dv.p, n * sizeof(double), hipMemcpyDeviceToHost));
+  if (dp.p) MMX_HIP(hipMemcpy(pad, dp.p, rows * 10 * sizeof(double), hipMemcpyDeviceToHost));
+}
+
+template <int D>
+void debug_nn_fill(int nV, const double* X, const int* gid, const double* sbox, const int* ncell, int nx, int ny,
+                   int nz, const double* gx, const double* gy, const double* gz, const double* mon, const int* box,
+                   double* vals, int* fail) {
+  constexpr int DD = D * D;
+  const GridBox B = checked_box("mmadmm_debug_nn_fill", D, nx, ny, nz, box);
+  const size_t rows = (size_t)(nx + 1) * (ny + 1) * (D == 3 ? nz + 1 : 1);
+  double lo[3] = {INFINITY, INFINITY, INFINITY}, hi[3] = {-INFINITY, -INFINITY, -INFINITY};
+  for (int v = 0; v < nV; ++v)
+    for (int d = 0; d < D; ++d) {
+      lo[d] = std::min(lo[d], X[(size_t)v * D + d]);
+      hi[d] = std::max(hi[d], X[(size_t)v * D + d]);
+    }
+  CellGrid cg{};
+  cg.hmin = INFINITY;
+  for (int d = 0; d < 3; ++d) {
+    const double ext = d < D ? hi[d] - lo[d] : 0.0;
+    if (d < D && (ncell[d] < 1 || ncell[d] > 4096)) throw Error(MMADMM_ERR_INVALID, "mmadmm_debug_nn_fill: bad ncell");
+    cg.lo[d] = d < D ? lo[d] : 0.0;
+    cg.n[d] = (d < D && ext > 0) ? ncell[d] : 1;
+    cg.inv[d] = (d < D && ext > 0) ? cg.n[d] / ext : 0.0;
+    if (d < D && ext > 0) cg.hmin = std::min(cg.hmin, ext / cg.n[d]);
+  }
+  if (!(cg.hmin < INFINITY)) cg.hmin = 0.0;
+  const size_t nc = (size_t)cg.n[0] * cg.n[1] * cg.n[2];
+  const bool parent = RegridKnobs::from_env().parentKernels != 0;
+  DevBuf<double> dX, dgx, dgy, dgz, dmon, dvals;
+  DevBuf<int> dgid, cellOf, counts, starts, fillc, nodes, sup, dfail;
+  DevBuf<unsigned char> scan;
+  dX.upload(X, (size_t)nV * D, nullptr);
+  dgx.upload(gx, (D == 3 ? ny : nx) + 1, nullptr);
+  dgy.upload(gy, (D == 3 ? nx : ny) + 1, nullptr);
+  if (D == 3) dgz.upload(gz, nz + 1, nullptr);
+  dmon.upload(mon, (size_t)nV * DD, nullptr);
+  if (gid) dgid.upload(gid, nV, nullptr);
+  dvals.alloc(rows * DD);
+  MMX_HIP(hipMemset(dvals.p, 0xFF, rows * DD * sizeof(double)));
+  dfail.alloc(1);
+  MMX_HIP(hipMemset(dfail.p, 0, sizeof(int)));
+  cellOf.alloc(nV);
+  nodes.alloc(nV);
+  counts.alloc(nc + 1);
+  starts.alloc(nc + 1);
+  fillc.alloc(nc);
+  const size_t scanBytes = bin_scan_bytes((int)nc);
+  scan.alloc(std::max<size_t>(scanBytes, 1));
+  if (!parent) sup.alloc(nn_super_cells(cg));
+  launch_bin<D>(dX.p, nV, cg, cellOf.p, counts.p, starts.p, fillc.p, nodes.p, scan.p, scanBytes, nullptr);
+  NnCand cand{nullptr, {0, 0, 0}, {0, 0, 0}, nullptr};
+  if (gid) {
+    cand.gid = dgid.p;
+    cand.fail = dfail.p;
+    for (int d = 0; d < D; ++d) {
+      cand.slo[d] = sbox[d];
+      cand.shi[d] = sbox[D + d];
+    }
+  }
+  launch_nn_fill<D>(dX.p, cg, starts.p, nodes.p, dgx.p, dgy.p, D == 3 ? dgz.p : dgy.p, nx, ny, nz, dmon.p, dvals.p, B,
+                    sup.p, nullptr, cand);
+  MMX_HIP(hipGetLastError());
+  MMX_HIP(hipDeviceSynchronize());
+  MMX_HIP(hipMemcpy(vals, dvals.p, rows * DD * sizeof(double), hipMemcpyDeviceToHost));
+  MMX_HIP(hipMemcpy(fail, dfail.p, sizeof(int), hipMemcpyDeviceToHost));
+}
+
+}
+}
+
+extern "C" int mmadmm_debug_smooth(int dim, int nx, int ny, int nz, const double* in, const int* box, int passes,
+                                   int part, double* vals, double* pad) {
+  return mmx::guarded([&] {
+    if ((dim != 2 && dim != 3) || nx < 1 || ny < 1 || (dim == 3 && nz < 1) || passes < 0 || !in || !box || !vals)
+      throw mmx::Error(MMADMM_ERR_INVALID, "mmadmm_debug_smooth: bad arguments");
+    if (dim == 2)
+      mmx::debug_smooth<2>(nx, ny, 0, in, box, passes, part, vals, nullptr);
+    else
+      mmx::debug_smooth<3>(nx, ny, nz, in, box, passes, part, vals, pad);
+  });
+}
+
+extern "C" int mmadmm_debug_nn_fill(int dim, int nV, const double* X, const int32_t* gid, const double* sbox,
+                                    const int32_t* ncell, int nx, int ny, int nz, const double* gx, const double* gy,
+                                    const double* gz, const double* mon, const int* box, double* vals, int* fail) {
+  return mmx::guarded([&] {
+    if ((dim != 2 && dim != 3) || nV < 1 || nx < 1 || ny < 1 || (dim == 3 && (nz < 1 || !gz)) || !X || !ncell ||
+        !gx || !gy || !mon || !box || !vals || !fail || (gid && !sbox))
+      throw mmx::Error(MMADMM_ERR_INVALID, "mmadmm_debug_nn_fill: bad arguments");
+    if (dim == 2)
+      mmx::debug_nn_fill<2>(nV, X, gid, sbox, ncell, nx, ny, 0, gx, gy, gz, mon, box, vals, fail);
+    else
+      mmx::debug_nn_fill<3>(nV, X, gid, sbox, ncell, nx, ny, nz, gx, gy, gz, mon, box, vals, fail);
+  });
+}
diff --git a/mm-admm_amd/csrc/kernels/regrid_kernels.h b/mm-admm_amd/csrc/kernels/regrid_kernels.h
--- a/mm-admm_amd/csrc/kernels/regrid_kernels.h
+++ b/mm-admm_amd/csrc/kernels/regrid_kernels.h
@@ -31,10 +31,12 @@
   double slo[3], shi[3];
   int* fail;
 };
+size_t nn_super_cells(const CellGrid& cg);
 template <int D>
 void launch_nn_fill(const double* X, const CellGrid& cg, const int* starts, const int* cellNodes, const double* gx,
                     const double* gy, const double* gz, int nx, int ny, int nz, const double* monVals, double* vals,
-                    const GridBox& box, hipStream_t st, const NnCand& cand = NnCand{nullptr, {0, 0, 0}, {0, 0, 0}, nullptr});
+                    const GridBox& box, int* sup, hipStream_t st,
+                    const NnCand& cand = NnCand{nullptr, {0, 0, 0}, {0, 0, 0}, nullptr});
 template <int D>
 void launch_select_owned(const double* X, const int* ownLocal, const int* ownGid, int nOwned, int nranks, int rank,
                          const double* sboxes, int* counts, double* send, int cap, hipStream_t st);
@@ -42,10 +44,17 @@
 void launch_build_cand(const double* X, const int* gidLocal, int nLocal, const double* recv, int nRecv, double* cx,
                        int* cgid, hipStream_t st);
 template <int D>
-void launch_smooth(const double* in, double* out, int nx, int ny, int nz, const GridBox& box, hipStream_t st);
+void launch_smooth(const double* in, double* out, double* pad, int nx, int ny, int nz, const GridBox& box,
+                   bool parentKernels, hipStream_t st);
 template <int D>
 void launch_box_commit(const double* src, double* vals, double* pad, int nx, int ny, int nz, const GridBox& box,
-                       hipStream_t st);
+                       bool parentKernels, hipStream_t st);
+inline bool smooth_fill_in_vals(int passes, bool part, bool parentKernels) {
+  return !part && !parentKernels && passes % 2 == 0;
+}
+template <int D>
+void launch_smooth_commit(double* tmp, double* tmp2, double* vals, double* pad, int nx, int ny, int nz,
+                          const GridBox& R, int passes, bool part, bool parentKernels, hipStream_t st);
 
 void launch_rows_gather(int D, const int* idx, int n, const double* in, double* out, hipStream_t st);
 void launch_rows_scatter(int D, const int* idx, int n, const double* in, double* out, hipStream_t st);
diff --git a/mm-admm_amd/csrc/kernels/regrid_kernels.hip b/mm-admm_amd/csrc/kernels/regrid_kernels.hip
--- a/mm-admm_amd/csrc/kernels/regrid_kernels.hip
+++ b/mm-admm_amd/csrc/kernels/regrid_kernels.hip
@@ -1,7 +1,10 @@
 #include <hip/hip_runtime.h>
 
+#include <algorithm>
+
 #include <hipcub/hipcub.hpp>
 
+#include "admm_kernels.h"
 #include "regrid_kernels.h"
 
 namespace mmx {
@@ -148,12 +151,12 @@
 }
 
 template <int D>
-__global__ void __launch_bounds__(kRB) k_nn_fill(const double* __restrict__ X, CellGrid cg,
-                                                 const int* __restrict__ starts, const int* __restrict__ cellNodes,
-                                                 const double* __restrict__ gx, const double* __restrict__ gy,
-                                                 const double* __restrict__ gz, int nx, int ny, int nz,
-                                                 const double* __restrict__ monVals, double* __restrict__ vals,
-                                                 GridBox box, NnCand cand) {
+__global__ void __launch_bounds__(kRB) k_nn_fill_box(const double* __restrict__ X, CellGrid cg,
+                                                     const int* __restrict__ starts,
+                                                     const int* __restrict__ cellNodes, const double* __restrict__ gx,
+                                                     const double* __restrict__ gy, const double* __restrict__ gz,
+                                                     int nx, int ny, int nz, const double* __restrict__ monVals,
+                                                     double* __restrict__ vals, GridBox box, NnCand cand) {
   constexpr int DD = D * D;
   const long long p = (long long)blockIdx.x * kRB + threadIdx.x;
   if (p >= box_rows(box)) return;
@@ -210,6 +213,132 @@
   for (int e = 0; e < DD; ++e) vals[row * DD + e] = monVals[(size_t)bi * DD + e];
 }
 
+constexpr int kSup = 8;
+
+__host__ __device__ inline int sup_cells(int n) { return (n + kSup - 1) / kSup; }
+
+template <int D>
+__global__ void __launch_bounds__(kRB) k_super_count(CellGrid cg, const int* __restrict__ starts,
+                                                     int* __restrict__ sup) {
+  const int n0 = cg.n[0], n1 = cg.n[1], n2 = (D == 3) ? cg.n[2] : 1;
+  const int ns0 = sup_cells(n0), ns1 = sup_cells(n1), ns2 = (D == 3) ? sup_cells(n2) : 1;
+  constexpr int W = (D == 3) ? kSup * kSup : kSup;
+  const int t = blockIdx.x * kRB + threadIdx.x;
+  const int s = t / W, w = t % W;
+  int cnt = 0;
+  if (s < ns0 * ns1 * ns2) {
+    const int s0 = s % ns0, s1 = (s / ns0) % ns1, s2 = s / (ns0 * ns1);
+    const int xa = s0 * kSup, xb = min(xa + kSup, n0);
+    const int cy = s1 * kSup + w % kSup, cz = s2 * kSup + w / kSup;
+    if (cy < n1 && cz < n2) {
+      const int base = (cz * n1 + cy) * n0;
+      cnt = starts[base + xb] - starts[base + xa];
+    }
+  }
+#pragma unroll
+  for (int off = W / 2; off > 0; off >>= 1) cnt += __shfl_down(cnt, off, W);
+  if (w == 0 && s < ns0 * ns1 * ns2) sup[s] = cnt;
+}
+
+template <int D>
+__global__ void __launch_bounds__(kRB) k_nn_fill(const double* __restrict__ X, CellGrid cg,
+                                                 const int* __restrict__ starts, const int* __restrict__ cellNodes,
+                                                 const int* __restrict__ sup, const double* __restrict__ gx,
+                                                 const double* __restrict__ gy, const double* __restrict__ gz, int nx,
+                                                 int ny, int nz, const double* __restrict__ monVals,
+                                                 double* __restrict__ vals, GridBox box, NnCand cand) {
+  constexpr int DD = D * D;
+  const long long p = (long long)blockIdx.x * kRB + threadIdx.x;
+  if (p >= box_rows(box)) return;
+  int sx, sy, k;
+  const size_t row = box_row(box, p, nx, ny, sx, sy, k);
+  const int i = (D == 2) ? sx : sy, j = (D == 2) ? sy : sx;
+  double q[3] = {gx[i], gy[j], D == 3 ? gz[k] : 0.0};
+  int c[3] = {0, 0, 0};
+  cellOf<D>(q, cg, c);
+  const int c0 = c[0], c1 = c[1], c2 = c[2];
+  const int n0 = cg.n[0], n1 = cg.n[1], n2 = (D == 3) ? cg.n[2] : 1;
+  const int ns0 = sup_cells(n0), ns1 = sup_cells(n1);
+  const double h2 = cg.hmin * cg.hmin;
+  double best = INFINITY;
+  int bi = -1, bg = -1;
+  auto visit = [&](int cz, int cy, int xa, int xb) {
+    const int base = (cz * n1 + cy) * n0;
+    const int tb = starts[base + xb + 1];
+    for (int t = starts[base + xa]; t < tb; ++t) {
+      const int v = cellNodes[t];
+      const int gv = cand.gid ? cand.gid[v] : v;
+      double dd = 0.0;
+#pragma unroll
+      for (int d = 0; d < D; ++d) {
+        const double df = q[d] - X[(size_t)v * D + d];
+        dd += df * df;
+      }
+      if (dd < best || (dd == best && gv < bg)) {
+        best = dd;
+        bi = v;
+        bg = gv;
+      }
+    }
+  };
+  auto term = [](int a) {
+    const double m = (double)(a - 1) - 1e-6;
+    return a > 1 ? m * m : 0.0;
+  };
+  int rmax = 0;
+#pragma unroll
+  for (int d = 0; d < D; ++d) rmax = max(rmax, max(c[d], cg.n[d] - 1 - c[d]));
+  visit(c2, c1, c0, c0);
+  for (int r = 1; r <= rmax; ++r) {
+    const int x0 = max(c0 - r, 0), x1 = min(c0 + r, n0 - 1);
+    const int y0 = max(c1 - r, 0), y1 = min(c1 + r, n1 - 1);
+    const int z0 = (D == 3) ? max(c2 - r, 0) : 0, z1 = (D == 3) ? min(c2 + r, n2 - 1) : 0;
+    auto rowOf = [&](int cz, int cy, int dy, int dz) {
+      const double rem = best / h2 - (term(dy) + term(dz));
+      if (rem < 0.0) return;
+      const int w = (int)fmin(sqrt(rem), 1e9) + 2;
+      visit(cz, cy, max(x0, c0 - w), min(x1, c0 + w));
+    };
+    for (int cz = z0; cz <= z1; ++cz) {
+      const int dz = (D == 3) ? abs(cz - c2) : 0;
+      if (D == 3 && dz == r) {
+        for (int cy = y0; cy <= y1; ++cy) rowOf(cz, cy, abs(cy - c1), dz);
+        continue;
+      }
+      if (c1 - r >= 0) rowOf(cz, c1 - r, r, dz);
+      if (c1 + r < n1) rowOf(cz, c1 + r, r, dz);
+      const bool hasL = c0 - r >= 0, hasR = c0 + r < n0;
+      if (!hasL && !hasR) continue;
+      const int ya = max(c1 - r + 1, 0), yb = min(c1 + r - 1, n1 - 1);
+      for (int cy = ya; cy <= yb;) {
+        const int ye = min(yb, (cy / kSup) * kSup + kSup - 1);
+        const int srow = ((cz / kSup) * ns1 + cy / kSup) * ns0;
+        const bool l = hasL && sup[srow + (c0 - r) / kSup] > 0, rt = hasR && sup[srow + (c0 + r) / kSup] > 0;
+        if (l || rt)
+          for (int y = cy; y <= ye; ++y) {
+            if (best < (term(r) + term(abs(y - c1)) + term(dz)) * h2) continue;
+            if (l) visit(cz, y, c0 - r, c0 - r);
+            if (rt) visit(cz, y, c0 + r, c0 + r);
+          }
+        cy = ye + 1;
+      }
+    }
+    const double lb = ((double)r - 1e-6) * cg.hmin;
+    if (bi >= 0 && best < lb * lb) break;
+  }
+  if (cand.gid) {
+    double gap = INFINITY;
+#pragma unroll
+    for (int d = 0; d < D; ++d) gap = fmin(gap, fmin(q[d] - cand.slo[d], cand.shi[d] - q[d]));
+    if (!(bi >= 0 && gap > 0.0 && best < gap * gap * (1.0 - 1e-9))) {
+      atomicOr(cand.fail, 1);
+      if (bi < 0) return;
+    }
+  }
+#pragma unroll
+  for (int e = 0; e < DD; ++e) vals[row * DD + e] = monVals[(size_t)bi * DD + e];
+}
+
 template <int D>
 __global__ void __launch_bounds__(kRB) k_select_owned(const double* __restrict__ X, const int* __restrict__ ownLocal,
                                                       const int* __restrict__ ownGid, int nOwned, int nranks, int rank,
@@ -255,9 +384,45 @@
   }
 }
 
-template <int D>
-__global__ void __launch_bounds__(kRB) k_smooth(const double* __restrict__ in, double* __restrict__ out, int nx,
-                                                int ny, int nz, GridBox box) {
+constexpr int kRunsY = 32768;
+
+template <int D>
+__global__ void __launch_bounds__(kRB) k_smooth(const double* __restrict__ in, double* __restrict__ out,
+                                                double* __restrict__ pad, int nx, int ny, int nz, GridBox box) {
+  constexpr int DD = D * D;
+  const int bx = box.hi[0] - box.lo[0] + 1, by = box.hi[1] - box.lo[1] + 1, bz = box.hi[2] - box.lo[2] + 1;
+  const int xe = blockIdx.x * kRB + threadIdx.x;
+  const long long run = (long long)blockIdx.z * kRunsY + blockIdx.y;
+  if (xe >= bx * DD || run >= (long long)by * bz) return;
+  const int i = box.lo[0] + xe / DD, j = box.lo[1] + (int)(run % by), k = box.lo[2] + (int)(run / by);
+  const long long S = (long long)(nx + 1) * DD, P = (long long)(ny + 1) * S;
+  const long long e = ((long long)k * (ny + 1) + j) * S + (long long)box.lo[0] * DD + xe;
+  const bool interior = i >= 1 && i < nx && j >= 1 && j < ny && (D == 2 || (k >= 1 && k < nz));
+  double v;
+  if (!interior) {
+    v = in[e];
+  } else if constexpr (D == 2) {
+    v = 0.6 * in[e];
+    v += 0.1 * in[e + DD];
+    v += 0.1 * in[e - DD];
+    v += 0.1 * in[e + S];
+    v += 0.1 * in[e - S];
+  } else {
+    const double h = 0.4 / 6.0;
+    v = 0.6 * in[e] + h * in[e + DD] + h * in[e - DD] + h * in[e + S] + h * in[e - S] + h * in[e + P] + h * in[e - P];
+  }
+  out[e] = v;
+  if (D == 3 && pad) {
+    const long long c = e / DD;
+    const int q = xe % DD;
+    pad[c * 10 + q] = v;
+    if (q == DD - 1) pad[c * 10 + 9] = 0.0;
+  }
+}
+
+template <int D>
+__global__ void __launch_bounds__(kRB) k_smooth_row(const double* __restrict__ in, double* __restrict__ out, int nx,
+                                                    int ny, int nz, GridBox box) {
   constexpr int DD = D * D;
   const long long p = (long long)blockIdx.x * kRB + threadIdx.x;
   const long long P = (long long)(nx + 1) * (ny + 1);
@@ -288,6 +453,28 @@
 __global__ void __launch_bounds__(kRB) k_box_commit(const double* __restrict__ src, double* __restrict__ vals,
                                                     double* __restrict__ pad, int nx, int ny, int nz, GridBox box) {
   constexpr int DD = D * D;
+  const int xe = blockIdx.x * kRB + threadIdx.x;
+  const long long run = (long long)blockIdx.z * kRunsY + blockIdx.y;
+  if (xe >= (nx + 1) * DD || run >= (long long)(ny + 1) * (D == 3 ? nz + 1 : 1)) return;
+  const int i = xe / DD, j = (int)(run % (ny + 1)), k = (int)(run / (ny + 1));
+  const long long e = run * (nx + 1) * DD + xe;
+  const bool in = i >= box.lo[0] && i <= box.hi[0] && j >= box.lo[1] && j <= box.hi[1] && k >= box.lo[2] &&
+                  k <= box.hi[2];
+  const double v = in ? src[e] : __builtin_nan("");
+  vals[e] = v;
+  if (D == 3 && pad) {
+    const long long c = e / DD;
+    const int q = xe % DD;
+    pad[c * 10 + q] = v;
+    if (q == DD - 1) pad[c * 10 + 9] = 0.0;
+  }
+}
+
+template <int D>
+__global__ void __launch_bounds__(kRB) k_box_commit_row(const double* __restrict__ src, double* __restrict__ vals,
+                                                        double* __restrict__ pad, int nx, int ny, int nz,
+                                                        GridBox box) {
+  constexpr int DD = D * D;
   const long long c = (long long)blockIdx.x * kRB + threadIdx.x;
   const long long P = (long long)(nx + 1) * (ny + 1);
   if (c >= P * (D == 3 ? nz + 1 : 1)) return;
@@ -359,11 +546,22 @@
 template <int D>
 void launch_nn_fill(const double* X, const CellGrid& cg, const int* starts, const int* cellNodes, const double* gx,
                     const double* gy, const double* gz, int nx, int ny, int nz, const double* monVals, double* vals,
-                    const GridBox& box, hipStream_t st, const NnCand& cand) {
+                    const GridBox& box, int* sup, hipStream_t st, const NnCand& cand) {
   const long long n = host_box_rows(box);
-  if (n > 0)
-    hipLaunchKernelGGL(k_nn_fill<D>, dim3(blocks(n)), dim3(kRB), 0, st, X, cg, starts, cellNodes, gx, gy, gz, nx, ny,
-                       nz, monVals, vals, box, cand);
+  if (n <= 0) return;
+  if (!sup) {
+    hipLaunchKernelGGL(k_nn_fill_box<D>, dim3(blocks(n)), dim3(kRB), 0, st, X, cg, starts, cellNodes, gx, gy, gz, nx,
+                       ny, nz, monVals, vals, box, cand);
+    return;
+  }
+  hipLaunchKernelGGL(k_super_count<D>, dim3(blocks((long long)nn_super_cells(cg) * (D == 3 ? kSup * kSup : kSup))),
+                     dim3(kRB), 0, st, cg, starts, sup);
+  hipLaunchKernelGGL(k_nn_fill<D>, dim3(blocks(n)), dim3(kRB), 0, st, X, cg, starts, cellNodes, sup, gx, gy, gz, nx,
+                     ny, nz, monVals, vals, box, cand);
+}
+
+size_t nn_super_cells(const CellGrid& cg) {
+  return (size_t)sup_cells(cg.n[0]) * sup_cells(cg.n[1]) * sup_cells(cg.n[2]);
 }
 
 template <int D>
@@ -382,17 +580,69 @@
                        nRecv, cx, cgid);
 }
 
-template <int D>
-void launch_smooth(const double* in, double* out, int nx, int ny, int nz, const GridBox& box, hipStream_t st) {
+static dim3 run_grid(long long runEntries, long long runs) {
+  return dim3(blocks(runEntries), (unsigned)std::min<long long>(runs, kRunsY), (unsigned)((runs + kRunsY - 1) / kRunsY));
+}
+
+template <int D>
+void launch_smooth(const double* in, double* out, double* pad, int nx, int ny, int nz, const GridBox& box,
+                   bool parentKernels, hipStream_t st) {
   const long long n = host_box_rows(box);
-  if (n > 0) hipLaunchKernelGGL(k_smooth<D>, dim3(blocks(n)), dim3(kRB), 0, st, in, out, nx, ny, nz, box);
+  if (n <= 0) return;
+  if (parentKernels) {
+    hipLaunchKernelGGL(k_smooth_row<D>, dim3(blocks(n)), dim3(kRB), 0, st, in, out, nx, ny, nz, box);
+    return;
+  }
+  const long long bx = box.hi[0] - box.lo[0] + 1;
+  hipLaunchKernelGGL(k_smooth<D>, run_grid(bx * D * D, n / bx), dim3(kRB), 0, st, in, out, pad, nx, ny, nz, box);
 }
 
 template <int D>
 void launch_box_commit(const double* src, double* vals, double* pad, int nx, int ny, int nz, const GridBox& box,
-                       hipStream_t st) {
-  const long long rows = (long long)(nx + 1) * (ny + 1) * (D == 3 ? nz + 1 : 1);
-  hipLaunchKernelGGL(k_box_commit<D>, dim3(blocks(rows)), dim3(kRB), 0, st, src, vals, pad, nx, ny, nz, box);
+                       bool parentKernels, hipStream_t st) {
+  const long long runs = (long long)(ny + 1) * (D == 3 ? nz + 1 : 1), rows = (long long)(nx + 1) * runs;
+  if (parentKernels)
+    hipLaunchKernelGGL(k_box_commit_row<D>, dim3(blocks(rows)), dim3(kRB), 0, st, src, vals, pad, nx, ny, nz, box);
+  else
+    hipLaunchKernelGGL(k_box_commit<D>, run_grid((long long)(nx + 1) * D * D, runs), dim3(kRB), 0, st, src, vals, pad,
+                       nx, ny, nz, box);
+}
+
+template <int D>
+void launch_smooth_commit(double* tmp, double* tmp2, double* vals, double* pad, int nx, int ny, int nz,
+                          const GridBox& R, int passes, bool part, bool parentKernels, hipStream_t st) {
+  const int gn[3] = {nx, ny, D == 3 ? nz : 0};
+  auto widen = [&](int w) {
+    GridBox o = R;
+    for (int d = 0; d < D; ++d) {
+      o.lo[d] = std::max(0, R.lo[d] - w);
+      o.hi[d] = std::min(gn[d], R.hi[d] + w);
+    }
+    return o;
+  };
+  const size_t bytes = (size_t)(nx + 1) * (ny + 1) * (D == 3 ? nz + 1 : 1) * D * D * sizeof(double);
+  if (!part && !parentKernels) {
+    double* cur = smooth_fill_in_vals(passes, part, parentKernels) ? vals : tmp;
+    for (int it = 0; it < passes; ++it) {
+      double* oth = cur == vals ? tmp : vals;
+      launch_smooth<D>(cur, oth, it == passes - 1 ? pad : nullptr, nx, ny, nz, R, false, st);
+      cur = oth;
+    }
+    if (passes == 0 && D == 3 && pad) launch_pad_rows(vals, (long long)(bytes / sizeof(double) / 9), pad, st);
+    return;
+  }
+  double* cur = tmp;
+  double* oth = part ? tmp2 : vals;
+  for (int it = 0; it < passes; ++it) {
+    launch_smooth<D>(cur, oth, nullptr, nx, ny, nz, widen(part ? passes - 1 - it : 0), parentKernels, st);
+    std::swap(cur, oth);
+  }
+  if (part) {
+    launch_box_commit<D>(cur, vals, pad, nx, ny, nz, R, parentKernels, st);
+  } else {
+    if (cur != vals) (void)hipMemcpyAsync(vals, cur, bytes, hipMemcpyDeviceToDevice, st);
+    if (D == 3 && pad) launch_pad_rows(vals, (long long)(bytes / sizeof(double) / 9), pad, st);
+  }
 }
 
 void launch_rows_gather(int D, const int* idx, int n, const double* in, double* out, hipStream_t st) {
@@ -410,13 +660,17 @@
   template void launch_monitor_tv<D>(const double*, int, const double*, double*, hipStream_t);                  \
   template void launch_nn_fill<D>(const double*, const CellGrid&, const int*, const int*, const double*,        \
                                   const double*, const double*, int, int, int, const double*, double*,          \
-                                  const GridBox&, hipStream_t, const NnCand&);                                 \
+                                  const GridBox&, int*, hipStream_t, const NnCand&);                           \
   template void launch_select_owned<D>(const double*, const int*, const int*, int, int, int, const double*, int*, \
                                        double*, int, hipStream_t);                                               \
   template void launch_build_cand<D>(const double*, const int*, int, const double*, int, double*, int*,          \
                                      hipStream_t);                                                               \
-  template void launch_smooth<D>(const double*, double*, int, int, int, const GridBox&, hipStream_t);           \
-  template void launch_box_commit<D>(const double*, double*, double*, int, int, int, const GridBox&, hipStream_t);
+  template void launch_smooth<D>(const double*, double*, double*, int, int, int, const GridBox&, bool,          \
+                                 hipStream_t);                                                                   \
+  template void launch_box_commit<D>(const double*, double*, double*, int, int, int, const GridBox&, bool,       \
+                                     hipStream_t);                                                               \
+  template void launch_smooth_commit<D>(double*, double*, double*, double*, int, int, int, const GridBox&, int,  \
+                                        bool, bool, hipStream_t);
 MMX_REGRID_INST(2)
 MMX_REGRID_INST(3)
 #undef MMX_REGRID_INST
diff --git a/mm-admm_amd/python/mmadmm_amd.py b/mm-admm_amd/python/mmadmm_amd.py
--- a/mm-admm_amd/python/mmadmm_amd.py
+++ b/mm-admm_amd/python/mmadmm_amd.py
@@ -138,6 +138,10 @@
     L.mmadmm_debug_blockgrad.argtypes = [ctypes.c_void_p, ctypes.c_int, c_double_p, c_double_p, ctypes.c_int,
                                          c_double_p]
     L.mmadmm_devmath.argtypes = [ctypes.c_int, ctypes.c_int, c_double_p, c_double_p]
+    L.mmadmm_debug_smooth.argtypes = [ctypes.c_int] * 4 + [c_double_p, c_int_p, ctypes.c_int, ctypes.c_int, c_double_p,
+                                                         c_double_p]
+    L.mmadmm_debug_nn_fill.argtypes = ([ctypes.c_int, ctypes.c_int, c_double_p, c_int_p, c_double_p, c_int_p] +
+                                       [ctypes.c_int] * 3 + [c_double_p] * 4 + [c_int_p, c_double_p, c_int_p])
     vp = ctypes.c_void_p
     L.mmadmm_comm_unique_id.argtypes = [vp, ctypes.c_int]
     L.mmadmm_comm_create_rccl.argtypes = [ctypes.c_int, ctypes.c_int, vp, ctypes.c_int, ctypes.POINTER(vp)]
@@ -845,3 +849,40 @@
     out = np.zeros_like(x)
     _check(lib().mmadmm_devmath(op, x.size, _dp(x), _dp(out)))
     return out
+
+
+def debug_smooth(dim, shape, vals, box=None, passes=None, part=False, pad=False):
+    nx, ny = int(shape[0]), int(shape[1])
+    nz = int(shape[2]) if dim == 3 else 0
+    rows = (nx + 1) * (ny + 1) * (nz + 1)
+    v = np.ascontiguousarray(vals, dtype=np.float64).reshape(-1)
+    if v.size != rows * dim * dim:
+        raise ValueError(f"debug_smooth: vals must hold {rows * dim * dim} values")
+    b = np.ascontiguousarray(box if box is not None else ((0, 0, 0), (nx, ny, nz)), dtype=np.int32).reshape(6)
+    out = np.zeros_like(v)
+    p = np.zeros(rows * 10) if (pad and dim == 3) else None
+    _check(lib().mmadmm_debug_smooth(dim, nx, ny, nz, _dp(v), _ip(b), (5 if dim == 2 else 2) if passes is None else passes,
+                                     int(part), _dp(out), _dp(p) if p is not None else None))
+    return (out, p) if pad else out
+
+
+def debug_nn_fill(dim, X, mon, ncell, grid, box=None, gid=None, sbox=None):
+    X = np.ascontiguousarray(X, dtype=np.float64).reshape(-1, dim)
+    mon = np.ascontiguousarray(mon, dtype=np.float64).reshape(-1)
+    if mon.size != X.shape[0] * dim * dim:
+        raise ValueError("debug_nn_fill: mon must hold nV * dim^2 values")
+    g = [np.ascontiguousarray(a, dtype=np.float64) for a in grid]
+    nx, ny = (g[0].size - 1, g[1].size - 1) if dim == 2 else (g[1].size - 1, g[0].size - 1)
+    nz = g[2].size - 1 if dim == 3 else 0
+    b = np.ascontiguousarray(box if box is not None else ((0, 0, 0), (nx, ny, nz)), dtype=np.int32).reshape(6)
+    nc = np.ascontiguousarray(ncell, dtype=np.int32).reshape(dim)
+    gd = np.ascontiguousarray(gid, dtype=np.int32) if gid is not None else None
+    sb = np.ascontiguousarray(sbox, dtype=np.float64).reshape(2 * dim) if sbox is not None else None
+    if gd is not None and (gd.size != X.shape[0] or sb is None):
+        raise ValueError("debug_nn_fill: gid needs one id per vertex and a search box")
+    out = np.zeros((nx + 1) * (ny + 1) * (nz + 1) * dim * dim)
+    fail = np.zeros(1, dtype=np.int32)
+    _check(lib().mmadmm_debug_nn_fill(dim, X.shape[0], _dp(X), _ip(gd) if gd is not None else None,
+                                      _dp(sb) if sb is not None else None, _ip(nc), nx, ny, nz, _dp(g[0]), _dp(g[1]),
+                                      _dp(g[2]) if dim == 3 else None, _dp(mon), _ip(b), _dp(out), _ip(fail)))
+    return out, int(fail[0])
```

Result: no change. 2653 (-0.1%).
